# bempt/uda_aerial_semantic_segmentation_research

Measured on AMD Instinct MI355X. Metric: training images/sec at 512x512, higher is better.
Workload: dtype fp32

## Files before the change

include/udaseg.h:

```cpp
#ifndef UDASEG_H
#define UDASEG_H

#include <stddef.h>
#include <stdint.h>

#ifdef __cplusplus
extern "C" {
#endif

#define UDASEG_OK 0
#define UDASEG_E_BADARG (-1)
#define UDASEG_E_UNSUPPORTED (-2)
#define UDASEG_E_WORKSPACE (-3)
#define UDASEG_E_HIP (-4)

#define UDASEG_ACT_NONE 0
#define UDASEG_ACT_LEAKY 1

int udaseg_version(void);
#define UDASEG_OPT_GENERIC_GATHER 0
#define UDASEG_OPT_F32_SPLIT 1
#define UDASEG_OPT_WGRAD_GENERIC 2
#define UDASEG_OPT_F32_HALO 3
#define UDASEG_OPT_F3_CFG 4
#define UDASEG_OPT_F3_WS 5
#define UDASEG_OPT_F3_SIGNS 6
#define UDASEG_OPT_IGEMM_TILE 7
#define UDASEG_OPT_IGEMM_X3 8
#define UDASEG_OPT_NO_FOLD 9
#define UDASEG_OPT_WGRAD_X3_BLOCKS 10
#define UDASEG_OPT_WGRAD_BLOCKS 11
#define UDASEG_OPT_WGRAD_NO_XCD 12
#define UDASEG_OPT_WGRAD_X3 13
#define UDASEG_OPT_NO_WGRAD_HALO 14
#define UDASEG_OPT_WGRAD_F3_BLOCKS 15
#define UDASEG_OPT_WGRAD_HALO_BLOCKS 16
#define UDASEG_OPT_WGRAD_DEEP_BLOCKS 17
#define UDASEG_OPT_WGRAD_DB 18
#define UDASEG_OPT_REDUCE_BLOCKS 19
#define UDASEG_OPT_BN_APPLY_PT 20
#define UDASEG_OPT_GEMM_1X1_TILE 21
#define UDASEG_OPT_GEMM_1X1 22
#define UDASEG_OPT_GEMM_1X1_MAXM 23
#define UDASEG_OPT_NO_STREAM 24
#define UDASEG_OPT_HALO_CFG 25
#define UDASEG_OPT_NO_HALO 26
#define UDASEG_OPT_NO_HALO_S2 27
#define UDASEG_OPT_HALO_W16 28
#define UDASEG_OPT_HALO_DEEP 29
#define UDASEG_OPT_HALO_S2_CK 30
#define UDASEG_OPT_UP_CFG 31
#define UDASEG_OPT_WGRAD_UP_BLOCKS 32
#define UDASEG_OPT_COUNT 33
int udaseg_set_option(int key, int value);
int udaseg_get_option(int key);
int udaseg_option_count(void);
const char* udaseg_option_name(int key);
int udaseg_option_epoch(void);
const char* udaseg_last_error(void);
int udaseg_device_count(void);
int udaseg_memset_async(void* ptr, int value, size_t bytes, void* stream);
int udaseg_stream_wait(void* waiter_stream, void* signal_stream);

typedef struct {
  int n, hi, wi, ci;
  int ho, wo, co;
  int kh, kw, stride, pad;
} udaseg_conv_desc;


int udaseg_conv2d_fwd(const udaseg_conv_desc* d, const float* x, const float* w, const float* bias, float* y,
                      int act, float slope, int accumulate, void* stream);
int udaseg_conv2d_fwd_bnstats(const udaseg_conv_desc* d, const float* x, const float* w, const float* bias, float* y,
                              double* stats, void* stream);
int udaseg_conv2d_fwd_fused(const udaseg_conv_desc* d, const float* x, const float* w, const float* bias,
                            const float* residual, float* y, int act, float slope, void* stream);
int udaseg_conv2d_fwd_bf16(const udaseg_conv_desc* d, const void* x, const void* w, const float* bias, const void* residual,
                           void* y, int out_f32, int act, float slope, double* stats, void* stream);
int udaseg_conv2d_dgrad_bf16(const udaseg_conv_desc* d, const void* dy, const void* w_t, void* dx, int accumulate,
                             void* stream);
int udaseg_conv2d_wgrad_bf16(const udaseg_conv_desc* d, const void* x, const void* dy, float* dw, int accumulate, void* stream);
int udaseg_conv2d_dgrad(const udaseg_conv_desc* d, const float* dy, const float* w_t, float* dx, int accumulate,
                        void* stream);
int udaseg_conv2d_dgrad_bnreduce_ok(const udaseg_conv_desc* d);
int udaseg_conv2d_dgrad_bnreduce(const udaseg_conv_desc* d, const float* dy, const float* w_t, float* dx, const float* prev_y,
                                 const float* save_mean, const float* save_rstd, const float* gamma, const float* beta, int act,
                                 float slope, double* bsums, void* stream);
int udaseg_conv2d_dgrad_bnreduce_bf16_ok(const udaseg_conv_desc* d);
int udaseg_conv2d_dgrad_bnreduce_bf16(const udaseg_conv_desc* d, const void* dy, const void* w_t, void* dx, const void* prev_y,
                                      const float* save_mean, const float* save_rstd, const float* gamma, const float* beta,
                                      int act, float slope, double* bsums, void* stream);
int udaseg_conv2d_wgrad(const udaseg_conv_desc* d, const float* x, const float* dy, float* dw, int accumulate,
                        void* stream);
int udaseg_conv2d_fwd_upcat(const udaseg_conv_desc* d, const float* a, const float* skip, int ca, const float* w,
                            const float* bias, float* y, int act, float slope, double* stats, void* stream);
int udaseg_conv2d_fwd_upcat_bf16(const udaseg_conv_desc* d, const void* a, const void* skip, int ca, const void* w,
                                 const float* bias, void* y, int act, float slope, double* stats, void* stream);
int udaseg_conv2d_dgrad_split(const udaseg_conv_desc* d, const float* dy, const float* w_t, float* dx_a, float* dx_b, int ca,
                              void* stream);
int udaseg_conv2d_dgrad_split_bf16(const udaseg_conv_desc* d, const void* dy, const void* w_t, void* dx_a, void* dx_b, int ca,
                                   void* stream);
int udaseg_conv2d_wgrad_part(const udaseg_conv_desc* d, const float* src, int src_c, int c_off, int up, const float* dy,
                             float* dw, int accumulate, void* stream);
int udaseg_conv2d_wgrad_part_bf16(const udaseg_conv_desc* d, const void* src, int src_c, int c_off, int up, const void* dy,
                                  float* dw, int accumulate, void* stream);
int udaseg_pack_dgrad_weights(const udaseg_conv_desc* d, const float* w, float* w_t, void* stream);
int udaseg_pack_dgrad_batched(const float* arena, float* packed, const int* table, int entries, void* stream);
double udaseg_conv_flops(const udaseg_conv_desc* d);

int udaseg_nchw_to_nhwc(const float* x, float* y, int n, int c, int h, int w, int cpad, void* stream);

int udaseg_bn_replicas(void);
int udaseg_bn_stats(const float* y, int64_t pixels, int c, double* sums, void* stream);
int udaseg_bn_stats_bf16(const void* y, int64_t pixels, int c, double* sums, void* stream);
int udaseg_bn_apply(const float* y, const double* sums, const float* gamma, const float* beta, const float* residual,
                    float* z, int64_t pixels, int c, float eps, float momentum, float* running_mean,
                    float* running_var, float* save_mean, float* save_rstd, int act, float slope, void* stream);
int udaseg_bn_apply_eval(const float* y, const float* gamma, const float* beta, const float* running_mean,
                         const float* running_var, const float* residual, float* z, int64_t pixels, int c, float eps,
                         int act, float slope, void* stream);
int udaseg_bn_fold(const float* w, const float* bias, const float* gamma, const float* beta, const float* running_mean,
                   const float* running_var, float eps, int co, int row_len, float* w_folded, float* bias_folded, void* stream);
int udaseg_bn_bwd_reduce(const float* dz, const float* z, const float* y, const float* save_mean,
                         const float* save_rstd, const float* gamma, const float* beta, int64_t pixels, int c,
                         double* bsums, int act, float slope, void* stream);
int udaseg_bn_bwd_apply(const float* dz, const float* z, const float* y, const float* save_mean,
                        const float* save_rstd, const float* gamma, const float* beta, const double* bsums, float* dy,
                        float* dres, float* dgamma, float* dbeta, int64_t pixels, int c, int act, float slope,
                        int accumulate_dy, int accumulate_dres, int accumulate_param, void* stream);
int udaseg_act_bwd(const float* dz, const float* z, float* dy, int64_t count, int act, float slope, void* stream);
int udaseg_channel_sum(const float* x, int64_t pixels, int c, float* out,
                       int accumulate, void* stream);
int udaseg_channel_sum_ws(const float* x, int64_t pixels, int c, float* out, int accumulate, float* scratch,
                          size_t scratch_bytes, void* stream);
size_t udaseg_channel_sum_scratch_bytes(int c);

int udaseg_maxpool3x3s2_fwd(const float* x, float* y, uint8_t* idx, int n, int h, int w, int c, void* stream);
int udaseg_maxpool3x3s2_bwd(const float* dy, const uint8_t* idx, float* dx, int n, int h, int w, int c, int accumulate,
                            void* stream);
int udaseg_upsample2x_concat_fwd(const float* a, const float* skip, float* out, int n, int h, int w, int ca, int cb,
                                 void* stream);
int udaseg_upsample2x_concat_bwd(const float* dout, float* da, float* dskip, int n, int h, int w, int ca, int cb,
                                 int accumulate_da, int accumulate_dskip, void* stream);

int udaseg_upsample2x_bilinear_concat_fwd(const void* a, const void* skip, void* out, int n, int h, int w, int ca, int cb,
                                          int bf16, void* stream);
int udaseg_upsample2x_bilinear_concat_bwd(const void* dout, void* da, void* dskip, int n, int h, int w, int ca, int cb,
                                          int accumulate_da, int accumulate_dskip, int bf16, void* stream);

int udaseg_ce_partials(void);
int udaseg_ce_fwd(const float* logits, const int64_t* target, int64_t pixels, int classes, int ldc, float* lse,
                  double* partials, float* loss, void* stream);
int udaseg_ce_bwd(const float* logits, const int64_t* target, const float* lse, const float* grad_out, int64_t pixels,
                  int classes, int ldc, float* dlogits, float* colsum_partials, float* colsum, void* stream);

int udaseg_ce_fwd_bwd(const float* logits, const int64_t* target, int64_t pixels, int classes, int ldc, double* partials, float* loss,
                      float* dlogits, float* colsum_partials, float* colsum, void* stream);
int udaseg_scale_unless_one(float* x, int64_t count, float* x2, int count2, const float* g, void* stream);

int udaseg_seg_partials(void);
int udaseg_dice_fwd(const float* logits, const int64_t* target, int batch, int64_t pix_per_image, int classes, int ldc,
                    float smooth, float eps, int pooled, double* sums, float* coef, float* loss, void* stream);
int udaseg_dice_bwd(const float* logits, const int64_t* target, const float* coef, const float* grad_out, float weight,
                    int batch, int64_t pix_per_image, int classes, int ldc, float* dlogits, int accumulate, void* stream);
int udaseg_focal_fwd(const float* logits, const int64_t* target, const float* class_weights, float alpha, float gamma,
                     int64_t pixels, int classes, int ldc, int mean, double* partials, float* loss, int accumulate,
                     void* stream);
int udaseg_focal_bwd(const float* logits, const int64_t* target, const float* class_weights, float alpha, float gamma,
                     const float* grad_out, float weight, int64_t pixels, int classes, int ldc, float* dlogits,
                     int accumulate, void* stream);
int udaseg_consistency_fwd(const float* z1, const float* z2, float temperature, int batch, int64_t pixels, int classes,
                           int ldc, double* partials, float* loss, void* stream);
int udaseg_consistency_bwd(const float* z1, const float* z2, float temperature, const float* grad_out, float weight,
                           int batch, int64_t pixels, int classes, int ldc, float* d1, float* d2, int accumulate,
                           void* stream);

int udaseg_argmax_confusion(const float* logits, const int64_t* target, int64_t pixels, int classes, int ldc,
                            int64_t* confusion, int64_t* pred, void* stream);

int udaseg_gap_splits(int hw);
int udaseg_gap_linear_sigmoid_fwd(const float* z, const float* w, const float* b, float* partial, float* pooled,
                                  float* p, int n, int hw, int c, void* stream);
int udaseg_gap_linear_sigmoid_bwd(const float* dp, const float* p, const float* pooled, const float* w, float* dz,
                                  float* dw, float* db, int n, int hw, int c, int accumulate_param, void* stream);
int udaseg_gap_linear_fwd(const float* z, const float* w, const float* b, float* partial, float* pooled, float* logit, int n,
                          int hw, int c, void* stream);
int udaseg_gap_linear_bwd(const float* dlogit, const float* pooled, const float* w, float* dz, float* dw, float* db, int n,
                          int hw, int c, int accumulate_param, void* stream);
int udaseg_bce_logits_fwd(const float* x, int n, float label, float weight, float* loss, int accumulate, void* stream);
int udaseg_bce_logits_bwd(const float* x, int n, float label, float weight, const float* grad_out, float* dx,
                          int accumulate, void* stream);
int udaseg_bce_logits_target_fwd(const float* x, const float* target, int n, float weight, float* loss, int accumulate,
                                 void* stream);
int udaseg_bce_logits_target_bwd(const float* x, const float* target, int n, float weight, const float* grad_out, float* dx,
                                 int accumulate, void* stream);

int udaseg_adam_flat(float* p, const float* g, float* m, float* v, int64_t count, float lr, float beta1, float beta2,
                     float eps, float bc1, float bc2, void* stream);

int udaseg_prepare_batch_u8(const uint8_t* images, const uint8_t* masks, const int32_t* d4, int n, int h, int w,
                            const float* mean255, const float* inv_std255, void* out_images, int cpad, int out_bf16,
                            int64_t* out_masks, int square_checked, void* stream);

int udaseg_set_workspace(void* ptr, size_t bytes);
size_t udaseg_workspace_bytes(const udaseg_conv_desc* d);

int udaseg_bn_apply_bf16(const void* y, const double* sums, const float* gamma, const float* beta, const void* residual,
                         void* z, int64_t pixels, int c, float eps, float momentum, float* running_mean, float* running_var,
                         float* save_mean, float* save_rstd, int act, float slope, void* stream);
int udaseg_bn_bwd_reduce_bf16(const void* dz, const void* z, const void* y, const float* save_mean, const float* save_rstd,
                              int64_t pixels, int c, double* bsums, int act, float slope, void* stream);
int udaseg_bn_bwd_apply_bf16(const void* dz, const void* z, const void* y, const float* save_mean, const float* save_rstd,
                             const float* gamma, const double* bsums, void* dy, void* dres, float* dgamma, float* dbeta,
                             int64_t pixels, int c, int act, float slope, int accumulate_dy, int accumulate_dres,
                             int accumulate_param, void* stream);
int udaseg_act_bwd_bf16(const void* dz, const void* z, void* dy, int64_t count, int act, float slope, void* stream);
int udaseg_channel_sum_bf16(const void* x, int64_t pixels, int c, float* out, int accumulate, void* stream);
int udaseg_channel_sum_bf16_ws(const void* x, int64_t pixels, int c, float* out, int accumulate, float* scratch,
                               size_t scratch_bytes, void* stream);
int udaseg_nchw_to_nhwc_bf16(const float* x, void* y, int n, int c, int h, int w, int cpad, void* stream);
int udaseg_cast_f32_to_bf16(const float* x, void* y, int64_t count, void* stream);
int udaseg_maxpool3x3s2_fwd_bf16(const void* x, void* y, uint8_t* idx, int n, int h, int w, int c, void* stream);
int udaseg_maxpool3x3s2_bwd_bf16(const void* dy, const uint8_t* idx, void* dx, int n, int h, int w, int c, int accumulate,
                                 void* stream);
int udaseg_upsample2x_concat_bwd_bf16(const void* dout, void* da, void* dskip, int n, int h, int w, int ca, int cb,
                                      int accumulate_da, int accumulate_dskip, void* stream);
int udaseg_gap_partial_bf16(const void* z, float* partial, int n, int hw, int c, void* stream);
int udaseg_gap_finish(const float* partial, const float* w, const float* b, float* pooled, float* p, int n, int hw, int c,
                      void* stream);
int udaseg_gap_bwd_broadcast_bf16(const float* dp, const float* p, const float* w, void* dz, int n, int hw, int c, void* stream);
int udaseg_gap_bwd_param(const float* dp, const float* p, const float* pooled, float* dw, float* db, int n, int c,
                         int accumulate_param, void* stream);
int udaseg_pack_dgrad_batched_bf16(const float* arena, void* packed, const int* table, int entries, void* stream);

int64_t udaseg_frag_elems(int n_out, int k_in, int ks);
int udaseg_set_stats_scratch(void* ptr, size_t bytes);
int udaseg_pack_frag_batched_bf16(const void* w16, const void* wt16, void* packed, const int* table, int entries, void* stream);
int udaseg_bn_finalize(const double* sums, const float* gamma, const float* beta, int64_t pixels, int c, float eps, float momentum,
                       float* running_mean, float* running_var, float* save_mean, float* save_rstd, float* scale, float* shift,
                       void* stream);
int udaseg_bn_bwd_apply_recompute_bf16(const void* dz, const void* y, const float* fwd_scale, const float* fwd_shift,
                                       const float* save_mean, const float* save_rstd, const float* gamma, const double* bsums,
                                       void* dy, float* dgamma, float* dbeta, int64_t pixels, int c, int act, float slope,
                                       void* stream);
int udaseg_conv2d_wgrad_halo_bf16_ok(const udaseg_conv_desc* d, int up_ca);
int udaseg_conv2d_wgrad_halo_bf16(const udaseg_conv_desc* d, const void* x, const void* skip, int up_ca, const void* dy, float* dw,
                                  void* stream);
int udaseg_conv2d_wgrad_bnin_bf16(const udaseg_conv_desc* d, const void* x, const float* in_scale, const float* in_shift, int in_act,
                                  float in_slope, const void* dy, float* dw, int accumulate, void* stream);
int udaseg_conv_frag_ok(const udaseg_conv_desc* d, int dgrad, int up_ca);
int udaseg_conv_frag_preferred(const udaseg_conv_desc* d, int dgrad, int up_ca);
int udaseg_conv2d_fwd_frag_bf16(const udaseg_conv_desc* d, const void* x, const void* skip, int up_ca, const void* wfrag,
                                const float* bias, const float* in_scale, const float* in_shift, int in_act, float in_slope,
                                void* y, int out_f32, int act, float slope, double* stats, void* stream);
int udaseg_conv2d_dgrad_frag_bf16(const udaseg_conv_desc* d, const void* dy, const void* wfrag_t, void* dx, void* dx2, int split,
                                  const void* prev_y, const float* save_mean, const float* save_rstd, const float* gamma,
                                  const float* beta, int bn_act, float bn_slope, double* bsums, int accumulate, void* stream);

int udaseg_pack_frag_batched_f32x3(const float* w32, const float* wt32, void* packed, const int* table, int entries, void* stream);
int udaseg_conv_f32x3_ok(const udaseg_conv_desc* d, int dgrad, int up_ca);
int udaseg_conv_f32x3_preferred(const udaseg_conv_desc* d, int dgrad, int up_ca);
int udaseg_f32x3_force_config(int cfg);
int udaseg_conv2d_fwd_f32x3(const udaseg_conv_desc* d, const float* x, const float* skip, int up_ca, const void* wfrag3,
                            const float* bias, float* y, int act, float slope, double* stats, void* stream);
int udaseg_conv2d_fwd_f32x3_bnin_ok(const udaseg_conv_desc* d, int up);
int udaseg_conv2d_fwd_f32x3_bnin_writes(const udaseg_conv_desc* d);
int udaseg_conv2d_fwd_f32x3_bnin(const udaseg_conv_desc* d, const float* x, int up, const float* in_scale, const float* in_shift,
                                 int in_act, float in_slope, float* z_out, const void* wfrag3, const float* bias, float* y, int act,
                                 float slope, double* stats, void* stream);
int udaseg_conv2d_wgrad_bnin_ok(const udaseg_conv_desc* d, int up);
int udaseg_conv2d_wgrad_bnin(const udaseg_conv_desc* d, const float* x, int up, const float* in_scale, const float* in_shift,
                             int in_act, float in_slope, const float* dy, float* dw, int accumulate, void* stream);
int udaseg_conv2d_dgrad_f32x3(const udaseg_conv_desc* d, const float* dy, const void* wfrag3_t, float* dx, float* dx2, int split,
                              const float* prev_y, const float* save_mean, const float* save_rstd, const float* gamma,
                              const float* beta, int bn_act, float bn_slope, double* bsums, int accumulate, void* stream);

int udaseg_conv2d_wgrad_halo_f32x3_ok(const udaseg_conv_desc* d, int up_ca);
int udaseg_conv2d_wgrad_halo_f32x3(const udaseg_conv_desc* d, const float* x, const float* skip, int up_ca, const float* dy,
                                   float* dw, void* stream);

int udaseg_conv_up_f32x3_ok(const udaseg_conv_desc* d, int up_ca);
int udaseg_pack_up_batched_f32x3(const float* w32, const float* wt32, void* packed, const int* table, int entries, void* stream);
int udaseg_conv2d_fwd_up_f32x3(const udaseg_conv_desc* d, const float* a, int up_ca, const void* wfrag_up, float* y, int accumulate,
                               double* stats, void* stream);
int udaseg_conv2d_dgrad_up_f32x3(const udaseg_conv_desc* d, const float* dy, int up_ca, const void* wfrag_up_t, float* da,
                                 const float* prev_y, const float* save_mean, const float* save_rstd, const float* gamma,
                                 const float* beta, int bn_act, float bn_slope, double* bsums, int accumulate, void* stream);
int udaseg_up_f32x3_force_config(int cfg);
int udaseg_conv2d_wgrad_up_f32x3_ok(const udaseg_conv_desc* d, int up_ca);
int udaseg_conv2d_wgrad_up_f32x3(const udaseg_conv_desc* d, const float* a, int up_ca, const float* dy, float* dw, void* stream);
int udaseg_conv2d_wgrad_halo_slice_f32x3(const udaseg_conv_desc* d, const float* x, const float* dy, float* dw, int ldw, int c_off,
                                         void* stream);
int udaseg_wgrad_up_set_blocks(int blocks);

int udaseg_conv_n16_f32x3_ok(const udaseg_conv_desc* d, int dgrad);
int udaseg_conv2d_fwd_n16_f32x3(const udaseg_conv_desc* d, const float* x, const float* in_scale, const float* in_shift, int in_act,
                                float in_slope, const void* wfrag, float* y, double* stats, void* stream);
int udaseg_conv2d_dgrad_n16_f32x3(const udaseg_conv_desc* d, const float* dy, const void* wfrag_t, float* dx, const float* prev_y,
                                  const float* save_mean, const float* save_rstd, const float* gamma, const float* beta, int bn_act,
                                  float bn_slope, double* bsums, void* stream);

int udaseg_conv_stem_f32x3_ok(const udaseg_conv_desc* d);
int udaseg_conv2d_fwd_stem_f32x3(const udaseg_conv_desc* d, const float* x, const void* wfrag, float* y, double* stats, void* stream);

int udaseg_debug_set_timeline(void* buffer, int blocks);

int udaseg_fill_f32(float* p, int64_t count, float value, void* stream);
int udaseg_axpy_f32(float* y, const float* x, int64_t count, float alpha, void* stream);
int udaseg_add_i64(int64_t* p, int64_t count, int64_t value, void* stream);
int udaseg_scale_f32(const float* x, float* y, int64_t count, float alpha, void* stream);

int udaseg_predict_gather_u8(const uint8_t* image, int h, int w, int th, int tw, int rows, int cols, int sy, int sx, int first,
                             int tiles, int views, const float* mean255, const float* inv_std255, void* out, int cpad,
                             int out_bf16, void* stream);
int udaseg_predict_blend(const float* logits, int ldc, int h, int w, int th, int tw, int rows, int cols, int sy, int sx, int first,
                         int tiles, int views, int classes, const float* win_y, const float* win_x, float* acc, int ldp,
                         float* wsum, void* stream);
int udaseg_predict_finish(float* probs, const float* wsum, int64_t pixels, int classes, int ldc, int64_t* labels, void* stream);
int udaseg_predict_threshold(const float* logits, int n, int hw, int classes, int ldc, float* out, void* stream);

int udaseg_prof_enable(int on);
int udaseg_prof_reset(void);
int udaseg_prof_read(int family, double* total_ms, double* total_flops, int64_t* launches);
int udaseg_prof_kernel_count(void);
const char* udaseg_prof_kernel_name(int kid);
int udaseg_prof_kernel_read(int kid, double* total_ms, double* total_flops, int64_t* launches);
int udaseg_prof_records(int family, int max_records, double* ms, double* flops, int* kind, int* desc11);

#ifdef __cplusplus
}
#endif
#endif
```

uda_aerial_semantic_segmentation_research_amd/_lib.py:

```python
import ctypes as C
import os

_HERE = os.path.dirname(os.path.abspath(__file__))
LIB_PATH = os.environ.get("UDASEG_LIB", os.path.join(_HERE, "libudaseg_hip.so"))

ACT_NONE = 0
ACT_LEAKY = 1


class ConvDesc(C.Structure):
    _fields_ = [(k, C.c_int) for k in ("n", "hi", "wi", "ci", "ho", "wo", "co", "kh", "kw", "stride", "pad")]


_P = C.c_void_p
_I = C.c_int
_L = C.c_int64
_F = C.c_float
_D = C.POINTER(ConvDesc)

SIGNATURES = {
    "udaseg_version": (_I, []),
    "udaseg_set_option": (_I, [_I, _I]),
    "udaseg_get_option": (_I, [_I]),
    "udaseg_option_count": (_I, []),
    "udaseg_option_name": (C.c_char_p, [_I]),
    "udaseg_option_epoch": (_I, []),
    "udaseg_last_error": (C.c_char_p, []),
    "udaseg_device_count": (_I, []),
    "udaseg_memset_async": (_I, [_P, _I, C.c_size_t, _P]),
    "udaseg_stream_wait": (_I, [_P, _P]),
    "udaseg_conv2d_fwd": (_I, [_D, _P, _P, _P, _P, _I, _F, _I, _P]),
    "udaseg_conv2d_fwd_bnstats": (_I, [_D, _P, _P, _P, _P, _P, _P]),
    "udaseg_conv2d_fwd_fused": (_I, [_D, _P, _P, _P, _P, _P, _I, _F, _P]),
    "udaseg_conv2d_fwd_bf16": (_I, [_D, _P, _P, _P, _P, _P, _I, _I, _F, _P, _P]),
    "udaseg_conv2d_dgrad_bf16": (_I, [_D, _P, _P, _P, _I, _P]),
    "udaseg_conv2d_wgrad_bf16": (_I, [_D, _P, _P, _P, _I, _P]),
    "udaseg_conv2d_dgrad": (_I, [_D, _P, _P, _P, _I, _P]),
    "udaseg_conv2d_wgrad": (_I, [_D, _P, _P, _P, _I, _P]),
    "udaseg_conv2d_dgrad_bnreduce_ok": (_I, [_D]),
    "udaseg_conv2d_dgrad_bnreduce": (_I, [_D, _P, _P, _P, _P, _P, _P, _P, _P, _I, _F, _P, _P]),
    "udaseg_conv2d_dgrad_bnreduce_bf16_ok": (_I, [_D]),
    "udaseg_conv2d_dgrad_bnreduce_bf16": (_I, [_D, _P, _P, _P, _P, _P, _P, _P, _P, _I, _F, _P, _P]),
    "udaseg_conv2d_fwd_upcat": (_I, [_D, _P, _P, _I, _P, _P, _P, _I, _F, _P, _P]),
    "udaseg_conv2d_fwd_upcat_bf16": (_I, [_D, _P, _P, _I, _P, _P, _P, _I, _F, _P, _P]),
    "udaseg_conv2d_dgrad_split": (_I, [_D, _P, _P, _P, _P, _I, _P]),
    "udaseg_conv2d_dgrad_split_bf16": (_I, [_D, _P, _P, _P, _P, _I, _P]),
    "udaseg_conv2d_wgrad_part": (_I, [_D, _P, _I, _I, _I, _P, _P, _I, _P]),
    "udaseg_conv2d_wgrad_part_bf16": (_I, [_D, _P, _I, _I, _I, _P, _P, _I, _P]),
    "udaseg_pack_dgrad_weights": (_I, [_D, _P, _P, _P]),
    "udaseg_pack_dgrad_batched": (_I, [_P, _P, _P, _I, _P]),
    "udaseg_conv_flops": (C.c_double, [_D]),
    "udaseg_nchw_to_nhwc": (_I, [_P, _P, _I, _I, _I, _I, _I, _P]),
    "udaseg_bn_replicas": (_I, []),
    "udaseg_bn_stats": (_I, [_P, _L, _I, _P, _P]),
    "udaseg_bn_stats_bf16": (_I, [_P, _L, _I, _P, _P]),
    "udaseg_bn_apply": (_I, [_P, _P, _P, _P, _P, _P, _L, _I, _F, _F, _P, _P, _P, _P, _I, _F, _P]),
    "udaseg_bn_apply_eval": (_I, [_P, _P, _P, _P, _P, _P, _P, _L, _I, _F, _I, _F, _P]),
    "udaseg_bn_fold": (_I, [_P, _P, _P, _P, _P, _P, _F, _I, _I, _P, _P, _P]),
    "udaseg_bn_bwd_reduce": (_I, [_P, _P, _P, _P, _P, _P, _P, _L, _I, _P, _I, _F, _P]),
    "udaseg_bn_bwd_apply": (_I, [_P, _P, _P, _P, _P, _P, _P, _P, _P, _P, _P, _P, _L, _I, _I, _F, _I, _I, _I, _P]),
    "udaseg_act_bwd": (_I, [_P, _P, _P, _L, _I, _F, _P]),
    "udaseg_channel_sum": (_I, [_P, _L, _I, _P, _I, _P]),
    "udaseg_channel_sum_ws": (_I, [_P, _L, _I, _P, _I, _P, C.c_size_t, _P]),
    "udaseg_channel_sum_scratch_bytes": (C.c_size_t, [_I]),
    "udaseg_maxpool3x3s2_fwd": (_I, [_P, _P, _P, _I, _I, _I, _I, _P]),
    "udaseg_maxpool3x3s2_bwd": (_I, [_P, _P, _P, _I, _I, _I, _I, _I, _P]),
    "udaseg_upsample2x_concat_fwd": (_I, [_P, _P, _P, _I, _I, _I, _I, _I, _P]),
    "udaseg_upsample2x_concat_bwd": (_I, [_P, _P, _P, _I, _I, _I, _I, _I, _I, _I, _P]),
    "udaseg_upsample2x_bilinear_concat_fwd": (_I, [_P, _P, _P, _I, _I, _I, _I, _I, _I, _P]),
    "udaseg_upsample2x_bilinear_concat_bwd": (_I, [_P, _P, _P, _I, _I, _I, _I, _I, _I, _I, _I, _P]),
    "udaseg_ce_partials": (_I, []),
    "udaseg_ce_fwd": (_I, [_P, _P, _L, _I, _I, _P, _P, _P, _P]),
    "udaseg_ce_bwd": (_I, [_P, _P, _P, _P, _L, _I, _I, _P, _P, _P, _P]),
    "udaseg_ce_fwd_bwd": (_I, [_P, _P, _L, _I, _I, _P, _P, _P, _P, _P, _P]),
    "udaseg_scale_unless_one": (_I, [_P, _L, _P, _I, _P, _P]),
    "udaseg_seg_partials": (_I, []),
    "udaseg_dice_fwd": (_I, [_P, _P, _I, _L, _I, _I, _F, _F, _I, _P, _P, _P, _P]),
    "udaseg_gap_linear_fwd": (_I, [_P, _P, _P, _P, _P, _P, _I, _I, _I, _P]),
    "udaseg_gap_linear_bwd": (_I, [_P, _P, _P, _P, _P, _P, _I, _I, _I, _I, _P]),
    "udaseg_bce_logits_target_fwd": (_I, [_P, _P, _I, _F, _P, _I, _P]),
    "udaseg_bce_logits_target_bwd": (_I, [_P, _P, _I, _F, _P, _P, _I, _P]),
    "udaseg_scale_f32": (_I, [_P, _P, _L, _F, _P]),
    "udaseg_prepare_batch_u8": (_I, [_P, _P, _P, _I, _I, _I, _P, _P, _P, _I, _I, _P, _I, _P]),
    "udaseg_predict_gather_u8": (_I, [_P, _I, _I, _I, _I, _I, _I, _I, _I, _I, _I, _I, _P, _P, _P, _I, _I, _P]),
    "udaseg_predict_blend": (_I, [_P, _I, _I, _I, _I, _I, _I, _I, _I, _I, _I, _I, _I, _I, _P, _P, _P, _I, _P, _P]),
    "udaseg_predict_finish": (_I, [_P, _P, _L, _I, _I, _P, _P]),
    "udaseg_predict_threshold": (_I, [_P, _I, _I, _I, _I, _P, _P]),
    "udaseg_dice_bwd": (_I, [_P, _P, _P, _P, _F, _I, _L, _I, _I, _P, _I, _P]),
    "udaseg_focal_fwd": (_I, [_P, _P, _P, _F, _F, _L, _I, _I, _I, _P, _P, _I, _P]),
    "udaseg_focal_bwd": (_I, [_P, _P, _P, _F, _F, _P, _F, _L, _I, _I, _P, _I, _P]),
    "udaseg_consistency_fwd": (_I, [_P, _P, _F, _I, _L, _I, _I, _P, _P, _P]),
    "udaseg_consistency_bwd": (_I, [_P, _P, _F, _P, _F, _I, _L, _I, _I, _P, _P, _I, _P]),
    "udaseg_argmax_confusion": (_I, [_P, _P, _L, _I, _I, _P, _P, _P]),
    "udaseg_gap_splits": (_I, [_I]),
    "udaseg_gap_linear_sigmoid_fwd": (_I, [_P, _P, _P, _P, _P, _P, _I, _I, _I, _P]),
    "udaseg_gap_linear_sigmoid_bwd": (_I, [_P, _P, _P, _P, _P, _P, _P, _I, _I, _I, _I, _P]),
    "udaseg_bce_logits_fwd": (_I, [_P, _I, _F, _F, _P, _I, _P]),
    "udaseg_bce_logits_bwd": (_I, [_P, _I, _F, _F, _P, _P, _I, _P]),
    "udaseg_adam_flat": (_I, [_P, _P, _P, _P, _L, _F, _F, _F, _F, _F, _F, _P]),
    "udaseg_bn_apply_bf16": (_I, [_P, _P, _P, _P, _P, _P, _L, _I, _F, _F, _P, _P, _P, _P, _I, _F, _P]),
    "udaseg_bn_bwd_reduce_bf16": (_I, [_P, _P, _P, _P, _P, _L, _I, _P, _I, _F, _P]),
    "udaseg_bn_bwd_apply_bf16": (_I, [_P, _P, _P, _P, _P, _P, _P, _P, _P, _P, _P, _L, _I, _I, _F, _I, _I, _I, _P]),
    "udaseg_act_bwd_bf16": (_I, [_P, _P, _P, _L, _I, _F, _P]),
    "udaseg_channel_sum_bf16": (_I, [_P, _L, _I, _P, _I, _P]),
    "udaseg_channel_sum_bf16_ws": (_I, [_P, _L, _I, _P, _I, _P, C.c_size_t, _P]),
    "udaseg_nchw_to_nhwc_bf16": (_I, [_P, _P, _I, _I, _I, _I, _I, _P]),
    "udaseg_cast_f32_to_bf16": (_I, [_P, _P, _L, _P]),
    "udaseg_maxpool3x3s2_fwd_bf16": (_I, [_P, _P, _P, _I, _I, _I, _I, _P]),
    "udaseg_maxpool3x3s2_bwd_bf16": (_I, [_P, _P, _P, _I, _I, _I, _I, _I, _P]),
    "udaseg_upsample2x_concat_bwd_bf16": (_I, [_P, _P, _P, _I, _I, _I, _I, _I, _I, _I, _P]),
    "udaseg_gap_partial_bf16": (_I, [_P, _P, _I, _I, _I, _P]),
    "udaseg_gap_finish": (_I, [_P, _P, _P, _P, _P, _I, _I, _I, _P]),
    "udaseg_gap_bwd_broadcast_bf16": (_I, [_P, _P, _P, _P, _I, _I, _I, _P]),
    "udaseg_gap_bwd_param": (_I, [_P, _P, _P, _P, _P, _I, _I, _I, _P]),
    "udaseg_pack_dgrad_batched_bf16": (_I, [_P, _P, _P, _I, _P]),
    "udaseg_bn_finalize": (_I, [_P, _P, _P, _L, _I, _F, _F, _P, _P, _P, _P, _P, _P, _P]),
    "udaseg_bn_bwd_apply_recompute_bf16": (_I, [_P, _P, _P, _P, _P, _P, _P, _P, _P, _P, _P, _L, _I, _I, _F, _P]),
    "udaseg_conv2d_wgrad_halo_bf16_ok": (_I, [_D, _I]),
    "udaseg_conv2d_wgrad_halo_bf16": (_I, [_D, _P, _P, _I, _P, _P, _P]),
    "udaseg_conv2d_wgrad_bnin_bf16": (_I, [_D, _P, _P, _P, _I, _F, _P, _P, _I, _P]),
    "udaseg_frag_elems": (_L, [_I, _I, _I]),
    "udaseg_set_stats_scratch": (_I, [_P, C.c_size_t]),
    "udaseg_pack_frag_batched_bf16": (_I, [_P, _P, _P, _P, _I, _P]),
    "udaseg_conv_frag_ok": (_I, [_D, _I, _I]),
    "udaseg_conv_frag_preferred": (_I, [_D, _I, _I]),
    "udaseg_conv2d_fwd_frag_bf16": (_I, [_D, _P, _P, _I, _P, _P, _P, _P, _I, _F, _P, _I, _I, _F, _P, _P]),
    "udaseg_conv2d_dgrad_frag_bf16": (_I, [_D, _P, _P, _P, _P, _I, _P, _P, _P, _P, _P, _I, _F, _P, _I, _P]),
    "udaseg_pack_frag_batched_f32x3": (_I, [_P, _P, _P, _P, _I, _P]),
    "udaseg_conv2d_wgrad_halo_f32x3_ok": (_I, [_D, _I]),
    "udaseg_conv2d_wgrad_halo_f32x3": (_I, [_D, _P, _P, _I, _P, _P, _P]),
    "udaseg_conv_f32x3_ok": (_I, [_D, _I, _I]),
    "udaseg_f32x3_force_config": (_I, [_I]),
    "udaseg_conv_f32x3_preferred": (_I, [_D, _I, _I]),
    "udaseg_conv2d_fwd_f32x3": (_I, [_D, _P, _P, _I, _P, _P, _P, _I, _F, _P, _P]),
    "udaseg_conv2d_fwd_f32x3_bnin_ok": (_I, [_D, _I]),
    "udaseg_conv2d_fwd_f32x3_bnin_writes": (_I, [_D]),
    "udaseg_conv2d_fwd_f32x3_bnin": (_I, [_D, _P, _I, _P, _P, _I, _F, _P, _P, _P, _P, _I, _F, _P, _P]),
    "udaseg_conv2d_wgrad_bnin_ok": (_I, [_D, _I]),
    "udaseg_conv2d_wgrad_bnin": (_I, [_D, _P, _I, _P, _P, _I, _F, _P, _P, _I, _P]),
    "udaseg_conv2d_dgrad_f32x3": (_I, [_D, _P, _P, _P, _P, _I, _P, _P, _P, _P, _P, _I, _F, _P, _I, _P]),
    "udaseg_conv_up_f32x3_ok": (_I, [_D, _I]),
    "udaseg_pack_up_batched_f32x3": (_I, [_P, _P, _P, _P, _I, _P]),
    "udaseg_conv2d_fwd_up_f32x3": (_I, [_D, _P, _I, _P, _P, _I, _P, _P]),
    "udaseg_conv2d_dgrad_up_f32x3": (_I, [_D, _P, _I, _P, _P, _P, _P, _P, _P, _P, _I, _F, _P, _I, _P]),
    "udaseg_up_f32x3_force_config": (_I, [_I]),
    "udaseg_conv2d_wgrad_up_f32x3_ok": (_I, [_D, _I]),
    "udaseg_conv2d_wgrad_up_f32x3": (_I, [_D, _P, _I, _P, _P, _P]),
    "udaseg_conv2d_wgrad_halo_slice_f32x3": (_I, [_D, _P, _P, _P, _I, _I, _P]),
    "udaseg_wgrad_up_set_blocks": (_I, [_I]),
    "udaseg_conv_stem_f32x3_ok": (_I, [_D]),
    "udaseg_conv2d_fwd_stem_f32x3": (_I, [_D, _P, _P, _P, _P, _P]),
    "udaseg_conv_n16_f32x3_ok": (_I, [_D, _I]),
    "udaseg_conv2d_fwd_n16_f32x3": (_I, [_D, _P, _P, _P, _I, _F, _P, _P, _P, _P]),
    "udaseg_conv2d_dgrad_n16_f32x3": (_I, [_D, _P, _P, _P, _P, _P, _P, _P, _P, _I, _F, _P, _P]),
    "udaseg_set_workspace": (_I, [_P, C.c_size_t]),
    "udaseg_workspace_bytes": (C.c_size_t, [_D]),
    "udaseg_debug_set_timeline": (_I, [_P, _I]),
    "udaseg_fill_f32": (_I, [_P, _L, _F, _P]),
    "udaseg_axpy_f32": (_I, [_P, _P, _L, _F, _P]),
    "udaseg_add_i64": (_I, [_P, _L, _L, _P]),
    "udaseg_prof_enable": (_I, [_I]),
    "udaseg_prof_reset": (_I, []),
    "udaseg_prof_read": (_I, [_I, C.POINTER(C.c_double), C.POINTER(C.c_double), C.POINTER(C.c_int64)]),
    "udaseg_prof_kernel_count": (_I, []),
    "udaseg_prof_kernel_name": (C.c_char_p, [_I]),
    "udaseg_prof_kernel_read": (_I, [_I, C.POINTER(C.c_double), C.POINTER(C.c_double), C.POINTER(C.c_int64)]),
    "udaseg_prof_records": (_I, [_I, _I, C.POINTER(C.c_double), C.POINTER(C.c_double), C.POINTER(C.c_int), C.POINTER(C.c_int)]),
}

OPTIONS = {"GENERIC_GATHER": 0, "F32_SPLIT": 1, "WGRAD_GENERIC": 2, "F32_HALO": 3, "F3_CFG": 4, "F3_WS": 5, "F3_SIGNS": 6, "IGEMM_TILE": 7, "IGEMM_X3": 8, "NO_FOLD": 9, "WGRAD_X3_BLOCKS": 10, "WGRAD_BLOCKS": 11, "WGRAD_NO_XCD": 12, "WGRAD_X3": 13, "NO_WGRAD_HALO": 14, "WGRAD_F3_BLOCKS": 15, "WGRAD_HALO_BLOCKS": 16, "WGRAD_DEEP_BLOCKS": 17, "WGRAD_DB": 18, "REDUCE_BLOCKS": 19, "BN_APPLY_PT": 20, "GEMM_1X1_TILE": 21, "GEMM_1X1": 22, "GEMM_1X1_MAXM": 23, "NO_STREAM": 24, "HALO_CFG": 25, "NO_HALO": 26, "NO_HALO_S2": 27, "HALO_W16": 28, "HALO_DEEP": 29, "HALO_S2_CK": 30, "UP_CFG": 31, "WGRAD_UP_BLOCKS": 32}

_lib = None


def load():
    global _lib
    if _lib is not None:
        return _lib
    if not os.path.exists(LIB_PATH):
        raise RuntimeError(
            f"{LIB_PATH} not found: the HIP extension is not built. Run `python -c \"import __graft_entry__ as g; "
            f"g.build()\"` (or `make -C {os.path.join(_HERE, 'csrc')}`). There is no CPU fallback.")
    lib = C.CDLL(LIB_PATH)
    for name, (res, args) in SIGNATURES.items():
        fn = getattr(lib, name)
        fn.restype = res
        fn.argtypes = args
    _lib = lib
    return lib


def check(rc, what=""):
    if rc != 0:
        msg = load().udaseg_last_error().decode(errors="replace")
        raise RuntimeError(f"libudaseg_hip {what} failed (rc={rc}): {msg}")


def require_gpu():
    lib = load()
    if lib.udaseg_device_count() < 1:
        raise RuntimeError("libudaseg_hip: no HIP device visible; this path has no CPU fallback")
    return lib
```

uda_aerial_semantic_segmentation_research_amd/csrc/api.hip:

```cpp
#include <string.h>
#include <mutex>
#include <vector>

#include "common.h"
#include "options.h"

namespace udaseg {

static thread_local char g_err[512] = "";

void set_error(const char* fmt, ...) {
  va_list ap;
  va_start(ap, fmt);
  vsnprintf(g_err, sizeof(g_err), fmt, ap);
  va_end(ap);
}

int hip_fail(hipError_t e, const char* what) {
  set_error("%s: %s", what, hipGetErrorString(e));
  return UDASEG_E_HIP;
}

struct ProfRec {
  hipEvent_t a, b;
  double flops;
  int kind;
  udaseg_conv_desc d;
};
static bool g_prof_on = false;
struct KRec {
  hipEvent_t a, b;
  double flops;
};
static const char* const g_knames_fixed[PROF_NKERNELS] = {
    "conv_igemm_kernel<128, 128, 2, 2, false, false, false>", "conv_igemm_kernel<128, 64, 2, 2, false, false, false>",
    "conv_igemm_kernel<64, 64, 2, 2, false, false, false>",   "conv_igemm_kernel<128, 32, 4, 1, false, false, false>",
    "conv3x3_small_kernel<1, 1>",                             "conv3x3_small_kernel<2, 1>",
    "conv3x3_small_kernel<1, 2>",                             "conv_wgrad_kernel<64, 64, 2, 2, false>",
    "conv_wgrad_kernel<32, 128, 1, 4, false>",                "conv3x3_small_wgrad_kernel<1, 1>",
    "conv3x3_small_wgrad_kernel<2, 1>",                       "conv3x3_small_wgrad_kernel<1, 2>",
    "conv_igemm_kernel<*, bf16>",                             "conv_wgrad_bf16_kernel",
    "conv_igemm_kernel<128, 128, 2, 2, false, true, false>",  "conv_igemm_kernel<128, 64, 2, 2, false, true, false>",
    "conv_igemm_kernel<64, 64, 2, 2, false, true, false>",    "conv_igemm_kernel<128, 32, 4, 1, false, true, false>",
    "conv_wgrad_kernel<64, 64, 2, 2, true>",                  "conv_wgrad_kernel<32, 128, 1, 4, true>",
    "conv_igemm_kernel<128, 128, 2, 2, false, true, true>",   "conv_igemm_kernel<128, 64, 2, 2, false, true, true>",
    "conv_igemm_kernel<64, 64, 2, 2, false, true, true>",     "conv_igemm_kernel<128, 32, 4, 1, false, true, true>"};
constexpr int PROF_MAX_KERNELS = 160;
static std::vector<KRec> g_krecs[PROF_MAX_KERNELS];
static char g_knames_dyn[PROF_MAX_KERNELS][160];
static int g_nkernels = PROF_NKERNELS;

static std::mutex g_kprof_mutex;
int kprof_id(const char* name) {
  std::lock_guard<std::mutex> lock(g_kprof_mutex);
  for (int k = PROF_NKERNELS; k < g_nkernels; ++k)
    if (strcmp(g_knames_dyn[k], name) == 0) return k;
  if (g_nkernels >= PROF_MAX_KERNELS) {
    static bool warned = false;
    if (!warned) {
      fprintf(stderr, "libudaseg_hip: kernel-timing table full (%d symbols); '%s' and later symbols are booked under '%s'\n",
              PROF_MAX_KERNELS, name, g_knames_dyn[PROF_NKERNELS]);
      warned = true;
    }
    return PROF_NKERNELS;
  }
  strncpy(g_knames_dyn[g_nkernels], name, sizeof(g_knames_dyn[0]) - 1);
  return g_nkernels++;
}
static const char* kname(int kid) {
  if (kid < 0 || kid >= g_nkernels) return "";
  return kid < PROF_NKERNELS ? g_knames_fixed[kid] : g_knames_dyn[kid];
}
static std::vector<ProfRec> g_recs[2];
static std::vector<hipEvent_t> g_pool;
static hipEvent_t g_open[2];

static hipEvent_t get_event() {
  if (!g_pool.empty()) {
    hipEvent_t e = g_pool.back();
    g_pool.pop_back();
    return e;
  }
  hipEvent_t e;
  if (hipEventCreate(&e) != hipSuccess) return nullptr;
  return e;
}

hipEvent_t kprof_begin(hipStream_t s) {
  if (!g_prof_on) return nullptr;
  hipEvent_t a = get_event();
  if (a) (void)hipEventRecord(a, s);
  return a;
}

void kprof_end(int kid, hipEvent_t a, hipStream_t s, double flops) {
  if (!a) return;
  hipEvent_t b = get_event();
  if (!b || kid < 0 || kid >= PROF_MAX_KERNELS) return;
  (void)hipEventRecord(b, s);
  g_krecs[kid].push_back({a, b, flops});
}

static int g_prof_suspended = 0;
void prof_suspend(int on) { g_prof_suspended = on; }

void prof_begin(int family, hipStream_t s) {
  if (!g_prof_on || g_prof_suspended) return;
  g_open[family] = get_event();
  if (g_open[family]) (void)hipEventRecord(g_open[family], s);
}

void prof_end(int family, hipStream_t s, double flops, int kind, const udaseg_conv_desc* d) {
  if (!g_prof_on || g_prof_suspended || !g_open[family]) return;
  hipEvent_t b = get_event();
  if (!b) return;
  (void)hipEventRecord(b, s);
  ProfRec r = {g_open[family], b, flops, kind, {}};
  if (d) r.d = *d;
  g_recs[family].push_back(r);
  g_open[family] = nullptr;
}

}

using namespace udaseg;

extern "C" int udaseg_version(void) { return 100; }
extern "C" const char* udaseg_last_error(void) { return g_err; }

extern "C" int udaseg_device_count(void) {
  int n = 0;
  if (hipGetDeviceCount(&n) != hipSuccess) return 0;
  return n;
}

extern "C" int udaseg_memset_async(void* ptr, int value, size_t bytes, void* stream) {
  UDASEG_CHECK_ARG(ptr != nullptr || bytes == 0, "memset_async: NULL pointer");
  if (bytes == 0) return UDASEG_OK;
  hipError_t e = hipMemsetAsync(ptr, value, bytes, as_stream(stream));
  if (e != hipSuccess) return hip_fail(e, "hipMemsetAsync");
  return UDASEG_OK;
}

extern "C" int udaseg_stream_wait(void* waiter, void* signal) {
  constexpr int RING = 256;
  static hipEvent_t ring[16][RING] = {};
  static unsigned next[16] = {};
  static std::mutex mu;
  int dev = 0;
  UDASEG_CHECK_ARG(hipGetDevice(&dev) == hipSuccess && dev >= 0 && dev < 16, "stream_wait: no current HIP device");
  std::lock_guard<std::mutex> lk(mu);
  const unsigned slot = next[dev] % RING;
  if (ring[dev][slot] == nullptr) {
    hipError_t e = hipEventCreateWithFlags(&ring[dev][slot], hipEventDisableTiming);
    if (e != hipSuccess) {
      ring[dev][slot] = nullptr;
      return hip_fail(e, "hipEventCreateWithFlags(stream_wait ring)");
    }
  }
  hipEvent_t ev = ring[dev][slot];
  hipError_t e = hipEventRecord(ev, as_stream(signal));
  if (e != hipSuccess) return hip_fail(e, "hipEventRecord(stream_wait: is `signal` a stream of the current device?)");
  e = hipStreamWaitEvent(as_stream(waiter), ev, 0);
  if (e != hipSuccess) return hip_fail(e, "hipStreamWaitEvent(stream_wait)");
  ++next[dev];
  return UDASEG_OK;
}

extern "C" int udaseg_prof_enable(int on) {
  g_prof_on = on != 0;
  return UDASEG_OK;
}

extern "C" int udaseg_prof_reset(void) {
  for (int f = 0; f < 2; ++f) {
    for (auto& r : g_recs[f]) {
      g_pool.push_back(r.a);
      g_pool.push_back(r.b);
    }
    g_recs[f].clear();
  }
  for (int k = 0; k < g_nkernels; ++k) {
    for (auto& r : g_krecs[k]) {
      g_pool.push_back(r.a);
      g_pool.push_back(r.b);
    }
    g_krecs[k].clear();
  }
  return UDASEG_OK;
}

extern "C" int udaseg_prof_read(int family, double* total_ms, double* total_flops, int64_t* launches) {
  UDASEG_CHECK_ARG(family >= 0 && family < 2 && total_ms && total_flops && launches, "prof_read: bad arguments");
  double ms = 0.0, fl = 0.0;
  for (auto& r : g_recs[family]) {
    hipError_t e = hipEventSynchronize(r.b);
    if (e != hipSuccess) return hip_fail(e, "hipEventSynchronize(prof)");
    float t = 0.f;
    e = hipEventElapsedTime(&t, r.a, r.b);
    if (e != hipSuccess) return hip_fail(e, "hipEventElapsedTime(prof)");
    ms += t;
    fl += r.flops;
  }
  *total_ms = ms;
  *total_flops = fl;
  *launches = (int64_t)g_recs[family].size();
  return UDASEG_OK;
}

extern "C" int udaseg_prof_records(int family, int max_records, double* ms, double* flops, int* kind, int* desc11) {
  UDASEG_CHECK_ARG(family >= 0 && family < 2 && ms && flops && kind && desc11 && max_records >= 0, "prof_records: bad arguments");
  int n = 0;
  for (auto& r : g_recs[family]) {
    if (n >= max_records) break;
    hipError_t e = hipEventSynchronize(r.b);
    if (e != hipSuccess) return hip_fail(e, "hipEventSynchronize(prof)");
    float t = 0.f;
    e = hipEventElapsedTime(&t, r.a, r.b);
    if (e != hipSuccess) return hip_fail(e, "hipEventElapsedTime(prof)");
    ms[n] = t;
    flops[n] = r.flops;
    kind[n] = r.kind;
    const int v[11] = {r.d.n, r.d.hi, r.d.wi, r.d.ci, r.d.ho, r.d.wo, r.d.co, r.d.kh, r.d.kw, r.d.stride, r.d.pad};
    for (int i = 0; i < 11; ++i) desc11[n * 11 + i] = v[i];
    ++n;
  }
  return n;
}

namespace udaseg {
enum { K_INT, K_FLAG, K_OFF0 };
struct OptRow {
  const char* env;
  int kind, dflt;
};
static const OptRow g_opt_rows[UDASEG_OPT_COUNT] = {
     {"UDASEG_IGEMM_GENERIC", K_INT, 0},
     {"UDASEG_F32_SPLIT", K_OFF0, 1},
     {"UDASEG_WGRAD_GENERIC", K_INT, 0},
     {"UDASEG_F32_SPLIT", K_OFF0, 1},
     {"UDASEG_F3_CFG", K_INT, 0},
     {"UDASEG_F3_WS", K_OFF0, 1},
     {"UDASEG_F3_SIGNS", K_OFF0, 1},
     {"UDASEG_IGEMM_TILE", K_INT, 0},
     {"UDASEG_IGEMM_X3", K_INT, 1},
     {"UDASEG_NO_FOLD", K_FLAG, 0},
     {"UDASEG_WGRAD_X3_BLOCKS", K_INT, 1024},
     {"UDASEG_WGRAD_BLOCKS", K_INT, 0},
     {"UDASEG_WGRAD_NO_XCD", K_FLAG, 0},
     {"UDASEG_WGRAD_X3", K_OFF0, 1},
     {"UDASEG_NO_WGRAD_HALO", K_FLAG, 0},
     {"UDASEG_WGRAD_F3_BLOCKS", K_INT, 120},
     {"UDASEG_WGRAD_HALO_BLOCKS", K_INT, 96},
     {"UDASEG_WGRAD_DEEP_BLOCKS", K_INT, 0},
     {"UDASEG_WGRAD_DB", K_INT, 1},
     {"UDASEG_REDUCE_BLOCKS", K_INT, 0},
     {"UDASEG_BN_APPLY_PT", K_INT, 4},
     {"UDASEG_GEMM_1X1_TILE", K_INT, 0},
     {"UDASEG_GEMM_1X1", K_OFF0, 1},
     {"UDASEG_GEMM_1X1_MAXM", K_INT, 73728},
     {"UDASEG_NO_STREAM", K_FLAG, 0},
     {"UDASEG_HALO_CFG", K_INT, 0},
     {"UDASEG_NO_HALO", K_FLAG, 0},
     {"UDASEG_NO_HALO_S2", K_FLAG, 0},
     {"UDASEG_HALO_W16", K_INT, 6},
     {"UDASEG_HALO_DEEP", K_OFF0, 1},
     {"UDASEG_HALO_S2_CK", K_INT, 64},
     {"UDASEG_UP_CFG", K_INT, 0},
     {"UDASEG_WGRAD_UP_BLOCKS", K_INT, 0}};
int g_opt_val[UDASEG_OPT_COUNT];
static int g_opt_default[UDASEG_OPT_COUNT];
std::atomic<bool> g_opt_ready{false};
static std::atomic<int> g_opt_epoch{0};
static std::mutex g_opt_mutex;
void opt_init() {
  std::lock_guard<std::mutex> lk(g_opt_mutex);
  if (g_opt_ready.load(std::memory_order_relaxed)) return;
  for (int k = 0; k < UDASEG_OPT_COUNT; ++k) {
    const OptRow& r = g_opt_rows[k];
    const char* e = getenv(r.env);
    int v = r.dflt;
    if (r.kind == K_INT) v = e ? atoi(e) : r.dflt;
    else if (r.kind == K_FLAG) v = e != nullptr ? 1 : 0;
    else v = (e && atoi(e) == 0) ? 0 : 1;
    g_opt_default[k] = g_opt_val[k] = v;
  }
  g_opt_ready.store(true, std::memory_order_release);
}
}

extern "C" int udaseg_set_option(int key, int value) {
  UDASEG_CHECK_ARG(key >= 0 && key < UDASEG_OPT_COUNT, "set_option: unknown key %d (0 .. %d)", key, UDASEG_OPT_COUNT - 1);
  UDASEG_CHECK_ARG(value >= -1, "set_option: value must be >= 0, or -1 for the default");
  udaseg::opt_get(key);
  std::lock_guard<std::mutex> lk(udaseg::g_opt_mutex);
  udaseg::g_opt_val[key] = value < 0 ? udaseg::g_opt_default[key] : value;
  if (key == UDASEG_OPT_GENERIC_GATHER)
    udaseg::g_opt_val[UDASEG_OPT_WGRAD_GENERIC] = value < 0 ? udaseg::g_opt_default[UDASEG_OPT_WGRAD_GENERIC] : value;
  udaseg::g_opt_epoch.fetch_add(1);
  return UDASEG_OK;
}

extern "C" int udaseg_get_option(int key) {
  if (key < 0 || key >= UDASEG_OPT_COUNT) return -1;
  return udaseg::opt_get(key);
}

extern "C" int udaseg_option_count(void) { return UDASEG_OPT_COUNT; }
extern "C" const char* udaseg_option_name(int key) { return key >= 0 && key < UDASEG_OPT_COUNT ? udaseg::g_opt_rows[key].env : ""; }
extern "C" int udaseg_option_epoch(void) { return udaseg::g_opt_epoch.load(); }

extern "C" int udaseg_prof_kernel_count(void) { return g_nkernels; }
extern "C" const char* udaseg_prof_kernel_name(int kid) { return kname(kid); }

extern "C" int udaseg_prof_kernel_read(int kid, double* total_ms, double* total_flops, int64_t* launches) {
  UDASEG_CHECK_ARG(kid >= 0 && kid < g_nkernels && total_ms && total_flops && launches, "prof_kernel_read: bad arguments");
  double ms = 0.0, fl = 0.0;
  for (auto& r : g_krecs[kid]) {
    hipError_t e = hipEventSynchronize(r.b);
    if (e != hipSuccess) return hip_fail(e, "hipEventSynchronize(kprof)");
    float t = 0.f;
    e = hipEventElapsedTime(&t, r.a, r.b);
    if (e != hipSuccess) return hip_fail(e, "hipEventElapsedTime(kprof)");
    ms += t;
    fl += r.flops;
  }
  *total_ms = ms;
  *total_flops = fl;
  *launches = (int64_t)g_krecs[kid].size();
  return UDASEG_OK;
}
```

uda_aerial_semantic_segmentation_research_amd/csrc/common.h:

```cpp
#pragma once
#include <stdlib.h>
#include <hip/hip_runtime.h>
#include <stdint.h>
#include <stdio.h>
#include <stdarg.h>
#include <atomic>

#include "../../include/udaseg.h"
#include "options.h"

namespace udaseg {

void set_error(const char* fmt, ...);
int hip_fail(hipError_t e, const char* what);

#define UDASEG_CHECK_ARG(cond, ...)                 \
  do {                                              \
    if (!(cond)) {                                  \
      ::udaseg::set_error(__VA_ARGS__);             \
      return UDASEG_E_BADARG;                       \
    }                                               \
  } while (0)

#define UDASEG_LAUNCH_CHECK(what)                          \
  do {                                                     \
    hipError_t e__ = hipGetLastError();                    \
    if (e__ != hipSuccess) return ::udaseg::hip_fail(e__, what); \
  } while (0)

static inline hipStream_t as_stream(void* s) { return reinterpret_cast<hipStream_t>(s); }
static inline int64_t cdiv64(int64_t a, int64_t b) { return (a + b - 1) / b; }
static inline int cdiv(int a, int b) { return (a + b - 1) / b; }

typedef float f32x4 __attribute__((ext_vector_type(4)));
typedef float f32x16 __attribute__((ext_vector_type(16)));

__device__ __forceinline__ int fast_div(int n, int d, float rcp) {
  int q = (int)((float)n * rcp);
  int r = n - q * d;
  if (r < 0) { q -= 1; r += d; }
  if (r >= d) { q += 1; }
  return q;
}

__device__ __forceinline__ float act_apply(float x, int act, float slope) {
  return (act == UDASEG_ACT_LEAKY && x < 0.f) ? x * slope : x;
}
__device__ __forceinline__ float act_grad(float z, int act, float slope) {
  return (act == UDASEG_ACT_LEAKY && !(z > 0.f)) ? slope : 1.f;
}

__device__ __forceinline__ float wave_sum(float v) {
#pragma unroll
  for (int o = 32; o > 0; o >>= 1) v += __shfl_xor(v, o, 64);
  return v;
}
__device__ __forceinline__ double wave_sum_d(double v) {
#pragma unroll
  for (int o = 32; o > 0; o >>= 1) v += __shfl_xor(v, o, 64);
  return v;
}

template <int V, typename T>
__device__ __forceinline__ void block_fold_atomic(const T (&v)[V], T* __restrict__ dst, int cq, T* __restrict__ red) {
  const int tid = threadIdx.x, bs = blockDim.x;
#pragma unroll
  for (int e = 0; e < V; ++e) red[tid * V + e] = v[e];
  __syncthreads();
  if (cq >= bs) {
    const int base = (int)(((int64_t)blockIdx.x * bs) % cq);
    for (int j = tid; j < bs * V; j += bs) {
      int qq = base + j / V;
      if (qq >= cq) qq -= cq;
      atomicAdd(dst + qq * V + (j % V), red[j]);
    }
  } else {
    const int C = cq * V;
    for (int t = tid; t < C; t += bs) {
      T s = 0;
      for (int r = t / V; r < bs; r += cq) s += red[r * V + (t % V)];
      atomicAdd(dst + t, s);
    }
  }
  __syncthreads();
}

constexpr int BN_REPLICAS = 16;
constexpr int REDUCE_MAX_BLOCKS = 512;
static inline int reduce_max_blocks() {
  const int x = opt_get(UDASEG_OPT_REDUCE_BLOCKS);
  return x > 0 ? x : REDUCE_MAX_BLOCKS;
}

template <typename OutT>
__device__ __forceinline__ void pack_dgrad_tiles(const float* __restrict__ w, OutT* __restrict__ wt, int co, int T, int ci) {
  __shared__ float tile[32][33];
  const int ta = (co + 31) >> 5, tb = (ci + 31) >> 5;
  const int ntiles = T * ta * tb;
  const int row = threadIdx.x >> 3, q = threadIdx.x & 7;
  for (int tl = blockIdx.x; tl < ntiles; tl += gridDim.x) {
    const int b = tl % tb, r = tl / tb, a = r % ta, t = r / ta;
    {
      const int o = 32 * a + row, c = 32 * b + 4 * q;
      f32x4 v = {0.f, 0.f, 0.f, 0.f};
      if (o < co && c < ci) v = *reinterpret_cast<const f32x4*>(w + ((size_t)o * T + t) * ci + c);
#pragma unroll
      for (int k = 0; k < 4; ++k) tile[row][4 * q + k] = v[k];
    }
    __syncthreads();
    {
      const int c = 32 * b + row, o = 32 * a + 4 * q;
      if (c < ci && o < co) {
        OutT* dst = wt + ((size_t)c * T + t) * co + o;
        if constexpr (sizeof(OutT) == 4) {
          f32x4 v;
#pragma unroll
          for (int k = 0; k < 4; ++k) v[k] = tile[4 * q + k][row];
          *reinterpret_cast<f32x4*>(dst) = v;
        } else {
          unsigned short h[4];
#pragma unroll
          for (int k = 0; k < 4; ++k) h[k] = __builtin_bit_cast(unsigned short, (__bf16)tile[4 * q + k][row]);
          uint2 pk;
          pk.x = (unsigned)h[0] | ((unsigned)h[1] << 16);
          pk.y = (unsigned)h[2] | ((unsigned)h[3] << 16);
          *reinterpret_cast<uint2*>(dst) = pk;
        }
      }
    }
    __syncthreads();
  }
}
constexpr int PACK_DGRAD_GRID_X = 256;

void* workspace_ptr(size_t* bytes);

constexpr int CHSUM_REPLICAS = 16;
constexpr int CHSUM_DIRECT_BLOCKS = 32;
static __global__ void fold_replicas_kernel(const float* __restrict__ rep, int c, float* __restrict__ out, int accumulate) {
  const int i = blockIdx.x * blockDim.x + threadIdx.x;
  if (i >= c) return;
  float s = 0.f;
#pragma unroll
  for (int r = 0; r < CHSUM_REPLICAS; ++r) s += rep[(size_t)r * c + i];
  out[i] = accumulate ? out[i] + s : s;
}

struct StreamShape {
  int bs;
  int grid;
  int c4;
};

static inline StreamShape stream_shape(int64_t n4, int c4, int max_blocks = 2048, int per_thread = 4) {
  StreamShape s;
  s.c4 = c4;
  int unit;
  if (c4 <= 256) {
    s.bs = (256 / c4) * c4;
    unit = 1;
  } else {
    s.bs = 256;
    unit = (c4 + 255) / 256;
    while ((unit * 256) % c4 != 0) ++unit;
  }
  int64_t want = (n4 + (int64_t)s.bs * per_thread - 1) / ((int64_t)s.bs * per_thread);
  if (want > max_blocks) want = max_blocks;
  if (want < 1) want = 1;
  s.grid = (int)(((want + unit - 1) / unit) * unit);
  while ((int64_t)s.grid * s.bs < c4) s.grid += unit;
  return s;
}


static inline int apply_per_thread() {
  const int v = opt_get(UDASEG_OPT_BN_APPLY_PT);
  return (v < 1 || v > 256) ? 4 : v;
}

bool small_conv_applicable(int k, int stride, int pad, int ci_gather, int co_out);
int launch_small_conv(const float* x, const float* w, const float* bias, float* y, int n, int h, int wd, int ci, int co,
                      int flip, int accumulate, int act, float slope, double* stats, const float* residual, hipStream_t s,
                      int up = 0);
bool small_wgrad_applicable(int k, int stride, int pad, int ci, int co, int ntiles);
int launch_small_wgrad(const float* x, const float* dy, float* dw, int n, int h, int wd, int ci, int co, int accumulate,
                       hipStream_t s, int up = 0, const float* in_scale = nullptr, const float* in_shift = nullptr,
                       int in_act = 0, float in_slope = 0.f);

constexpr int PROF_NKERNELS = 24;
int kprof_id(const char* rocprof_symbol);
hipEvent_t kprof_begin(hipStream_t s);
void kprof_end(int kid, hipEvent_t a, hipStream_t s, double flops);
struct KTimer {
  std::atomic<int>* kid;
  hipStream_t s;
  hipEvent_t ev;
  double work;
  KTimer(std::atomic<int>* k, const char* rocprof_symbol, hipStream_t st, double w) : kid(k), s(st), work(w) {
    if (*kid < 0) *kid = kprof_id(rocprof_symbol);
    ev = kprof_begin(s);
  }
  ~KTimer() { kprof_end(*kid, ev, s, work); }
};
void prof_begin(int family, hipStream_t s);
void prof_suspend(int on);
void prof_end(int family, hipStream_t s, double flops, int kind, const udaseg_conv_desc* d);

}
```

uda_aerial_semantic_segmentation_research_amd/csrc/conv_n16_f32x3.hip:

```cpp
#include <stdlib.h>

#include "common.h"
#include "halo_common.h"

namespace udaseg {

struct N16Args {
  const float* x;
  const void* wf;
  float* y;
  int n, h, w, ci;
  double* stats;
  double* sscr;
  const float* bnb_y;
  const float* bnb_mean;
  const float* bnb_rstd;
  const float* bnb_gamma;
  const float* bnb_beta;
  int bnb_act;
  float bnb_slope;
  const float* in_scale;
  const float* in_shift;
  int in_act;
  float in_slope;
  int ntx, nty, nk16;
  int q1, q3;
  unsigned x_bytes, w_plane_bytes, y_bytes;
};

typedef float f32x4v __attribute__((ext_vector_type(4)));

struct N16Cfg {
  static constexpr int NT = 256, WM = 4, RPW = 2;
  static constexpr int TH = WM * RPW, TW = 32;
  static constexpr int HR = TH + 2, HWD = TW + 2;
  static constexpr int PLANE = HR * HWD * 32;
  static constexpr int LDS_HALO = 3 * PLANE;
  static constexpr int NPIECE = HR * HWD * 2;
  static constexpr int NI = (NPIECE + NT - 1) / NT;
  static constexpr int WCHUNK = 5 * 3 * 1024;
  static constexpr int NB = 2 * RPW;
};

template <int N>
__device__ __forceinline__ void row16_sum_n(float (&x)[N]) {
#pragma unroll
  for (int v = 0; v < N; ++v) asm volatile("v_add_f32_dpp %0, %0, %0 row_ror:8 row_mask:0xf bank_mask:0xf" : "+v"(x[v]));
  asm volatile("s_nop 1");
#pragma unroll
  for (int v = 0; v < N; ++v) asm volatile("v_add_f32_dpp %0, %0, %0 row_ror:4 row_mask:0xf bank_mask:0xf" : "+v"(x[v]));
  asm volatile("s_nop 1");
#pragma unroll
  for (int v = 0; v < N; ++v) asm volatile("v_add_f32_dpp %0, %0, %0 row_ror:2 row_mask:0xf bank_mask:0xf" : "+v"(x[v]));
  asm volatile("s_nop 1");
#pragma unroll
  for (int v = 0; v < N; ++v) asm volatile("v_add_f32_dpp %0, %0, %0 row_ror:1 row_mask:0xf bank_mask:0xf" : "+v"(x[v]));
  asm volatile("s_nop 1");
}

template <bool XF>
__global__ __launch_bounds__(256, 2) void conv3x3_n16_f32x3_kernel(const N16Args a) {
  using C = N16Cfg;
  extern __shared__ __attribute__((aligned(16))) char smem[];
  char* const wlds = smem + C::LDS_HALO;
  const int tid = threadIdx.x, lane = tid & 63;
  const int wave = __builtin_amdgcn_readfirstlane(tid >> 6);
  const int p = lane & 15, g = lane >> 4;

  const int H = a.h, W = a.w;
  const int ntiles = a.n * a.nty * a.ntx;
  const int oct = tid & 1;
  unsigned voff[C::NI], soffl[C::NI];
  unsigned inmask = 0;
#pragma unroll
  for (int i = 0; i < C::NI; ++i) soffl[i] = (unsigned)(((tid + i * C::NT) >> 1) * 32 + oct * 16);
  int img = 0, y0 = 0, x0 = 0;
  auto tile_setup = [&](int tl) {
    const int tx = tl % a.ntx;
    const int t2 = tl / a.ntx;
    const int ty = t2 % a.nty;
    img = t2 / a.nty;
    y0 = ty * C::TH;
    x0 = tx * C::TW;
#pragma unroll
    for (int i = 0; i < C::NI; ++i) {
      const int piece = tid + i * C::NT;
      const int pix = piece >> 1;
      const int hy = pix / C::HWD, hx = pix - hy * C::HWD;
      const int iy = y0 + hy - 1, ix = x0 + hx - 1;
      const bool ok = piece < C::NPIECE && (unsigned)iy < (unsigned)H && (unsigned)ix < (unsigned)W;
      voff[i] = ok ? (unsigned)((((img * H + iy) * W + ix) * a.ci + oct * 8) * 4) : 0x80000000u;
    }
  };
  __amdgpu_buffer_rsrc_t rs_x = __builtin_amdgcn_make_buffer_rsrc(const_cast<float*>(a.x), 0, (int)a.x_bytes, 0x00020000);
  __amdgpu_buffer_rsrc_t rs_w = __builtin_amdgcn_make_buffer_rsrc(const_cast<void*>(a.wf), 0, (int)(3u * a.w_plane_bytes), 0x00020000);

  u32x4 stage[C::NI][2];
  auto load_chunk = [&](int c) {
    const int soff = c * 64;
    const unsigned kill = (c * 16 + oct * 8 < a.ci) ? 0u : 0x80000000u;
    inmask = 0;
#pragma unroll
    for (int i = 0; i < C::NI; ++i) {
      stage[i][0] = __builtin_amdgcn_raw_buffer_load_b128(rs_x, (int)(voff[i] | kill), soff, 0);
      stage[i][1] = __builtin_amdgcn_raw_buffer_load_b128(rs_x, (int)(voff[i] | kill), soff + 16, 0);
      inmask |= (voff[i] != 0x80000000u ? 1u : 0u) << i;
    }
  };
  const bool xf_relu = a.in_act == UDASEG_ACT_LEAKY && a.in_slope == 0.f;
  auto store_chunk = [&](int c) {
    f32x4 sc0 = {0.f, 0.f, 0.f, 0.f}, sc1 = sc0, sh0 = sc0, sh1 = sc0;
    if constexpr (XF) {
      const int ch = c * 16 + oct * 8;
      if (ch < a.ci) {
        sc0 = *reinterpret_cast<const f32x4*>(a.in_scale + ch);
        sh0 = *reinterpret_cast<const f32x4*>(a.in_shift + ch);
        if (ch + 4 < a.ci) {
          sc1 = *reinterpret_cast<const f32x4*>(a.in_scale + ch + 4);
          sh1 = *reinterpret_cast<const f32x4*>(a.in_shift + ch + 4);
        }
      }
    }
#pragma unroll
    for (int i = 0; i < C::NI; ++i) {
      if (i < C::NI - 1 || tid + i * C::NT < C::NPIECE) {
        u32x4 lo = stage[i][0], hi = stage[i][1];
        if constexpr (XF) {
          const bool inside = (inmask >> i) & 1u;
          f32x4 l = __builtin_bit_cast(f32x4, lo), h = __builtin_bit_cast(f32x4, hi);
#pragma unroll
          for (int e = 0; e < 4; ++e) {
            float t0 = __builtin_fmaf(l[e], sc0[e], sh0[e]), t1 = __builtin_fmaf(h[e], sc1[e], sh1[e]);
            if (xf_relu) {
              t0 = t0 > 0.f ? t0 : 0.f;
              t1 = t1 > 0.f ? t1 : 0.f;
            } else {
              t0 = act_apply(t0, a.in_act, a.in_slope);
              t1 = act_apply(t1, a.in_act, a.in_slope);
            }
            l[e] = inside ? t0 : 0.f;
            h[e] = inside ? t1 : 0.f;
          }
          lo = __builtin_bit_cast(u32x4, l);
          hi = __builtin_bit_cast(u32x4, h);
        }
        u32x4 p0, p1, p2;
        split3(lo, hi, p0, p1, p2);
        *reinterpret_cast<u32x4*>(smem + soffl[i]) = p0;
        *reinterpret_cast<u32x4*>(smem + C::PLANE + soffl[i]) = p1;
        *reinterpret_cast<u32x4*>(smem + 2 * C::PLANE + soffl[i]) = p2;
      }
    }
  };

  {
    const int npc = a.nk16 * 5 * 64;
    for (int i = tid; i < 3 * npc; i += C::NT) {
      const int pl = i / npc, r = i - pl * npc;
      const int f = r >> 6, ln = r & 63;
      const u32x4 v = __builtin_amdgcn_raw_buffer_load_b128(rs_w, (int)(pl * a.w_plane_bytes + r * 16), 0, 0);
      *reinterpret_cast<u32x4*>(wlds + (f * 3 + pl) * 1024 + ln * 16) = v;
    }
  }

  int toff[5];
#pragma unroll
  for (int j = 0; j < 5; ++j) {
    int tap = 2 * j + (g >> 1);
    if (tap > 8) tap = 8;
    toff[j] = ((tap / 3) * C::HWD + (tap % 3)) * 32;
  }
  const int pbase = ((wave * C::RPW) * C::HWD + p) * 32 + (g & 1) * 16;

  __amdgpu_buffer_rsrc_t rs_y = __builtin_amdgcn_make_buffer_rsrc(a.y, 0, (int)a.y_bytes, 0x00020000);
  const bool want_stats = a.stats != nullptr && a.bnb_y == nullptr;
  const bool want_bnb = a.bnb_y != nullptr;
  __amdgpu_buffer_rsrc_t rs_p = __builtin_amdgcn_make_buffer_rsrc(const_cast<float*>(want_bnb ? a.bnb_y : a.x), 0,
                                                                  (int)(want_bnb ? a.y_bytes : 0u), 0x00020000);
  float s[8];
#pragma unroll
  for (int v = 0; v < 8; ++v) s[v] = 0.f;
  f32x4 sc = {0.f, 0.f, 0.f, 0.f}, sh = sc, mu = sc, rsd = sc;
  if (want_bnb) {
    mu = *reinterpret_cast<const f32x4*>(a.bnb_mean + 4 * g);
    rsd = *reinterpret_cast<const f32x4*>(a.bnb_rstd + 4 * g);
    const f32x4 gm = *reinterpret_cast<const f32x4*>(a.bnb_gamma + 4 * g), bt = *reinterpret_cast<const f32x4*>(a.bnb_beta + 4 * g);
#pragma unroll
    for (int e = 0; e < 4; ++e) {
      sc[e] = gm[e] * rsd[e];
      sh[e] = bt[e] - mu[e] * sc[e];
    }
  }

  int tile = blockIdx.x;
  if (tile < ntiles) {
    tile_setup(tile);
    load_chunk(0);
  }
  for (; tile < ntiles; tile += gridDim.x) {
    const int cimg = img, cy0 = y0, cx0 = x0;
    f32x4v acc[C::NB];
#pragma unroll
    for (int b = 0; b < C::NB; ++b) acc[b] = f32x4v{0.f, 0.f, 0.f, 0.f};
    for (int c = 0; c < a.nk16; ++c) {
      store_chunk(c);
      __syncthreads();
      if (c + 1 < a.nk16) {
        load_chunk(c + 1);
      } else if (tile + (int)gridDim.x < ntiles) {
        tile_setup(tile + gridDim.x);
        load_chunk(0);
      }
#pragma unroll
      for (int j = 0; j < 5; ++j) {
        const int G = 5 * c + j;
        if (G == a.q1 || G == a.q3) {
#pragma unroll
          for (int b = 0; b < C::NB; ++b) acc[b] = -acc[b];
        }
        u32x4 A[3];
#pragma unroll
        for (int pl = 0; pl < 3; ++pl) A[pl] = *reinterpret_cast<const u32x4*>(wlds + ((c * 5 + j) * 3 + pl) * 1024 + lane * 16);
#pragma unroll
        for (int b = 0; b < C::NB; ++b) {
          const int r = b >> 1, bx = b & 1;
          u32x4 B[3];
#pragma unroll
          for (int pl = 0; pl < 3; ++pl)
            B[pl] = *reinterpret_cast<const u32x4*>(smem + pl * C::PLANE + pbase + toff[j] + (r * C::HWD + bx * 16) * 32);
#pragma unroll
          for (int ij = 2; ij >= 0; --ij)
#pragma unroll
            for (int i = 0; i <= ij; ++i)
              acc[b] = __builtin_amdgcn_mfma_f32_16x16x32_bf16(__builtin_bit_cast(bf16x8, A[i]), __builtin_bit_cast(bf16x8, B[ij - i]), acc[b], 0, 0, 0);
        }
      }
      __syncthreads();
    }

#pragma unroll
    for (int b = 0; b < C::NB; ++b) {
      const int oy = cy0 + wave * C::RPW + (b >> 1), ox = cx0 + 16 * (b & 1) + p;
      const bool cv = oy < H && ox < W;
      const unsigned off = cv ? (((unsigned)((cimg * H + oy) * W + ox)) * 16u + 4u * (unsigned)g) * 4u : 0x80000000u;
      const u32x4 d = __builtin_bit_cast(u32x4, acc[b]);
      __builtin_amdgcn_raw_buffer_store_b128(d, rs_y, (int)off, 0, 0);
      if (want_stats) {
#pragma unroll
        for (int e = 0; e < 4; ++e) {
          const float q = cv ? acc[b][e] : 0.f;
          s[e] += q;
          s[4 + e] = __builtin_fmaf(q, q, s[4 + e]);
        }
      }
      if (want_bnb) {
        const f32x4 yv = __builtin_bit_cast(f32x4, __builtin_amdgcn_raw_buffer_load_b128(rs_p, (int)off, 0, 0));
#pragma unroll
        for (int e = 0; e < 4; ++e) {
          const float yy = yv[e];
          const float gg = cv ? acc[b][e] * act_grad(__builtin_fmaf(yy, sc[e], sh[e]), a.bnb_act, a.bnb_slope) : 0.f;
          s[e] += gg;
          s[4 + e] = __builtin_fmaf(gg, (yy - mu[e]) * rsd[e], s[4 + e]);
        }
      }
    }
  }
  if (want_stats || want_bnb) {
    asm volatile("s_nop 1");
    row16_sum_n(s);
    float* red = reinterpret_cast<float*>(smem);
    if (p == 0) {
#pragma unroll
      for (int e = 0; e < 4; ++e) {
        red[wave * 32 + 4 * g + e] = s[e];
        red[wave * 32 + 16 + 4 * g + e] = s[4 + e];
      }
    }
    __syncthreads();
    if (tid < 32) {
      const float tot = red[tid] + red[32 + tid] + red[64 + tid] + red[96 + tid];
      atomicAdd(a.stats + (size_t)(blockIdx.x % HALO_STATS_REPLICAS) * 32 + tid, (double)tot);
    }
  }
}

static bool n16_applicable(const udaseg_conv_desc* d, int dgrad) {
  if (!d || !f32_halo_enabled()) return false;
  if (d->kh != 3 || d->kw != 3 || d->stride != 1 || d->pad != 1 || d->ho != d->hi || d->wo != d->wi) return false;
  const int gathered = dgrad ? d->co : d->ci, produced = dgrad ? d->ci : d->co;
  if (produced != 16 || gathered % 8 != 0 || gathered < 8 || gathered > 32 || d->n <= 0 || d->hi <= 0 || d->wi < 16) return false;
  const long long px = (long long)d->n * d->hi * d->wi;
  return px * 32 * 4 < (1LL << 31);
}

static int launch_n16(N16Args a, hipStream_t s, double flops) {
  using C = N16Cfg;
  a.ntx = cdiv(a.w, C::TW);
  a.nty = cdiv(a.h, C::TH);
  a.nk16 = (a.ci + 15) / 16;
  a.q1 = a.q3 = -1;
  if (f3_signs_on()) {
    const int ng = 5 * a.nk16;
    a.q1 = (ng + 2) / 4;
    a.q3 = ng - a.q1;
  }
  const int lds = C::LDS_HALO + a.nk16 * C::WCHUNK;
  const long long ntiles = (long long)a.n * a.nty * a.ntx;
  if (ntiles <= 0) return UDASEG_OK;
  if (ntiles >= (1LL << 31)) return UDASEG_E_UNSUPPORTED;
  static int cus = 0;
  if (cus == 0) {
    int dev = 0;
    hipDeviceProp_t pr;
    cus = (hipGetDevice(&dev) == hipSuccess && hipGetDeviceProperties(&pr, dev) == hipSuccess && pr.multiProcessorCount > 0)
              ? pr.multiProcessorCount : 256;
  }
  const long long resident = (long long)cus * (a.nk16 == 1 ? 3 : 2);
  const long long blocks = ntiles < resident ? ntiles : resident;
  a.sscr = nullptr;
  const bool xf = a.in_scale != nullptr;
  auto kern = xf ? conv3x3_n16_f32x3_kernel<true> : conv3x3_n16_f32x3_kernel<false>;
  static std::atomic<bool> attr_done[2] = {{false}, {false}};
  if (!attr_done[xf]) {
    hipError_t e = hipFuncSetAttribute(reinterpret_cast<const void*>(kern), hipFuncAttributeMaxDynamicSharedMemorySize,
                                       C::LDS_HALO + 2 * C::WCHUNK);
    if (e != hipSuccess) return hip_fail(e, "hipFuncSetAttribute(conv3x3_n16_f32x3)");
    attr_done[xf] = true;
  }
  static std::atomic<int> kid[2] = {{-1}, {-1}};
  if (kid[xf] < 0) kid[xf] = kprof_id(xf ? "conv3x3_n16_f32x3_kernel<true>" : "conv3x3_n16_f32x3_kernel<false>");
  hipEvent_t ev = kprof_begin(s);
  hipLaunchKernelGGL(kern, dim3((unsigned)blocks), dim3(C::NT), lds, s, a);
  kprof_end(kid[xf], ev, s, flops);
  UDASEG_LAUNCH_CHECK("conv3x3_n16_f32x3 launch");
  return UDASEG_OK;
}

}

using namespace udaseg;

extern "C" int udaseg_conv_n16_f32x3_ok(const udaseg_conv_desc* d, int dgrad) { return n16_applicable(d, dgrad) ? 1 : 0; }

extern "C" int udaseg_conv2d_fwd_n16_f32x3(const udaseg_conv_desc* d, const float* x, const float* in_scale, const float* in_shift,
                                           int in_act, float in_slope, const void* wfrag, float* y, double* stats, void* stream) {
  UDASEG_CHECK_ARG(d && x && wfrag && y, "conv2d_fwd_n16_f32x3: NULL pointer");
  UDASEG_CHECK_ARG((in_scale == nullptr) == (in_shift == nullptr), "conv2d_fwd_n16_f32x3: in_scale and in_shift come together");
  UDASEG_CHECK_ARG(in_act == UDASEG_ACT_NONE || in_act == UDASEG_ACT_LEAKY, "conv2d_fwd_n16_f32x3: unknown activation %d", in_act);
  if (!n16_applicable(d, 0)) {
    set_error("conv2d_fwd_n16_f32x3: geometry not supported (ask udaseg_conv_n16_f32x3_ok first)");
    return UDASEG_E_UNSUPPORTED;
  }
  N16Args a = {};
  a.x = x; a.wf = wfrag; a.y = y;
  a.n = d->n; a.h = d->hi; a.w = d->wi; a.ci = d->ci;
  a.stats = stats;
  a.in_scale = in_scale; a.in_shift = in_shift; a.in_act = in_act; a.in_slope = in_slope;
  const long long px = (long long)d->n * d->hi * d->wi;
  a.x_bytes = (unsigned)(px * d->ci * 4);
  a.w_plane_bytes = (unsigned)(((d->ci + 15) / 16) * 5 * 1024);
  a.y_bytes = (unsigned)(px * 16 * 4);
  hipStream_t st = as_stream(stream);
  prof_begin(0, st);
  const int rc = launch_n16(a, st, udaseg_conv_flops(d));
  prof_end(0, st, udaseg_conv_flops(d), 0, d);
  return rc;
}

extern "C" int udaseg_conv2d_dgrad_n16_f32x3(const udaseg_conv_desc* d, const float* dy, const void* wfrag_t, float* dx,
                                             const float* prev_y, const float* save_mean, const float* save_rstd, const float* gamma,
                                             const float* beta, int bn_act, float bn_slope, double* bsums, void* stream) {
  UDASEG_CHECK_ARG(d && dy && wfrag_t && dx, "conv2d_dgrad_n16_f32x3: NULL pointer");
  const bool bn = prev_y != nullptr;
  UDASEG_CHECK_ARG(!bn || (save_mean && save_rstd && gamma && beta && bsums), "conv2d_dgrad_n16_f32x3: the BatchNorm-backward sums "
                   "need mean, rstd, gamma, beta, bsums");
  UDASEG_CHECK_ARG(bn || bsums == nullptr, "conv2d_dgrad_n16_f32x3: bsums without prev_y");
  if (!n16_applicable(d, 1)) {
    set_error("conv2d_dgrad_n16_f32x3: geometry not supported (ask udaseg_conv_n16_f32x3_ok first)");
    return UDASEG_E_UNSUPPORTED;
  }
  N16Args a = {};
  a.x = dy; a.wf = wfrag_t; a.y = dx;
  a.n = d->n; a.h = d->hi; a.w = d->wi; a.ci = d->co;
  if (bn) {
    a.bnb_y = prev_y; a.bnb_mean = save_mean; a.bnb_rstd = save_rstd; a.bnb_gamma = gamma; a.bnb_beta = beta;
    a.bnb_act = bn_act; a.bnb_slope = bn_slope; a.stats = bsums;
  }
  const long long px = (long long)d->n * d->hi * d->wi;
  a.x_bytes = (unsigned)(px * d->co * 4);
  a.w_plane_bytes = (unsigned)(((d->co + 15) / 16) * 5 * 1024);
  a.y_bytes = (unsigned)(px * 16 * 4);
  hipStream_t st = as_stream(stream);
  prof_begin(0, st);
  const int rc = launch_n16(a, st, udaseg_conv_flops(d));
  prof_end(0, st, udaseg_conv_flops(d), 1, d);
  return rc;
}
```

uda_aerial_semantic_segmentation_research_amd/csrc/conv_stem_f32x3.hip:

```cpp
#include <stdlib.h>

#include "common.h"
#include "halo_common.h"

namespace udaseg {

struct StemArgs {
  const float* x;
  const void* wf;
  float* y;
  int n, h, w;
  double* stats;
  int ntx, nty;
  int q1, q3;
  unsigned x_bytes, w_plane_bytes, y_bytes;
};

struct StemCfg {
  static constexpr int NT = 512, NW = 8;
  static constexpr int TH = 8, TW = 32;
  static constexpr int IR = 2 * TH + 5;
  static constexpr int NP = 35;
  static constexpr int ROWB = NP * 16;
  static constexpr int PLANE = IR * ROWB;
  static constexpr int LDS_BAND = 3 * PLANE;
  static constexpr int NPIECE = IR * NP;
  static constexpr int NI = (NPIECE + NT - 1) / NT;
  static constexpr int NFRAG = 7 * 2 * 2;
  static constexpr int LDS_W = 3 * NFRAG * 1024;
  static constexpr int LDS = LDS_BAND + LDS_W;
};

__global__ __launch_bounds__(512, 1) void conv_stem_f32x3_kernel(const StemArgs a) {
  using C = StemCfg;
  extern __shared__ __attribute__((aligned(16))) char smem[];
  char* const wlds = smem + C::LDS_BAND;
  const int tid = threadIdx.x, lane = tid & 63;
  const int wave = __builtin_amdgcn_readfirstlane(tid >> 6);
  const int lp = lane & 31, lh = lane >> 5;
  const int H = a.h, W = a.w, HO = a.h >> 1, WO = a.w >> 1;
  const int ntiles = a.n * a.nty * a.ntx;

  unsigned voff[C::NI][2];
  int img = 0, y0 = 0, x0 = 0;
  auto tile_setup = [&](int tl) {
    const int tx = tl % a.ntx;
    const int t2 = tl / a.ntx;
    const int ty = t2 % a.nty;
    img = t2 / a.nty;
    y0 = ty * C::TH;
    x0 = tx * C::TW;
#pragma unroll
    for (int i = 0; i < C::NI; ++i) {
      const int piece = tid + i * C::NT;
      const int r = piece / C::NP, q = piece - r * C::NP;
      const int iy = 2 * y0 - 3 + r, ix = 2 * x0 - 3 + 2 * q;
      const bool rok = piece < C::NPIECE && (unsigned)iy < (unsigned)H;
#pragma unroll
      for (int e = 0; e < 2; ++e)
        voff[i][e] = (rok && (unsigned)(ix + e) < (unsigned)W) ? (unsigned)(((img * H + iy) * W + ix + e) * 16) : 0x80000000u;
    }
  };
  __amdgpu_buffer_rsrc_t rs_x = __builtin_amdgcn_make_buffer_rsrc(const_cast<float*>(a.x), 0, (int)a.x_bytes, 0x00020000);
  __amdgpu_buffer_rsrc_t rs_w = __builtin_amdgcn_make_buffer_rsrc(const_cast<void*>(a.wf), 0, (int)(3u * a.w_plane_bytes), 0x00020000);
  u32x4 stage[C::NI][2];
  auto load_band = [&]() {
#pragma unroll
    for (int i = 0; i < C::NI; ++i) {
      stage[i][0] = __builtin_amdgcn_raw_buffer_load_b128(rs_x, (int)voff[i][0], 0, 0);
      stage[i][1] = __builtin_amdgcn_raw_buffer_load_b128(rs_x, (int)voff[i][1], 0, 0);
    }
  };
  auto store_band = [&]() {
#pragma unroll
    for (int i = 0; i < C::NI; ++i) {
      const int piece = tid + i * C::NT;
      if (i < C::NI - 1 || piece < C::NPIECE) {
        u32x4 p0, p1, p2;
        split3(stage[i][0], stage[i][1], p0, p1, p2);
        *reinterpret_cast<u32x4*>(smem + piece * 16) = p0;
        *reinterpret_cast<u32x4*>(smem + C::PLANE + piece * 16) = p1;
        *reinterpret_cast<u32x4*>(smem + 2 * C::PLANE + piece * 16) = p2;
      }
    }
  };

  for (int i = tid; i < 3 * C::NFRAG * 64; i += C::NT) {
    const int pl = i / (C::NFRAG * 64), r = i - pl * (C::NFRAG * 64);
    const int f = r >> 6, ln = r & 63;
    const u32x4 v = __builtin_amdgcn_raw_buffer_load_b128(rs_w, (int)(pl * a.w_plane_bytes + r * 16), 0, 0);
    *reinterpret_cast<u32x4*>(wlds + (f * 3 + pl) * 1024 + ln * 16) = v;
  }

  __amdgpu_buffer_rsrc_t rs_y = __builtin_amdgcn_make_buffer_rsrc(a.y, 0, (int)a.y_bytes, 0x00020000);
  const bool want_stats = a.stats != nullptr;
  float sA[32], sB[32];
#pragma unroll
  for (int v = 0; v < 32; ++v) sA[v] = sB[v] = 0.f;
  const int pbase = (2 * wave) * C::ROWB + 16 * lp + 16 * lh;

  int tile = blockIdx.x;
  if (tile < ntiles) {
    tile_setup(tile);
    load_band();
  }
  for (; tile < ntiles; tile += gridDim.x) {
    const int cimg = img, cy0 = y0, cx0 = x0;
    store_band();
    __syncthreads();
    if (tile + (int)gridDim.x < ntiles) {
      tile_setup(tile + gridDim.x);
      load_band();
    }
    f32x16 acc[2];
#pragma unroll
    for (int cb = 0; cb < 2; ++cb)
#pragma unroll
      for (int v = 0; v < 16; ++v) acc[cb][v] = 0.f;
#pragma unroll
    for (int ky = 0; ky < 7; ++ky)
#pragma unroll
      for (int h = 0; h < 2; ++h) {
        const int G = 2 * ky + h;
        if (G == a.q1 || G == a.q3) {
#pragma unroll
          for (int cb = 0; cb < 2; ++cb) acc[cb] = -acc[cb];
        }
        u32x4 B[3];
#pragma unroll
        for (int pl = 0; pl < 3; ++pl) B[pl] = *reinterpret_cast<const u32x4*>(smem + pl * C::PLANE + pbase + ky * C::ROWB + 32 * h);
#pragma unroll
        for (int cb = 0; cb < 2; ++cb) {
          u32x4 A[3];
#pragma unroll
          for (int pl = 0; pl < 3; ++pl) A[pl] = *reinterpret_cast<const u32x4*>(wlds + (((ky * 2 + h) * 2 + cb) * 3 + pl) * 1024 + lane * 16);
#pragma unroll
          for (int ij = 2; ij >= 0; --ij)
#pragma unroll
            for (int i = 0; i <= ij; ++i)
              acc[cb] = __builtin_amdgcn_mfma_f32_32x32x16_bf16(__builtin_bit_cast(bf16x8, A[i]), __builtin_bit_cast(bf16x8, B[ij - i]), acc[cb], 0, 0, 0);
        }
      }
    __syncthreads();

    const int oy = cy0 + wave, ox = cx0 + lp;
    const bool cv = oy < HO && ox < WO;
    const unsigned pixoff = (unsigned)((cimg * HO + oy) * WO + ox);
#pragma unroll
    for (int cb = 0; cb < 2; ++cb)
#pragma unroll
      for (int g = 0; g < 4; ++g) {
        const unsigned off = cv ? (pixoff * 64u + (unsigned)(cb * 32 + 8 * g + 4 * lh)) * 4u : 0x80000000u;
        float val[4];
#pragma unroll
        for (int e = 0; e < 4; ++e) val[e] = acc[cb][4 * g + e];
        if (want_stats) {
#pragma unroll
          for (int e = 0; e < 4; ++e) {
            const float q = cv ? val[e] : 0.f;
            sA[cb * 16 + 4 * g + e] += q;
            sB[cb * 16 + 4 * g + e] = __builtin_fmaf(q, q, sB[cb * 16 + 4 * g + e]);
          }
        }
        u32x4 d;
#pragma unroll
        for (int e = 0; e < 4; ++e) d[e] = __builtin_bit_cast(unsigned, val[e]);
        __builtin_amdgcn_raw_buffer_store_b128(d, rs_y, (int)off, 0, 0);
      }
  }
  if (want_stats) {
    asm volatile("s_nop 1");
    halfwave_sum_n(sA);
    halfwave_sum_n(sB);
    asm volatile("s_nop 1");
    float* red = reinterpret_cast<float*>(smem);
    if (lp == 31) {
#pragma unroll
      for (int v = 0; v < 32; ++v) {
        const int ch = (v >> 4) * 32 + (v & 3) + 8 * ((v & 15) >> 2) + 4 * lh;
        red[wave * 64 + ch] = sA[v];
        red[C::NW * 64 + wave * 64 + ch] = sB[v];
      }
    }
    __syncthreads();
    if (tid < 128) {
      const int which = tid >> 6, ch = tid & 63;
      float t = 0.f;
#pragma unroll
      for (int w8 = 0; w8 < C::NW; ++w8) t += red[which * C::NW * 64 + w8 * 64 + ch];
      atomicAdd(a.stats + (size_t)(blockIdx.x % HALO_STATS_REPLICAS) * 128 + which * 64 + ch, (double)t);
    }
  }
}

static bool stem_applicable(const udaseg_conv_desc* d) {
  if (!d || !f32_halo_enabled()) return false;
  if (d->kh != 7 || d->kw != 7 || d->stride != 2 || d->pad != 3 || d->ci != 4 || d->co != 64) return false;
  if (d->n <= 0 || d->hi < 2 || d->wi < 2 || d->hi % 2 != 0 || d->wi % 2 != 0 || d->ho * 2 != d->hi || d->wo * 2 != d->wi) return false;
  const long long pin = (long long)d->n * d->hi * d->wi, pout = (long long)d->n * d->ho * d->wo;
  return pin * 16 < (1LL << 31) && pout * 256 < (1LL << 31);
}

}

using namespace udaseg;

extern "C" int udaseg_conv_stem_f32x3_ok(const udaseg_conv_desc* d) { return stem_applicable(d) ? 1 : 0; }

extern "C" int udaseg_conv2d_fwd_stem_f32x3(const udaseg_conv_desc* d, const float* x, const void* wfrag, float* y, double* stats,
                                            void* stream) {
  UDASEG_CHECK_ARG(d && x && wfrag && y, "conv2d_fwd_stem_f32x3: NULL pointer");
  if (!stem_applicable(d)) {
    set_error("conv2d_fwd_stem_f32x3: geometry not supported (7x7 / stride 2 / pad 3, 4 -> 64 channels, even extents; ask "
              "udaseg_conv_stem_f32x3_ok first)");
    return UDASEG_E_UNSUPPORTED;
  }
  using C = StemCfg;
  StemArgs a = {};
  a.x = x; a.wf = wfrag; a.y = y;
  a.n = d->n; a.h = d->hi; a.w = d->wi;
  a.stats = stats;
  a.ntx = cdiv(d->wo, C::TW);
  a.nty = cdiv(d->ho, C::TH);
  a.q1 = a.q3 = -1;
  if (f3_signs_on()) {
    a.q1 = (14 + 2) / 4;
    a.q3 = 14 - a.q1;
  }
  a.x_bytes = (unsigned)((long long)d->n * d->hi * d->wi * 16);
  a.w_plane_bytes = (unsigned)(C::NFRAG * 1024);
  a.y_bytes = (unsigned)((long long)d->n * d->ho * d->wo * 256);
  const long long ntiles = (long long)d->n * a.nty * a.ntx;
  if (ntiles <= 0) return UDASEG_OK;
  static int cus = 0;
  if (cus == 0) {
    int dev = 0;
    hipDeviceProp_t pr;
    cus = (hipGetDevice(&dev) == hipSuccess && hipGetDeviceProperties(&pr, dev) == hipSuccess && pr.multiProcessorCount > 0)
              ? pr.multiProcessorCount : 256;
  }
  const long long blocks = ntiles < cus ? ntiles : cus;
  static std::atomic<bool> attr_done{false};
  if (!attr_done) {
    hipError_t e = hipFuncSetAttribute(reinterpret_cast<const void*>(conv_stem_f32x3_kernel), hipFuncAttributeMaxDynamicSharedMemorySize,
                                       C::LDS);
    if (e != hipSuccess) return hip_fail(e, "hipFuncSetAttribute(conv_stem_f32x3)");
    attr_done = true;
  }
  static std::atomic<int> kid{-1};
  if (kid < 0) kid = kprof_id("conv_stem_f32x3_kernel");
  hipStream_t st = as_stream(stream);
  prof_begin(0, st);
  hipEvent_t ev = kprof_begin(st);
  hipLaunchKernelGGL(conv_stem_f32x3_kernel, dim3((unsigned)blocks), dim3(C::NT), C::LDS, st, a);
  kprof_end(kid, ev, st, udaseg_conv_flops(d));
  prof_end(0, st, udaseg_conv_flops(d), 0, d);
  UDASEG_LAUNCH_CHECK("conv_stem_f32x3 launch");
  return UDASEG_OK;
}
```

uda_aerial_semantic_segmentation_research_amd/csrc/conv_wgrad.hip:

```cpp
#include <stdlib.h>

#include <type_traits>

#include "common.h"
#include "halo_common.h"

namespace udaseg {

struct WgradArgs {
  const void* x;
  const void* dy;
  float* dw;
  int hi, wi, ci, ho, wo, co;
  int kw, stride, pad;
  int M, J;
  int kchunk;
  int use_atomic;
  float inv_ci, inv_kw, inv_wo, inv_ho;
  int row_uniform;
  unsigned x_bytes, dy_bytes;
  int ci_full, c_off, J_ld, up;
  const float* in_scale;
  const float* in_shift;
  int in_act;
  float in_slope;
  int xcd_tiles, xcd_splits;
};

constexpr int WBK = 32;

template <int BMW, int BNW, int WAVES_M, int WAVES_N, bool ROWU>
__global__ __launch_bounds__(256) void conv_wgrad_kernel(const WgradArgs a) {
  constexpr int WM = BMW / WAVES_M, WN = BNW / WAVES_N;
  constexpr int TM = WM / 32, TN = WN / 32;
  constexpr int AQ = BMW / 4, BQ = BNW / 4;
  constexpr int A_ROWS = 256 / AQ, B_ROWS = 256 / BQ;
  constexpr int A_PASS = WBK / A_ROWS, B_PASS = WBK / B_ROWS;
  static_assert(WAVES_M * WAVES_N == 4, "4 waves");
  static_assert(A_PASS >= 1 && B_PASS >= 1, "tile too wide");

  __shared__ __attribute__((aligned(16))) float As[2][WBK][BMW];
  __shared__ __attribute__((aligned(16))) float Bs[2][WBK][BNW];

  const int tid = threadIdx.x, lane = tid & 63, wave = tid >> 6;
  const int lr = lane & 31, lh = lane >> 5;
  const int wm = (wave / WAVES_N) * WM, wn = (wave % WAVES_N) * WN;

  const int ntj = (a.J + BNW - 1) / BNW;
  const int co0 = (blockIdx.x / ntj) * BMW;
  const int j0 = (blockIdx.x % ntj) * BNW;
  const int kbeg = blockIdx.y * a.kchunk;
  const int kend = min(a.M, kbeg + a.kchunk);

  const int aq = tid % AQ, arow = tid / AQ;
  const int a_co = co0 + aq * 4;
  const bool a_ok = a_co < a.co;
  const int bq = tid % BQ, brow = tid / BQ;
  const int j = j0 + bq * 4;
  const bool b_ok = j < a.J;
  int b_dy = 0, b_dx = 0, b_c = 0;
  if (b_ok) {
    const int tap = fast_div(j, a.ci, a.inv_ci);
    b_c = j - tap * a.ci;
    const int r = fast_div(tap, a.kw, a.inv_kw);
    b_dy = r - a.pad;
    b_dx = (tap - r * a.kw) - a.pad;
  }

  f32x16 acc[TM][TN];
#pragma unroll
  for (int i = 0; i < TM; ++i)
#pragma unroll
    for (int jn = 0; jn < TN; ++jn)
#pragma unroll
      for (int v = 0; v < 16; ++v) acc[i][jn][v] = 0.f;

  f32x4 ra[A_PASS], rb[B_PASS];
  const int nkt = (kend - kbeg + WBK - 1) / WBK;

  unsigned u_ac[A_PASS], u_bc = 0;
  int u_bdy = 0, u_bx = 0;
  int s_ni[B_PASS], s_oy[B_PASS], s_ox[B_PASS];
  unsigned s_dyoff = 0;
  __amdgpu_buffer_rsrc_t rsrc_x, rsrc_dy;
  if constexpr (ROWU) {
    rsrc_x = __builtin_amdgcn_make_buffer_rsrc(const_cast<void*>(a.x), 0, (int)a.x_bytes, 0x00020000);
    rsrc_dy = __builtin_amdgcn_make_buffer_rsrc(const_cast<void*>(a.dy), 0, (int)a.dy_bytes, 0x00020000);
#pragma unroll
    for (int p = 0; p < A_PASS; ++p)
      u_ac[p] = a_ok ? (unsigned)((arow + A_ROWS * p) * a.co + a_co) * 4u : 0x80000000u;
    u_bdy = b_dy;
    u_bx = brow * a.stride + b_dx;
    u_bc = !b_ok ? 0x80000000u
                 : a.up ? (unsigned)((u_bx >> 1) * a.ci + b_c) * 4u
                        : (unsigned)((b_dy * a.wi + brow * a.stride + b_dx) * a.ci + b_c) * 4u;
    s_dyoff = (unsigned)kbeg * (unsigned)a.co * 4u;
#pragma unroll
    for (int p = 0; p < B_PASS; ++p) {
      const int m = kbeg + B_ROWS * p;
      const int t1 = m / a.wo;
      s_ox[p] = m - t1 * a.wo;
      s_ni[p] = t1 / a.ho;
      s_oy[p] = t1 - s_ni[p] * a.ho;
    }
  }

  auto load_tile = [&](int kt) {
    if constexpr (ROWU) {
#pragma unroll
      for (int p = 0; p < A_PASS; ++p)
        ra[p] = __builtin_bit_cast(f32x4, __builtin_amdgcn_raw_buffer_load_b128(rsrc_dy, (int)(u_ac[p] + s_dyoff), 0, 0));
      s_dyoff += (unsigned)(WBK * 4) * (unsigned)a.co;
#pragma unroll
      for (int p = 0; p < B_PASS; ++p) {
        const int oys = s_oy[p] * a.stride, oxs = s_ox[p] * a.stride;
        const bool ok = (unsigned)(oys + u_bdy) < (unsigned)a.hi && (unsigned)(oxs + u_bx) < (unsigned)a.wi;
        unsigned voff;
        if (a.up) {
          const int w2 = a.wi >> 1;
          const unsigned s_off = (unsigned)((s_ni[p] * (a.hi >> 1) * w2 + (oxs >> 1)) * a.ci) * 4u;
          voff = u_bc + s_off + (unsigned)(((oys + u_bdy) >> 1) * w2 * a.ci) * 4u;
        } else {
          const unsigned s_off = (unsigned)(((s_ni[p] * a.hi + oys) * a.wi + oxs) * a.ci) * 4u;
          voff = u_bc + s_off;
        }
        voff = ok ? voff : 0x80000000u;
        rb[p] = __builtin_bit_cast(f32x4, __builtin_amdgcn_raw_buffer_load_b128(rsrc_x, (int)voff, 0, 0));
        s_ox[p] += WBK;
        while (s_ox[p] >= a.wo) {
          s_ox[p] -= a.wo;
          if (++s_oy[p] == a.ho) {
            s_oy[p] = 0;
            ++s_ni[p];
          }
        }
      }
      return;
    }
    const int mb = kbeg + kt * WBK;
#pragma unroll
    for (int p = 0; p < A_PASS; ++p) {
      const int m = mb + arow + A_ROWS * p;
      f32x4 v = {0.f, 0.f, 0.f, 0.f};
      if (a_ok && m < kend) v = *reinterpret_cast<const f32x4*>(static_cast<const float*>(a.dy) + (size_t)m * a.co + a_co);
      ra[p] = v;
    }
#pragma unroll
    for (int p = 0; p < B_PASS; ++p) {
      const int m = mb + brow + B_ROWS * p;
      f32x4 v = {0.f, 0.f, 0.f, 0.f};
      if (b_ok && m < kend) {
        const int t1 = fast_div(m, a.wo, a.inv_wo);
        const int ox = m - t1 * a.wo;
        const int ni = fast_div(t1, a.ho, a.inv_ho);
        const int oy = t1 - ni * a.ho;
        const int iy = oy * a.stride + b_dy, ix = ox * a.stride + b_dx;
        if ((unsigned)iy < (unsigned)a.hi && (unsigned)ix < (unsigned)a.wi) {
          const size_t pix = a.up ? (size_t)(ni * (a.hi >> 1) + (iy >> 1)) * (a.wi >> 1) + (ix >> 1) : (size_t)(ni * a.hi + iy) * a.wi + ix;
          v = *reinterpret_cast<const f32x4*>(static_cast<const float*>(a.x) + pix * (size_t)a.ci + b_c);
        }
      }
      rb[p] = v;
    }
  };
  auto store_tile = [&](int buf) {
#pragma unroll
    for (int p = 0; p < A_PASS; ++p) *reinterpret_cast<f32x4*>(&As[buf][arow + A_ROWS * p][aq * 4]) = ra[p];
#pragma unroll
    for (int p = 0; p < B_PASS; ++p) *reinterpret_cast<f32x4*>(&Bs[buf][brow + B_ROWS * p][bq * 4]) = rb[p];
  };

  if (nkt > 0) {
    load_tile(0);
    store_tile(0);
  }
  __syncthreads();
  int cur = 0;
  for (int kt = 0; kt < nkt; ++kt) {
    const bool more = (kt + 1) < nkt;
    if (more) load_tile(kt + 1);
#pragma unroll
    for (int k2 = 0; k2 < WBK / 2; ++k2) {
      float af[TM], bf[TN];
#pragma unroll
      for (int i = 0; i < TM; ++i) af[i] = As[cur][2 * k2 + lh][wm + i * 32 + lr];
#pragma unroll
      for (int jn = 0; jn < TN; ++jn) bf[jn] = Bs[cur][2 * k2 + lh][wn + jn * 32 + lr];
#pragma unroll
      for (int i = 0; i < TM; ++i)
#pragma unroll
        for (int jn = 0; jn < TN; ++jn)
          acc[i][jn] = __builtin_amdgcn_mfma_f32_32x32x2f32(af[i], bf[jn], acc[i][jn], 0, 0, 0);
    }
    if (more) store_tile(cur ^ 1);
    __syncthreads();
    cur ^= 1;
  }

  int col[TN];
#pragma unroll
  for (int jn = 0; jn < TN; ++jn) {
    const int jj = j0 + wn + jn * 32 + lr;
    const int tap = fast_div(jj, a.ci, a.inv_ci);
    col[jn] = jj < a.J ? tap * a.ci_full + a.c_off + (jj - tap * a.ci) : -1;
  }
#pragma unroll
  for (int i = 0; i < TM; ++i)
#pragma unroll
    for (int v = 0; v < 16; ++v) {
      const int co = co0 + wm + i * 32 + (v & 3) + 8 * (v >> 2) + 4 * lh;
      if (co >= a.co) continue;
#pragma unroll
      for (int jn = 0; jn < TN; ++jn) {
        if (col[jn] >= 0) {
          float* dst = a.dw + (size_t)co * a.J_ld + col[jn];
          if (a.use_atomic) atomicAdd(dst, acc[i][jn][v]);
          else *dst = acc[i][jn][v];
        }
      }
    }
}

typedef short s16x4 __attribute__((ext_vector_type(4)));
typedef short s16x8 __attribute__((ext_vector_type(8)));
typedef __bf16 bf16x8w __attribute__((ext_vector_type(8)));
constexpr int WBKB = 64;

__device__ __forceinline__ bf16x8w tr_fragment(const unsigned short* row0, int ld) {
  const s16x4 lo = __builtin_amdgcn_ds_read_tr16_b64_v4i16((s16x4 __attribute__((address_space(3)))*)(row0));
  const s16x4 hi = __builtin_amdgcn_ds_read_tr16_b64_v4i16((s16x4 __attribute__((address_space(3)))*)(row0 + 4 * ld));
  const s16x8 f = __builtin_shufflevector(lo, hi, 0, 1, 2, 3, 4, 5, 6, 7);
  return __builtin_bit_cast(bf16x8w, f);
}

template <int BMW, int BNW, int WAVES_M, int WAVES_N, bool ROWU>
__global__ __launch_bounds__(256) void conv_wgrad_bf16_kernel(const WgradArgs a) {
  constexpr int WM = BMW / WAVES_M, WN = BNW / WAVES_N;
  constexpr int TM = WM / 32, TN = WN / 32;
  constexpr int LDA = BMW + 8, LDB = BNW + 8;
  constexpr int AQ = BMW / 8, BQ = BNW / 8;
  constexpr int A_ROWS = 256 / AQ, B_ROWS = 256 / BQ;
  constexpr int A_PASS = (WBKB + A_ROWS - 1) / A_ROWS, B_PASS = (WBKB + B_ROWS - 1) / B_ROWS;
  static_assert(WAVES_M * WAVES_N == 4, "4 waves");

  __shared__ __attribute__((aligned(16))) unsigned short As[2][WBKB][LDA];
  __shared__ __attribute__((aligned(16))) unsigned short Bs[2][WBKB][LDB];
  const unsigned short* xg = reinterpret_cast<const unsigned short*>(a.x);
  const unsigned short* dyg = reinterpret_cast<const unsigned short*>(a.dy);

  const int tid = threadIdx.x, lane = tid & 63, wave = tid >> 6;
  const int lr = lane & 31, lh = lane >> 5;
  const int wm = (wave / WAVES_N) * WM, wn = (wave % WAVES_N) * WN;
  const int grp = lane >> 4, cb = 16 * (grp & 1), hk = grp >> 1, tq = (lane & 15) >> 2, tp = lane & 3;

  const int ntj = (a.J + BNW - 1) / BNW;
  int tile_id = blockIdx.x, split_id = blockIdx.y;
  if (a.xcd_tiles > 0) {
    const int L = blockIdx.x, xcd = L & 7, idx = L >> 3;
    split_id = xcd + 8 * (idx / a.xcd_tiles);
    tile_id = idx % a.xcd_tiles;
  }
  const int co0 = (tile_id / ntj) * BMW;
  const int j0 = (tile_id % ntj) * BNW;
  const int kbeg = split_id * a.kchunk;
  const int kend = min(a.M, kbeg + a.kchunk);
  if (kbeg >= a.M) return;

  const int aq = tid % AQ, arow = tid / AQ;
  const int a_co = co0 + aq * 8;
  const bool a_ok = a_co < a.co;
  const int bq = tid % BQ, brow = tid / BQ;
  const int j = j0 + bq * 8;
  const bool b_ok = j < a.J;
  int b_dy = 0, b_dx = 0, b_c = 0;
  if (b_ok) {
    const int tap = fast_div(j, a.ci, a.inv_ci);
    b_c = j - tap * a.ci;
    const int r = fast_div(tap, a.kw, a.inv_kw);
    b_dy = r - a.pad;
    b_dx = (tap - r * a.kw) - a.pad;
  }

  f32x16 acc[TM][TN];
#pragma unroll
  for (int i = 0; i < TM; ++i)
#pragma unroll
    for (int jn = 0; jn < TN; ++jn)
#pragma unroll
      for (int v = 0; v < 16; ++v) acc[i][jn][v] = 0.f;

  f32x4 ra[A_PASS], rb[B_PASS];
  const int nkt = (kend - kbeg + WBKB - 1) / WBKB;
  const bool xform = a.in_scale != nullptr;
  const bool x_relu = a.in_act == UDASEG_ACT_LEAKY && a.in_slope == 0.f;
  float x_sc[8], x_sh[8];
  unsigned x_ok = 0;
  if (xform) {
#pragma unroll
    for (int e = 0; e < 8; ++e) {
      x_sc[e] = b_ok ? a.in_scale[b_c + e] : 0.f;
      x_sh[e] = b_ok ? a.in_shift[b_c + e] : 0.f;
    }
  }

  static_assert(!ROWU || (WBKB % A_ROWS == 0 && WBKB % B_ROWS == 0), "row-uniform passes must tile the K-tile");
  unsigned u_ac[A_PASS], u_bc = 0;
  int u_bdy = 0, u_bx = 0;
  int s_ni[B_PASS], s_oy[B_PASS], s_ox[B_PASS];
  unsigned s_dyoff = 0;
  __amdgpu_buffer_rsrc_t rsrc_x, rsrc_dy;
  if constexpr (ROWU) {
    rsrc_x = __builtin_amdgcn_make_buffer_rsrc(const_cast<void*>(a.x), 0, (int)a.x_bytes, 0x00020000);
    rsrc_dy = __builtin_amdgcn_make_buffer_rsrc(const_cast<void*>(a.dy), 0, (int)a.dy_bytes, 0x00020000);
#pragma unroll
    for (int p = 0; p < A_PASS; ++p)
      u_ac[p] = a_ok ? (unsigned)((arow + A_ROWS * p) * a.co + a_co) * 2u : 0x80000000u;
    u_bdy = b_dy;
    u_bx = brow * a.stride + b_dx;
    u_bc = !b_ok ? 0x80000000u
                 : a.up ? (unsigned)((u_bx >> 1) * a.ci + b_c) * 2u
                        : (unsigned)((b_dy * a.wi + brow * a.stride + b_dx) * a.ci + b_c) * 2u;
    s_dyoff = (unsigned)kbeg * (unsigned)a.co * 2u;
#pragma unroll
    for (int p = 0; p < B_PASS; ++p) {
      const int m = kbeg + B_ROWS * p;
      const int t1 = m / a.wo;
      s_ox[p] = m - t1 * a.wo;
      s_ni[p] = t1 / a.ho;
      s_oy[p] = t1 - s_ni[p] * a.ho;
    }
  }

  auto load_tile = [&](int kt) {
    if constexpr (ROWU) {
#pragma unroll
      for (int p = 0; p < A_PASS; ++p)
        ra[p] = __builtin_bit_cast(f32x4, __builtin_amdgcn_raw_buffer_load_b128(rsrc_dy, (int)(u_ac[p] + s_dyoff), 0, 0));
      s_dyoff += (unsigned)(WBKB * 2) * (unsigned)a.co;
#pragma unroll
      for (int p = 0; p < B_PASS; ++p) {
        const int oys = s_oy[p] * a.stride, oxs = s_ox[p] * a.stride;
        const bool ok = (unsigned)(oys + u_bdy) < (unsigned)a.hi && (unsigned)(oxs + u_bx) < (unsigned)a.wi;
        unsigned voff;
        if (a.up) {
          const int w2 = a.wi >> 1;
          const unsigned s_off = (unsigned)((s_ni[p] * (a.hi >> 1) * w2 + (oxs >> 1)) * a.ci) * 2u;
          voff = u_bc + s_off + (unsigned)(((oys + u_bdy) >> 1) * w2 * a.ci) * 2u;
        } else {
          const unsigned s_off = (unsigned)(((s_ni[p] * a.hi + oys) * a.wi + oxs) * a.ci) * 2u;
          voff = u_bc + s_off;
        }
        voff = ok ? voff : 0x80000000u;
        x_ok = (x_ok & ~(1u << p)) | ((ok && b_ok ? 1u : 0u) << p);
        rb[p] = __builtin_bit_cast(f32x4, __builtin_amdgcn_raw_buffer_load_b128(rsrc_x, (int)voff, 0, 0));
        s_ox[p] += WBKB;
        while (s_ox[p] >= a.wo) {
          s_ox[p] -= a.wo;
          if (++s_oy[p] == a.ho) {
            s_oy[p] = 0;
            ++s_ni[p];
          }
        }
      }
      return;
    }
    const int mb = kbeg + kt * WBKB;
#pragma unroll
    for (int p = 0; p < A_PASS; ++p) {
      const int row = arow + A_ROWS * p, m = mb + row;
      f32x4 v = {0.f, 0.f, 0.f, 0.f};
      if (a_ok && row < WBKB && m < kend) v = *reinterpret_cast<const f32x4*>(dyg + (size_t)m * a.co + a_co);
      ra[p] = v;
    }
#pragma unroll
    for (int p = 0; p < B_PASS; ++p) {
      const int row = brow + B_ROWS * p, m = mb + row;
      f32x4 v = {0.f, 0.f, 0.f, 0.f};
      bool inside = false;
      if (b_ok && row < WBKB && m < kend) {
        const int t1 = fast_div(m, a.wo, a.inv_wo);
        const int ox = m - t1 * a.wo;
        const int ni = fast_div(t1, a.ho, a.inv_ho);
        const int oy = t1 - ni * a.ho;
        const int iy = oy * a.stride + b_dy, ix = ox * a.stride + b_dx;
        if ((unsigned)iy < (unsigned)a.hi && (unsigned)ix < (unsigned)a.wi) {
          const size_t pix = a.up ? (size_t)(ni * (a.hi >> 1) + (iy >> 1)) * (a.wi >> 1) + (ix >> 1) : (size_t)(ni * a.hi + iy) * a.wi + ix;
          v = *reinterpret_cast<const f32x4*>(xg + pix * (size_t)a.ci + b_c);
          inside = true;
        }
      }
      x_ok = (x_ok & ~(1u << p)) | ((inside ? 1u : 0u) << p);
      rb[p] = v;
    }
  };
  auto store_tile = [&](int buf) {
#pragma unroll
    for (int p = 0; p < A_PASS; ++p)
      if (arow + A_ROWS * p < WBKB) *reinterpret_cast<f32x4*>(&As[buf][arow + A_ROWS * p][aq * 8]) = ra[p];
    if (xform) {
#pragma unroll
      for (int p = 0; p < B_PASS; ++p) {
        typedef unsigned u32x4w __attribute__((ext_vector_type(4)));
        const u32x4w wv = __builtin_bit_cast(u32x4w, rb[p]);
        u32x4w dv;
        const bool ok = (x_ok >> p) & 1u;
#pragma unroll
        for (int e = 0; e < 4; ++e) {
          const unsigned w = wv[e];
          float t0 = __builtin_fmaf(__builtin_bit_cast(float, w << 16), x_sc[2 * e], x_sh[2 * e]);
          float t1 = __builtin_fmaf(__builtin_bit_cast(float, w & 0xffff0000u), x_sc[2 * e + 1], x_sh[2 * e + 1]);
          if (x_relu) {
            t0 = t0 > 0.f ? t0 : 0.f;
            t1 = t1 > 0.f ? t1 : 0.f;
          } else {
            t0 = act_apply(t0, a.in_act, a.in_slope);
            t1 = act_apply(t1, a.in_act, a.in_slope);
          }
          dv[e] = ok ? ((unsigned)__builtin_bit_cast(unsigned short, (__bf16)t0) | ((unsigned)__builtin_bit_cast(unsigned short, (__bf16)t1) << 16))
                     : 0u;
        }
        rb[p] = __builtin_bit_cast(f32x4, dv);
      }
    }
#pragma unroll
    for (int p = 0; p < B_PASS; ++p)
      if (brow + B_ROWS * p < WBKB) *reinterpret_cast<f32x4*>(&Bs[buf][brow + B_ROWS * p][bq * 8]) = rb[p];
  };

  if (nkt > 0) {
    load_tile(0);
    store_tile(0);
  }
  __syncthreads();
  int cur = 0;
  for (int kt = 0; kt < nkt; ++kt) {
    const bool more = (kt + 1) < nkt;
    if (more) load_tile(kt + 1);
#pragma unroll
    for (int ks = 0; ks < WBKB / 16; ++ks) {
      bf16x8w af[TM], bfr[TN];
#pragma unroll
      for (int i = 0; i < TM; ++i) af[i] = tr_fragment(&As[cur][16 * ks + 8 * hk + tq][wm + 32 * i + cb + 4 * tp], LDA);
#pragma unroll
      for (int jn = 0; jn < TN; ++jn) bfr[jn] = tr_fragment(&Bs[cur][16 * ks + 8 * hk + tq][wn + 32 * jn + cb + 4 * tp], LDB);
#pragma unroll
      for (int i = 0; i < TM; ++i)
#pragma unroll
        for (int jn = 0; jn < TN; ++jn)
          acc[i][jn] = __builtin_amdgcn_mfma_f32_32x32x16_bf16(af[i], bfr[jn], acc[i][jn], 0, 0, 0);
    }
    if (more) store_tile(cur ^ 1);
    __syncthreads();
    cur ^= 1;
  }

  int col[TN];
#pragma unroll
  for (int jn = 0; jn < TN; ++jn) {
    const int jj = j0 + wn + jn * 32 + lr;
    const int tap = fast_div(jj, a.ci, a.inv_ci);
    col[jn] = jj < a.J ? tap * a.ci_full + a.c_off + (jj - tap * a.ci) : -1;
  }
#pragma unroll
  for (int i = 0; i < TM; ++i)
#pragma unroll
    for (int v = 0; v < 16; ++v) {
      const int co = co0 + wm + i * 32 + (v & 3) + 8 * (v >> 2) + 4 * lh;
      if (co >= a.co) continue;
#pragma unroll
      for (int jn = 0; jn < TN; ++jn) {
        if (col[jn] >= 0) {
          float* dst = a.dw + (size_t)co * a.J_ld + col[jn];
          if (a.use_atomic) atomicAdd(dst, acc[i][jn][v]);
          else *dst = acc[i][jn][v];
        }
      }
    }
}

constexpr int WBKX = 32;

template <int BMW, int BNW, int WAVES_M, int WAVES_N, bool ROWU>
__global__ __launch_bounds__(256) void conv_wgrad_x3_kernel(const WgradArgs a) {
  constexpr int WM = BMW / WAVES_M, WN = BNW / WAVES_N;
  constexpr int TM = WM / 32, TN = WN / 32;
  constexpr int LDA = BMW + 8, LDB = BNW + 8;
  constexpr int AQ = BMW / 8, BQ = BNW / 8;
  constexpr int A_ROWS = 256 / AQ, B_ROWS = 256 / BQ;
  constexpr int A_PASS = (WBKX + A_ROWS - 1) / A_ROWS, B_PASS = (WBKX + B_ROWS - 1) / B_ROWS;
  static_assert(WAVES_M * WAVES_N == 4, "4 waves");
  static_assert(!ROWU || (WBKX % A_ROWS == 0 && WBKX % B_ROWS == 0), "row-uniform passes must tile the K-tile");

  __shared__ __attribute__((aligned(16))) unsigned short As[3][2][WBKX][LDA];
  __shared__ __attribute__((aligned(16))) unsigned short Bs[3][2][WBKX][LDB];
  const float* xg = reinterpret_cast<const float*>(a.x);
  const float* dyg = reinterpret_cast<const float*>(a.dy);

  const int tid = threadIdx.x, lane = tid & 63, wave = tid >> 6;
  const int lr = lane & 31, lh = lane >> 5;
  const int wm = (wave / WAVES_N) * WM, wn = (wave % WAVES_N) * WN;
  const int grp = lane >> 4, cb = 16 * (grp & 1), hk = grp >> 1, tq = (lane & 15) >> 2, tp = lane & 3;

  const int ntj = (a.J + BNW - 1) / BNW;
  const int co0 = (blockIdx.x / ntj) * BMW;
  const int j0 = (blockIdx.x % ntj) * BNW;
  const int kbeg = blockIdx.y * a.kchunk;
  const int kend = min(a.M, kbeg + a.kchunk);
  if (kbeg >= a.M) return;

  const int aq = tid % AQ, arow = tid / AQ;
  const int a_co = co0 + aq * 8;
  const bool a_ok = a_co < a.co;
  const int bq = tid % BQ, brow = tid / BQ;
  const int j = j0 + bq * 8;
  const bool b_ok = j < a.J;
  int b_dy = 0, b_dx = 0, b_c = 0;
  if (b_ok) {
    const int tap = fast_div(j, a.ci, a.inv_ci);
    b_c = j - tap * a.ci;
    const int r = fast_div(tap, a.kw, a.inv_kw);
    b_dy = r - a.pad;
    b_dx = (tap - r * a.kw) - a.pad;
  }
  const bool b_two = (a.ci & 7) != 0;
  int b2_dy = 0, b2_dx = 0, b2_c = 0;
  const bool b2_ok = b_two && (j + 4) < a.J;
  if (b2_ok) {
    const int tap = fast_div(j + 4, a.ci, a.inv_ci);
    b2_c = (j + 4) - tap * a.ci;
    const int r = fast_div(tap, a.kw, a.inv_kw);
    b2_dy = r - a.pad;
    b2_dx = (tap - r * a.kw) - a.pad;
  }

  f32x16 acc[TM][TN];
#pragma unroll
  for (int i = 0; i < TM; ++i)
#pragma unroll
    for (int jn = 0; jn < TN; ++jn)
#pragma unroll
      for (int v = 0; v < 16; ++v) acc[i][jn][v] = 0.f;

  f32x16 acc2[TM][TN];
#pragma unroll
  for (int i = 0; i < TM; ++i)
#pragma unroll
    for (int jn = 0; jn < TN; ++jn)
#pragma unroll
      for (int v = 0; v < 16; ++v) acc2[i][jn][v] = 0.f;

  u32x4 ra[A_PASS][2], rb[B_PASS][2];
  const int nkt = (kend - kbeg + WBKX - 1) / WBKX;

  unsigned u_ac[A_PASS], u_bc = 0;
  int u_bdy = 0, u_bx = 0;
  int s_ni[B_PASS], s_oy[B_PASS], s_ox[B_PASS];
  unsigned s_dyoff = 0;
  __amdgpu_buffer_rsrc_t rsrc_x, rsrc_dy;
  if constexpr (ROWU) {
    rsrc_x = __builtin_amdgcn_make_buffer_rsrc(const_cast<void*>(a.x), 0, (int)a.x_bytes, 0x00020000);
    rsrc_dy = __builtin_amdgcn_make_buffer_rsrc(const_cast<void*>(a.dy), 0, (int)a.dy_bytes, 0x00020000);
#pragma unroll
    for (int p = 0; p < A_PASS; ++p)
      u_ac[p] = a_ok ? (unsigned)((arow + A_ROWS * p) * a.co + a_co) * 4u : 0x80000000u;
    u_bdy = b_dy;
    u_bx = brow * a.stride + b_dx;
    u_bc = !b_ok ? 0x80000000u
                 : a.up ? (unsigned)((u_bx >> 1) * a.ci + b_c) * 4u
                        : (unsigned)((b_dy * a.wi + brow * a.stride + b_dx) * a.ci + b_c) * 4u;
    s_dyoff = (unsigned)kbeg * (unsigned)a.co * 4u;
#pragma unroll
    for (int p = 0; p < B_PASS; ++p) {
      const int m = kbeg + B_ROWS * p;
      const int t1 = m / a.wo;
      s_ox[p] = m - t1 * a.wo;
      s_ni[p] = t1 / a.ho;
      s_oy[p] = t1 - s_ni[p] * a.ho;
    }
  }

  const u32x4 zero4 = {0u, 0u, 0u, 0u};
  auto load_tile = [&](int kt) {
    if constexpr (ROWU) {
#pragma unroll
      for (int p = 0; p < A_PASS; ++p) {
        ra[p][0] = __builtin_amdgcn_raw_buffer_load_b128(rsrc_dy, (int)(u_ac[p] + s_dyoff), 0, 0);
        ra[p][1] = __builtin_amdgcn_raw_buffer_load_b128(rsrc_dy, (int)(u_ac[p] + s_dyoff), 16, 0);
      }
      s_dyoff += (unsigned)(WBKX * 4) * (unsigned)a.co;
#pragma unroll
      for (int p = 0; p < B_PASS; ++p) {
        const int oys = s_oy[p] * a.stride, oxs = s_ox[p] * a.stride;
        const bool ok = (unsigned)(oys + u_bdy) < (unsigned)a.hi && (unsigned)(oxs + u_bx) < (unsigned)a.wi;
        unsigned voff;
        if (a.up) {
          const int w2 = a.wi >> 1;
          const unsigned s_off = (unsigned)((s_ni[p] * (a.hi >> 1) * w2 + (oxs >> 1)) * a.ci) * 4u;
          voff = u_bc + s_off + (unsigned)(((oys + u_bdy) >> 1) * w2 * a.ci) * 4u;
        } else {
          const unsigned s_off = (unsigned)(((s_ni[p] * a.hi + oys) * a.wi + oxs) * a.ci) * 4u;
          voff = u_bc + s_off;
        }
        voff = ok ? voff : 0x80000000u;
        rb[p][0] = __builtin_amdgcn_raw_buffer_load_b128(rsrc_x, (int)voff, 0, 0);
        rb[p][1] = __builtin_amdgcn_raw_buffer_load_b128(rsrc_x, (int)voff, 16, 0);
        s_ox[p] += WBKX;
        while (s_ox[p] >= a.wo) {
          s_ox[p] -= a.wo;
          if (++s_oy[p] == a.ho) {
            s_oy[p] = 0;
            ++s_ni[p];
          }
        }
      }
      return;
    }
    const int mb = kbeg + kt * WBKX;
#pragma unroll
    for (int p = 0; p < A_PASS; ++p) {
      const int row = arow + A_ROWS * p, m = mb + row;
      u32x4 v0 = zero4, v1 = zero4;
      if (a_ok && row < WBKX && m < kend) {
        const u32x4* src = reinterpret_cast<const u32x4*>(dyg + (size_t)m * a.co + a_co);
        v0 = src[0];
        if (a_co + 4 < a.co) v1 = src[1];
      }
      ra[p][0] = v0;
      ra[p][1] = v1;
    }
#pragma unroll
    for (int p = 0; p < B_PASS; ++p) {
      const int row = brow + B_ROWS * p, m = mb + row;
      u32x4 v0 = zero4, v1 = zero4;
      if (b_ok && row < WBKX && m < kend) {
        const int t1 = fast_div(m, a.wo, a.inv_wo);
        const int ox = m - t1 * a.wo;
        const int ni = fast_div(t1, a.ho, a.inv_ho);
        const int oy = t1 - ni * a.ho;
        {
          const int iy = oy * a.stride + b_dy, ix = ox * a.stride + b_dx;
          if ((unsigned)iy < (unsigned)a.hi && (unsigned)ix < (unsigned)a.wi) {
            const size_t pix = a.up ? (size_t)(ni * (a.hi >> 1) + (iy >> 1)) * (a.wi >> 1) + (ix >> 1) : (size_t)(ni * a.hi + iy) * a.wi + ix;
            const u32x4* src = reinterpret_cast<const u32x4*>(xg + pix * (size_t)a.ci + b_c);
            v0 = src[0];
            if (!b_two && j + 4 < a.J) v1 = src[1];
          }
        }
        if (b2_ok) {
          const int iy = oy * a.stride + b2_dy, ix = ox * a.stride + b2_dx;
          if ((unsigned)iy < (unsigned)a.hi && (unsigned)ix < (unsigned)a.wi) {
            const size_t pix = a.up ? (size_t)(ni * (a.hi >> 1) + (iy >> 1)) * (a.wi >> 1) + (ix >> 1) : (size_t)(ni * a.hi + iy) * a.wi + ix;
            v1 = *reinterpret_cast<const u32x4*>(xg + pix * (size_t)a.ci + b2_c);
          }
        }
      }
      rb[p][0] = v0;
      rb[p][1] = v1;
    }
  };
  auto store_tile = [&](auto BUF) {
    constexpr int buf = decltype(BUF)::value;
#pragma unroll
    for (int p = 0; p < A_PASS; ++p)
      if (arow + A_ROWS * p < WBKX) {
        u32x4 p0, p1, p2;
        split3(ra[p][0], ra[p][1], p0, p1, p2);
        if constexpr (buf != 0) {
          p0 ^= 0x80008000u;
          p1 ^= 0x80008000u;
          p2 ^= 0x80008000u;
        }
        *reinterpret_cast<u32x4*>(&As[0][buf][arow + A_ROWS * p][aq * 8]) = p0;
        *reinterpret_cast<u32x4*>(&As[1][buf][arow + A_ROWS * p][aq * 8]) = p1;
        *reinterpret_cast<u32x4*>(&As[2][buf][arow + A_ROWS * p][aq * 8]) = p2;
      }
#pragma unroll
    for (int p = 0; p < B_PASS; ++p)
      if (brow + B_ROWS * p < WBKX) {
        u32x4 p0, p1, p2;
        split3(rb[p][0], rb[p][1], p0, p1, p2);
        *reinterpret_cast<u32x4*>(&Bs[0][buf][brow + B_ROWS * p][bq * 8]) = p0;
        *reinterpret_cast<u32x4*>(&Bs[1][buf][brow + B_ROWS * p][bq * 8]) = p1;
        *reinterpret_cast<u32x4*>(&Bs[2][buf][brow + B_ROWS * p][bq * 8]) = p2;
      }
  };
  auto step = [&](auto CUR, int kt) {
    constexpr int cur = decltype(CUR)::value;
    const bool more = (kt + 1) < nkt;
    if (more) load_tile(kt + 1);
#pragma unroll
    for (int ks = 0; ks < WBKX / 16; ++ks) {
      bf16x8w af[3][TM], bfr[3][TN];
#pragma unroll
      for (int pl = 0; pl < 3; ++pl) {
#pragma unroll
        for (int i = 0; i < TM; ++i) af[pl][i] = tr_fragment(&As[pl][cur][16 * ks + 8 * hk + tq][wm + 32 * i + cb + 4 * tp], LDA);
#pragma unroll
        for (int jn = 0; jn < TN; ++jn) bfr[pl][jn] = tr_fragment(&Bs[pl][cur][16 * ks + 8 * hk + tq][wn + 32 * jn + cb + 4 * tp], LDB);
      }
#pragma unroll
      for (int pq = 2; pq >= 0; --pq)
#pragma unroll
        for (int pa = 0; pa <= pq; ++pa)
#pragma unroll
          for (int i = 0; i < TM; ++i)
#pragma unroll
            for (int jn = 0; jn < TN; ++jn) {
              if constexpr (cur != 0)
                acc2[i][jn] = __builtin_amdgcn_mfma_f32_32x32x16_bf16(af[pa][i], bfr[pq - pa][jn], acc2[i][jn], 0, 0, 0);
              else
                acc[i][jn] = __builtin_amdgcn_mfma_f32_32x32x16_bf16(af[pa][i], bfr[pq - pa][jn], acc[i][jn], 0, 0, 0);
            }
    }
    if (more) store_tile(std::integral_constant<int, cur ^ 1>{});
    __syncthreads();
  };

  if (nkt > 0) {
    load_tile(0);
    store_tile(std::integral_constant<int, 0>{});
  }
  __syncthreads();
  for (int kt = 0; kt < nkt; kt += 2) {
    step(std::integral_constant<int, 0>{}, kt);
    if (kt + 1 < nkt) step(std::integral_constant<int, 1>{}, kt + 1);
  }

#pragma unroll
  for (int i = 0; i < TM; ++i)
#pragma unroll
    for (int jn = 0; jn < TN; ++jn) acc[i][jn] -= acc2[i][jn];
  int col[TN];
#pragma unroll
  for (int jn = 0; jn < TN; ++jn) {
    const int jj = j0 + wn + jn * 32 + lr;
    const int tap = fast_div(jj, a.ci, a.inv_ci);
    col[jn] = jj < a.J ? tap * a.ci_full + a.c_off + (jj - tap * a.ci) : -1;
  }
#pragma unroll
  for (int i = 0; i < TM; ++i)
#pragma unroll
    for (int v = 0; v < 16; ++v) {
      const int co = co0 + wm + i * 32 + (v & 3) + 8 * (v >> 2) + 4 * lh;
      if (co >= a.co) continue;
#pragma unroll
      for (int jn = 0; jn < TN; ++jn) {
        if (col[jn] >= 0) {
          float* dst = a.dw + (size_t)co * a.J_ld + col[jn];
          if (a.use_atomic) atomicAdd(dst, acc[i][jn][v]);
          else *dst = acc[i][jn][v];
        }
      }
    }
}

template <int BMW, int BNW, int WAVES_M, int WAVES_N>
static int launch_wgrad_x3(WgradArgs a, int accumulate, hipStream_t s) {
  const int tiles = cdiv(a.co, BMW) * cdiv(a.J, BNW);
  int target = opt_get(UDASEG_OPT_WGRAD_X3_BLOCKS);
  if (target < 64) target = 1024;
  int splits = cdiv(target, tiles);
  const int max_splits = cdiv(a.M, 256);
  if (splits > max_splits) splits = max_splits;
  if (splits < 1) splits = 1;
  if (splits > 65535) splits = 65535;
  const int kchunk = cdiv(cdiv(a.M, splits), WBKX) * WBKX;
  splits = cdiv(a.M, kchunk);
  a.kchunk = kchunk;
  a.use_atomic = (splits > 1 || accumulate) ? 1 : 0;
  if (a.use_atomic && !accumulate) {
    if (a.J != a.J_ld) {
      set_error("conv2d_wgrad_part: a channel slice of dW must be accumulated onto a caller-zeroed gradient");
      return UDASEG_E_BADARG;
    }
    hipError_t e = hipMemsetAsync(a.dw, 0, (size_t)a.co * a.J * sizeof(float), s);
    if (e != hipSuccess) return hip_fail(e, "hipMemsetAsync(dw)");
  }
  dim3 grid((unsigned)tiles, (unsigned)splits), block(256);
  a.xcd_tiles = a.xcd_splits = 0;
  constexpr int b_rows = 256 / (BNW / 8);
  const long long xb = (long long)a.M / (a.ho * a.wo) * (a.up ? (a.hi >> 1) * (a.wi >> 1) : a.hi * a.wi) * a.ci * 4,
                  dyb = (long long)a.M * a.co * 4;
  a.row_uniform = !opt_get(UDASEG_OPT_WGRAD_GENERIC) && a.wo % b_rows == 0 && a.ci % 8 == 0 && a.co % 8 == 0 &&
                  xb <= (1LL << 30) && dyb <= (1LL << 30);
  a.x_bytes = (unsigned)xb;
  a.dy_bytes = (unsigned)dyb;
  hipEvent_t ev = kprof_begin(s);
  if (a.row_uniform)
    hipLaunchKernelGGL((conv_wgrad_x3_kernel<BMW, BNW, WAVES_M, WAVES_N, true>), grid, block, 0, s, a);
  else
    hipLaunchKernelGGL((conv_wgrad_x3_kernel<BMW, BNW, WAVES_M, WAVES_N, false>), grid, block, 0, s, a);
  static std::atomic<int> kidx[2] = {{-1}, {-1}};
  std::atomic<int>& kid = kidx[a.row_uniform ? 1 : 0];
  if (kid < 0) {
    char nm[96];
    snprintf(nm, sizeof(nm), "conv_wgrad_x3_kernel<%d, %d, %d, %d, %s>", BMW, BNW, WAVES_M, WAVES_N, a.row_uniform ? "true" : "false");
    kid = kprof_id(nm);
  }
  kprof_end(kid, ev, s, 2.0 * (double)a.M * a.co * a.J);
  UDASEG_LAUNCH_CHECK("conv_wgrad_x3 launch");
  return UDASEG_OK;
}

template <int BMW, int BNW, int WAVES_M, int WAVES_N>
static int launch_wgrad(WgradArgs a, int accumulate, hipStream_t s, bool bf16 = false) {
  const int tiles = cdiv(a.co, BMW) * cdiv(a.J, BNW);
  int target = opt_get(UDASEG_OPT_WGRAD_BLOCKS);
  const bool target_from_env = target >= 64;
  if (!target_from_env) target = 3072;
  const int bf16_target = (BMW == 32 && a.M >= (1 << 20)) ? 2048 : 512;
  int splits = cdiv(bf16 && !target_from_env ? bf16_target : target, tiles);
  const int max_splits = cdiv(a.M, 256);
  if (splits > max_splits) splits = max_splits;
  if (splits < 1) splits = 1;
  const int ktile = bf16 ? WBKB : WBK;
  int kchunk = cdiv(cdiv(a.M, splits), ktile) * ktile;
  splits = cdiv(a.M, kchunk);
  if (bf16 && splits >= 16 && tiles > 1 && splits % 8 != 0) {
    const int s8 = ((splits + 4) / 8) * 8;
    const int kc = cdiv(cdiv(a.M, s8), ktile) * ktile;
    if ((long long)kc * (s8 - 8) < a.M) {
      kchunk = kc;
      splits = s8;
    }
  }
  a.kchunk = kchunk;
  a.use_atomic = (splits > 1 || accumulate) ? 1 : 0;
  if (a.use_atomic && !accumulate) {
    if (a.J != a.J_ld) {
      set_error("conv2d_wgrad_part: a channel slice of dW must be accumulated onto a caller-zeroed gradient");
      return UDASEG_E_BADARG;
    }
    hipError_t e = hipMemsetAsync(a.dw, 0, (size_t)a.co * a.J * sizeof(float), s);
    if (e != hipSuccess) return hip_fail(e, "hipMemsetAsync(dw)");
  }
  dim3 grid((unsigned)tiles, (unsigned)splits), block(256);
  a.xcd_tiles = a.xcd_splits = 0;
  if (bf16 && splits % 8 == 0 && tiles > 1) {
    if (!opt_get(UDASEG_OPT_WGRAD_NO_XCD)) {
      a.xcd_tiles = tiles;
      a.xcd_splits = splits;
      grid = dim3((unsigned)(tiles * splits), 1u);
    }
  }
  hipEvent_t ev = kprof_begin(s);
  if (bf16) {
    constexpr int b_rows16 = 256 / (BNW / 8);
    const long long xb16 = (long long)a.M / (a.ho * a.wo) * (a.up ? (a.hi >> 1) * (a.wi >> 1) : a.hi * a.wi) * a.ci * 2,
                    dyb16 = (long long)a.M * a.co * 2;
    a.row_uniform = !opt_get(UDASEG_OPT_WGRAD_GENERIC) && a.wo % b_rows16 == 0 && xb16 <= (1LL << 30) && dyb16 <= (1LL << 30);
    a.x_bytes = (unsigned)xb16;
    a.dy_bytes = (unsigned)dyb16;
    if (a.row_uniform)
      hipLaunchKernelGGL((conv_wgrad_bf16_kernel<BMW, BNW, WAVES_M, WAVES_N, true>), grid, block, 0, s, a);
    else
      hipLaunchKernelGGL((conv_wgrad_bf16_kernel<BMW, BNW, WAVES_M, WAVES_N, false>), grid, block, 0, s, a);
    static std::atomic<int> kid16[2] = {{-1}, {-1}};
    std::atomic<int>& kid = kid16[a.row_uniform ? 1 : 0];
    if (kid < 0) {
      char nm[96];
      snprintf(nm, sizeof(nm), "conv_wgrad_bf16_kernel<%d, %d, %d, %d, %s>", BMW, BNW, WAVES_M, WAVES_N, a.row_uniform ? "true" : "false");
      kid = kprof_id(nm);
    }
    kprof_end(kid, ev, s, 2.0 * (double)a.M * a.co * a.J);
  } else {
    constexpr int b_rows = 256 / (BNW / 4);
    const long long xb = (long long)a.M / (a.ho * a.wo) * (a.up ? (a.hi >> 1) * (a.wi >> 1) : a.hi * a.wi) * a.ci * 4,
                    dyb = (long long)a.M * a.co * 4;
    a.row_uniform = !opt_get(UDASEG_OPT_WGRAD_GENERIC) && a.wo % b_rows == 0 && xb <= (1LL << 30) && dyb <= (1LL << 30);
    a.x_bytes = (unsigned)xb;
    a.dy_bytes = (unsigned)dyb;
    if (a.row_uniform)
      hipLaunchKernelGGL((conv_wgrad_kernel<BMW, BNW, WAVES_M, WAVES_N, true>), grid, block, 0, s, a);
    else
      hipLaunchKernelGGL((conv_wgrad_kernel<BMW, BNW, WAVES_M, WAVES_N, false>), grid, block, 0, s, a);
    int kid32 = (a.row_uniform ? 18 : 7) + (BMW == 64 ? 0 : 1);
    if (BMW == 128) {
      static std::atomic<int> kid128[2] = {{-1}, {-1}};
      std::atomic<int>& k = kid128[a.row_uniform ? 1 : 0];
      if (k < 0) {
        char nm[96];
        snprintf(nm, sizeof(nm), "conv_wgrad_kernel<%d, %d, %d, %d, %s>", BMW, BNW, WAVES_M, WAVES_N, a.row_uniform ? "true" : "false");
        k = kprof_id(nm);
      }
      kid32 = k;
    }
    kprof_end(kid32, ev, s, 2.0 * (double)a.M * a.co * a.J);
  }
  UDASEG_LAUNCH_CHECK("conv_wgrad launch");
  return UDASEG_OK;
}


}

using namespace udaseg;

static bool wgrad_x3_on() {
  return udaseg::opt_get(UDASEG_OPT_WGRAD_X3) != 0 && udaseg::f32_split_enabled();
}

static int conv2d_wgrad_impl(const udaseg_conv_desc* d, const void* x, int src_c, int c_off, int up, const void* dy, float* dw,
                             int accumulate, void* stream, int bf16, const float* in_scale = nullptr, const float* in_shift = nullptr,
                             int in_act = UDASEG_ACT_NONE, float in_slope = 0.f) {
  UDASEG_CHECK_ARG(d && x && dy && dw, "conv2d_wgrad: NULL pointer");
  const int g = bf16 ? 8 : 4;
  UDASEG_CHECK_ARG(d->ci % g == 0 && d->co % g == 0 && d->ci > 0 && d->co > 0, "conv2d_wgrad: channels must be multiples of %d", g);
  UDASEG_CHECK_ARG(d->kh > 0 && d->kw > 0 && d->stride >= 1 && d->pad >= 0, "conv2d_wgrad: bad kernel/stride");
  UDASEG_CHECK_ARG(d->n > 0 && d->hi > 0 && d->wi > 0 && d->ho > 0 && d->wo > 0, "conv2d_wgrad: non-positive extent");
  UDASEG_CHECK_ARG(d->ho == (d->hi + 2 * d->pad - d->kh) / d->stride + 1 && d->wo == (d->wi + 2 * d->pad - d->kw) / d->stride + 1,
                   "conv2d_wgrad: output extent %dx%d inconsistent with input %dx%d k%d s%d p%d", d->ho, d->wo, d->hi, d->wi,
                   d->kh, d->stride, d->pad);
  UDASEG_CHECK_ARG((long long)d->n * d->hi * d->wi * d->ci < (1LL << 31) && (long long)d->n * d->ho * d->wo * d->co < (1LL << 31),
                   "conv2d_wgrad: tensor exceeds 2^31 elements");
  UDASEG_CHECK_ARG(src_c > 0 && src_c % g == 0 && c_off >= 0 && c_off % g == 0 && c_off + src_c <= d->ci,
                   "conv2d_wgrad_part: channel slice [%d, %d) of %d", c_off, c_off + src_c, d->ci);
  UDASEG_CHECK_ARG(!up || (d->stride == 1 && d->hi % 2 == 0 && d->wi % 2 == 0), "conv2d_wgrad_part: an up-sampled source needs stride 1 and even extents");
  const bool whole = src_c == d->ci;
  UDASEG_CHECK_ARG(whole || accumulate, "conv2d_wgrad_part: a channel slice of dW must be accumulated onto a caller-zeroed gradient");
  WgradArgs a = {};
  a.x = x; a.dy = dy; a.dw = dw;
  a.hi = d->hi; a.wi = d->wi; a.ci = src_c; a.ho = d->ho; a.wo = d->wo; a.co = d->co;
  a.kw = d->kw; a.stride = d->stride; a.pad = d->pad;
  a.M = d->n * d->ho * d->wo;
  a.J = d->kh * d->kw * src_c;
  a.ci_full = d->ci; a.c_off = c_off; a.J_ld = d->kh * d->kw * d->ci; a.up = up;
  a.in_scale = in_scale; a.in_shift = in_shift; a.in_act = in_act; a.in_slope = in_slope;
  a.inv_ci = 1.0f / src_c; a.inv_kw = 1.0f / d->kw; a.inv_wo = 1.0f / d->wo; a.inv_ho = 1.0f / d->ho;
  if (d->kh == 1 && d->kw == 1 && d->stride == 1 && d->pad == 0 && !up) {
    a.hi = 1; a.wi = a.M; a.ho = 1; a.wo = a.M;
    a.inv_wo = 1.0f / (float)a.M; a.inv_ho = 1.0f;
  }
  hipStream_t st = as_stream(stream);
  prof_begin(1, st);
  int rc;
  udaseg_conv_desc dp = *d;
  dp.ci = src_c;
  if (bf16)
    rc = d->co >= 128 ? launch_wgrad<128, 64, 2, 2>(a, accumulate, st, true)
       : d->co > 32   ? launch_wgrad<64, 64, 2, 2>(a, accumulate, st, true)
                      : launch_wgrad<32, 128, 1, 4>(a, accumulate, st, true);
  else if (whole && d->kh == d->kw &&
           small_wgrad_applicable(d->kh, d->stride, d->pad, d->ci, d->co, d->n * cdiv(d->hi, 16) * cdiv(d->wi, 16)))
    rc = launch_small_wgrad(static_cast<const float*>(x), static_cast<const float*>(dy), dw, d->n, d->hi, d->wi, d->ci, d->co,
                            accumulate, st, up);
  else if (d->co > 32 && src_c % 8 == 0 && d->co % 8 == 0 && wgrad_x3_on()) rc = launch_wgrad_x3<64, 64, 2, 2>(a, accumulate, st);
  else if (d->co > 32) rc = launch_wgrad<64, 64, 2, 2>(a, accumulate, st);
  else rc = launch_wgrad<32, 128, 1, 4>(a, accumulate, st);
  prof_end(1, st, udaseg_conv_flops(&dp), 2, &dp);
  return rc;
}

extern "C" int udaseg_conv2d_wgrad(const udaseg_conv_desc* d, const float* x, const float* dy, float* dw,
                                   int accumulate, void* stream) {
  UDASEG_CHECK_ARG(d != nullptr, "conv2d_wgrad: NULL desc");
  return conv2d_wgrad_impl(d, x, d->ci, 0, 0, dy, dw, accumulate, stream, 0);
}

extern "C" int udaseg_conv2d_wgrad_bf16(const udaseg_conv_desc* d, const void* x, const void* dy, float* dw, int accumulate,
                                        void* stream) {
  UDASEG_CHECK_ARG(d != nullptr, "conv2d_wgrad_bf16: NULL desc");
  return conv2d_wgrad_impl(d, x, d->ci, 0, 0, dy, dw, accumulate, stream, 1);
}

extern "C" int udaseg_conv2d_wgrad_bnin_bf16(const udaseg_conv_desc* d, const void* x, const float* in_scale, const float* in_shift,
                                             int in_act, float in_slope, const void* dy, float* dw, int accumulate, void* stream) {
  UDASEG_CHECK_ARG(d != nullptr && in_scale != nullptr && in_shift != nullptr, "conv2d_wgrad_bnin_bf16: NULL desc / scale / shift");
  return conv2d_wgrad_impl(d, x, d->ci, 0, 0, dy, dw, accumulate, stream, 1, in_scale, in_shift, in_act, in_slope);
}

namespace udaseg {
bool wgrad_h2_applicable(const udaseg_conv_desc* d, int up_ca, bool f32);
int launch_wgrad_h2(const udaseg_conv_desc* d, const void* x, const void* x2, int up_ca, const void* dy, float* dw, bool f32, hipStream_t s,
                    const float* in_scale = nullptr, const float* in_shift = nullptr, int in_act = 0, float in_slope = 0.f,
                    int ldw = 0, int dw_coff = 0);
static bool wgrad_halo_off(bool f32) {
  const bool off = opt_get(UDASEG_OPT_NO_WGRAD_HALO) != 0;
  return f32 ? (off || !f32_halo_enabled()) : off;
}
}

extern "C" int udaseg_conv2d_wgrad_bnin_ok(const udaseg_conv_desc* d, int up) {
  if (!d || d->kh != 3 || d->kw != 3 || d->stride != 1 || d->pad != 1 || d->n <= 0 || d->hi <= 0 || d->wi <= 0 || d->ci % 8 != 0 ||
      d->co % 4 != 0)
    return 0;
  if (small_wgrad_applicable(d->kh, d->stride, d->pad, d->ci, d->co, d->n * cdiv(d->hi, 16) * cdiv(d->wi, 16))) return 1;
  return !up && !wgrad_halo_off(true) && wgrad_h2_applicable(d, 0, true) ? 1 : 0;
}

extern "C" int udaseg_conv2d_wgrad_bnin(const udaseg_conv_desc* d, const float* x, int up, const float* in_scale, const float* in_shift,
                                        int in_act, float in_slope, const float* dy, float* dw, int accumulate, void* stream) {
  UDASEG_CHECK_ARG(d && x && in_scale && in_shift && dy && dw, "conv2d_wgrad_bnin: NULL pointer");
  UDASEG_CHECK_ARG(in_act == UDASEG_ACT_NONE || in_act == UDASEG_ACT_LEAKY, "conv2d_wgrad_bnin: unknown activation %d", in_act);
  UDASEG_CHECK_ARG(d->ho == d->hi && d->wo == d->wi, "conv2d_wgrad_bnin: stride-1 'same' convolutions only");
  UDASEG_CHECK_ARG(!up || (d->hi % 2 == 0 && d->wi % 2 == 0), "conv2d_wgrad_bnin: an up-sampled source needs even extents");
  if (!udaseg_conv2d_wgrad_bnin_ok(d, up)) {
    set_error("conv2d_wgrad_bnin: geometry not supported (ask udaseg_conv2d_wgrad_bnin_ok)");
    return UDASEG_E_UNSUPPORTED;
  }
  hipStream_t st = as_stream(stream);
  const bool small = small_wgrad_applicable(d->kh, d->stride, d->pad, d->ci, d->co, d->n * cdiv(d->hi, 16) * cdiv(d->wi, 16));
  if (!small && !accumulate) {
    hipError_t e = hipMemsetAsync(dw, 0, (size_t)d->co * 9 * d->ci * sizeof(float), st);
    if (e != hipSuccess) return hip_fail(e, "hipMemsetAsync(dw)");
  }
  prof_begin(1, st);
  int rc;
  if (small) {
    rc = launch_small_wgrad(x, dy, dw, d->n, d->hi, d->wi, d->ci, d->co, accumulate, st, up, in_scale, in_shift, in_act, in_slope);
  } else {
    rc = launch_wgrad_h2(d, x, nullptr, 0, dy, dw, true, st, in_scale, in_shift, in_act, in_slope);
  }
  prof_end(1, st, udaseg_conv_flops(d), 2, d);
  return rc;
}

extern "C" int udaseg_conv2d_wgrad_halo_bf16_ok(const udaseg_conv_desc* d, int up_ca) {
  return d != nullptr && !wgrad_halo_off(false) && wgrad_h2_applicable(d, up_ca, false) ? 1 : 0;
}

extern "C" int udaseg_conv2d_wgrad_halo_bf16(const udaseg_conv_desc* d, const void* x, const void* skip, int up_ca, const void* dy,
                                             float* dw, void* stream) {
  UDASEG_CHECK_ARG(d && x && dy && dw, "conv2d_wgrad_halo_bf16: NULL pointer");
  UDASEG_CHECK_ARG(d->n > 0 && d->hi > 0 && d->wi > 0 && d->ho == d->hi && d->wo == d->wi, "conv2d_wgrad_halo_bf16: bad extents");
  UDASEG_CHECK_ARG(up_ca == 0 ? skip == nullptr : skip != nullptr, "conv2d_wgrad_halo_bf16: up_ca and skip come together");
  if (!udaseg_conv2d_wgrad_halo_bf16_ok(d, up_ca)) {
    set_error("conv2d_wgrad_halo_bf16: geometry not supported (ask udaseg_conv2d_wgrad_halo_bf16_ok first)");
    return UDASEG_E_UNSUPPORTED;
  }
  hipStream_t st = as_stream(stream);
  prof_begin(1, st);
  const int rc = launch_wgrad_h2(d, x, skip, up_ca, dy, dw, false, st);
  prof_end(1, st, udaseg_conv_flops(d), 2, d);
  return rc;
}

extern "C" int udaseg_conv2d_wgrad_halo_f32x3_ok(const udaseg_conv_desc* d, int up_ca) {
  return d != nullptr && !wgrad_halo_off(true) && wgrad_h2_applicable(d, up_ca, true) ? 1 : 0;
}

extern "C" int udaseg_conv2d_wgrad_halo_f32x3(const udaseg_conv_desc* d, const float* x, const float* skip, int up_ca, const float* dy,
                                              float* dw, void* stream) {
  UDASEG_CHECK_ARG(d && x && dy && dw, "conv2d_wgrad_halo_f32x3: NULL pointer");
  UDASEG_CHECK_ARG(d->n > 0 && d->hi > 0 && d->wi > 0 && d->ho == d->hi && d->wo == d->wi, "conv2d_wgrad_halo_f32x3: bad extents");
  UDASEG_CHECK_ARG((up_ca > 0) == (skip != nullptr), "conv2d_wgrad_halo_f32x3: up_ca=%d, skip %s", up_ca, skip ? "given" : "NULL");
  if (!udaseg_conv2d_wgrad_halo_f32x3_ok(d, up_ca)) {
    set_error("conv2d_wgrad_halo_f32x3: geometry not supported (ask udaseg_conv2d_wgrad_halo_f32x3_ok first)");
    return UDASEG_E_UNSUPPORTED;
  }
  hipStream_t st = as_stream(stream);
  prof_begin(1, st);
  const int rc = launch_wgrad_h2(d, x, skip, up_ca, dy, dw, true, st);
  prof_end(1, st, udaseg_conv_flops(d), 2, d);
  return rc;
}

extern "C" int udaseg_conv2d_wgrad_halo_slice_f32x3(const udaseg_conv_desc* d, const float* x, const float* dy, float* dw, int ldw,
                                                    int c_off, void* stream) {
  UDASEG_CHECK_ARG(d && x && dy && dw, "conv2d_wgrad_halo_slice_f32x3: NULL pointer");
  UDASEG_CHECK_ARG(d->n > 0 && d->hi > 0 && d->wi > 0 && d->ho == d->hi && d->wo == d->wi, "conv2d_wgrad_halo_slice_f32x3: bad extents");
  UDASEG_CHECK_ARG(ldw >= d->ci && c_off >= 0 && c_off + d->ci <= ldw && c_off % 4 == 0 && ldw % 4 == 0,
                   "conv2d_wgrad_halo_slice_f32x3: slice [%d, %d) of rows of %d channels", c_off, c_off + d->ci, ldw);
  if (!udaseg_conv2d_wgrad_halo_f32x3_ok(d, 0)) {
    set_error("conv2d_wgrad_halo_slice_f32x3: geometry not supported (ask udaseg_conv2d_wgrad_halo_f32x3_ok on the slice's descriptor)");
    return UDASEG_E_UNSUPPORTED;
  }
  hipStream_t st = as_stream(stream);
  prof_begin(1, st);
  const int rc = launch_wgrad_h2(d, x, nullptr, 0, dy, dw, true, st, nullptr, nullptr, 0, 0.f, ldw, c_off);
  prof_end(1, st, udaseg_conv_flops(d), 2, d);
  return rc;
}

extern "C" int udaseg_conv2d_wgrad_part(const udaseg_conv_desc* d, const float* src, int src_c, int c_off, int up,
                                        const float* dy, float* dw, int accumulate, void* stream) {
  UDASEG_CHECK_ARG(d != nullptr, "conv2d_wgrad_part: NULL desc");
  return conv2d_wgrad_impl(d, src, src_c, c_off, up, dy, dw, accumulate, stream, 0);
}

extern "C" int udaseg_conv2d_wgrad_part_bf16(const udaseg_conv_desc* d, const void* src, int src_c, int c_off, int up,
                                             const void* dy, float* dw, int accumulate, void* stream) {
  UDASEG_CHECK_ARG(d != nullptr, "conv2d_wgrad_part_bf16: NULL desc");
  return conv2d_wgrad_impl(d, src, src_c, c_off, up, dy, dw, accumulate, stream, 1);
}

namespace udaseg {
__global__ void pack_dgrad_kernel(const float* __restrict__ w, float* __restrict__ wt, int co, int T, int ci) {
  const long long total = (long long)co * T * ci;
  for (long long i = blockIdx.x * (long long)blockDim.x + threadIdx.x; i < total; i += (long long)gridDim.x * blockDim.x) {
    const int o = (int)(i % co);
    const long long r = i / co;
    const int t = (int)(r % T);
    const int c = (int)(r / T);
    wt[i] = w[((long long)o * T + t) * ci + c];
  }
}
}

namespace udaseg {
__global__ void pack_dgrad_batched_kernel(const float* __restrict__ arena, float* __restrict__ packed,
                                          const int* __restrict__ table) {
  const int* e = table + 5 * blockIdx.y;
  const float* w = arena + e[0];
  float* wt = packed + e[1];
  if ((e[2] | e[4]) & 3) {
    const int co = e[2], T = e[3], ci = e[4];
    const int total = co * T * ci;
    for (int i = blockIdx.x * blockDim.x + threadIdx.x; i < total; i += gridDim.x * blockDim.x) {
      const int o = i % co;
      const int r = i / co;
      const int t = r % T;
      const int c = r / T;
      wt[i] = w[(o * T + t) * ci + c];
    }
    return;
  }
  pack_dgrad_tiles<float>(w, wt, e[2], e[3], e[4]);
}
}

extern "C" int udaseg_pack_dgrad_batched(const float* arena, float* packed, const int* table, int entries, void* stream) {
  UDASEG_CHECK_ARG(arena && packed && table && entries > 0, "pack_dgrad_batched: bad arguments");
  hipLaunchKernelGGL(pack_dgrad_batched_kernel, dim3(PACK_DGRAD_GRID_X, entries), dim3(256), 0, as_stream(stream), arena, packed, table);
  UDASEG_LAUNCH_CHECK("pack_dgrad_batched launch");
  return UDASEG_OK;
}

extern "C" int udaseg_pack_dgrad_weights(const udaseg_conv_desc* d, const float* w, float* w_t, void* stream) {
  UDASEG_CHECK_ARG(d && w && w_t, "pack_dgrad_weights: NULL pointer");
  const long long total = (long long)d->co * d->kh * d->kw * d->ci;
  const int blocks = (int)((total + 255) / 256 > 2048 ? 2048 : (total + 255) / 256);
  hipLaunchKernelGGL(pack_dgrad_kernel, dim3(blocks), dim3(256), 0, as_stream(stream), w, w_t, d->co, d->kh * d->kw, d->ci);
  UDASEG_LAUNCH_CHECK("pack_dgrad launch");
  return UDASEG_OK;
}
```

Baseline: 1106.

## Add MFMA split-bf16 weight-gradient kernels for stem and narrow 3x3 convs

Adds dedicated persistent weight-gradient kernels for the 7x7 stride-2 stem conv and for 3x3 convs with 32 or fewer channels. They stage inputs and output gradients in LDS as three bf16 split planes and accumulate with bf16 MFMA. Partial results are reduced in LDS and then added atomically into dw. Both paths are on by default through new options, replacing the previous generic weight-gradient kernels for these shapes. The change also centralises device CU-count and LDS-capacity queries, at the cost of more code, atomics and a higher LDS footprint.

```diff
diff --git a/include/udaseg.h b/include/udaseg.h
--- a/include/udaseg.h
+++ b/include/udaseg.h
@@ -51,7 +51,9 @@
 #define UDASEG_OPT_HALO_S2_CK 30
 #define UDASEG_OPT_UP_CFG 31
 #define UDASEG_OPT_WGRAD_UP_BLOCKS 32
-#define UDASEG_OPT_COUNT 33
+#define UDASEG_OPT_STEM_WGRAD 33
+#define UDASEG_OPT_N16_WGRAD 34
+#define UDASEG_OPT_COUNT 35
 int udaseg_set_option(int key, int value);
 int udaseg_get_option(int key);
 int udaseg_option_count(void);
diff --git a/uda_aerial_semantic_segmentation_research_amd/_lib.py b/uda_aerial_semantic_segmentation_research_amd/_lib.py
--- a/uda_aerial_semantic_segmentation_research_amd/_lib.py
+++ b/uda_aerial_semantic_segmentation_research_amd/_lib.py
@@ -168,7 +168,7 @@
     "udaseg_prof_records": (_I, [_I, _I, C.POINTER(C.c_double), C.POINTER(C.c_double), C.POINTER(C.c_int), C.POINTER(C.c_int)]),
 }
 
-OPTIONS = {"GENERIC_GATHER": 0, "F32_SPLIT": 1, "WGRAD_GENERIC": 2, "F32_HALO": 3, "F3_CFG": 4, "F3_WS": 5, "F3_SIGNS": 6, "IGEMM_TILE": 7, "IGEMM_X3": 8, "NO_FOLD": 9, "WGRAD_X3_BLOCKS": 10, "WGRAD_BLOCKS": 11, "WGRAD_NO_XCD": 12, "WGRAD_X3": 13, "NO_WGRAD_HALO": 14, "WGRAD_F3_BLOCKS": 15, "WGRAD_HALO_BLOCKS": 16, "WGRAD_DEEP_BLOCKS": 17, "WGRAD_DB": 18, "REDUCE_BLOCKS": 19, "BN_APPLY_PT": 20, "GEMM_1X1_TILE": 21, "GEMM_1X1": 22, "GEMM_1X1_MAXM": 23, "NO_STREAM": 24, "HALO_CFG": 25, "NO_HALO": 26, "NO_HALO_S2": 27, "HALO_W16": 28, "HALO_DEEP": 29, "HALO_S2_CK": 30, "UP_CFG": 31, "WGRAD_UP_BLOCKS": 32}
+OPTIONS = {"GENERIC_GATHER": 0, "F32_SPLIT": 1, "WGRAD_GENERIC": 2, "F32_HALO": 3, "F3_CFG": 4, "F3_WS": 5, "F3_SIGNS": 6, "IGEMM_TILE": 7, "IGEMM_X3": 8, "NO_FOLD": 9, "WGRAD_X3_BLOCKS": 10, "WGRAD_BLOCKS": 11, "WGRAD_NO_XCD": 12, "WGRAD_X3": 13, "NO_WGRAD_HALO": 14, "WGRAD_F3_BLOCKS": 15, "WGRAD_HALO_BLOCKS": 16, "WGRAD_DEEP_BLOCKS": 17, "WGRAD_DB": 18, "REDUCE_BLOCKS": 19, "BN_APPLY_PT": 20, "GEMM_1X1_TILE": 21, "GEMM_1X1": 22, "GEMM_1X1_MAXM": 23, "NO_STREAM": 24, "HALO_CFG": 25, "NO_HALO": 26, "NO_HALO_S2": 27, "HALO_W16": 28, "HALO_DEEP": 29, "HALO_S2_CK": 30, "UP_CFG": 31, "WGRAD_UP_BLOCKS": 32, "STEM_WGRAD": 33, "N16_WGRAD": 34}
 
 _lib = None
 
diff --git a/uda_aerial_semantic_segmentation_research_amd/csrc/api.hip b/uda_aerial_semantic_segmentation_research_amd/csrc/api.hip
--- a/uda_aerial_semantic_segmentation_research_amd/csrc/api.hip
+++ b/uda_aerial_semantic_segmentation_research_amd/csrc/api.hip
@@ -226,6 +226,34 @@
     ++n;
   }
   return n;
+}
+
+namespace udaseg {
+constexpr int PROP_DEVICES = 16;
+static std::atomic<int> g_dev_cus[PROP_DEVICES];
+static std::atomic<long long> g_dev_lds[PROP_DEVICES];
+static void dev_props(int dev) {
+  hipDeviceProp_t pr;
+  if (hipGetDeviceProperties(&pr, dev) == hipSuccess) {
+    g_dev_cus[dev] = pr.multiProcessorCount > 0 ? pr.multiProcessorCount : 256;
+    g_dev_lds[dev] = (long long)pr.sharedMemPerBlockOptin;
+  } else {
+    g_dev_cus[dev] = 256;
+    g_dev_lds[dev] = -1;
+  }
+}
+int device_cu_count() {
+  int dev = 0;
+  if (hipGetDevice(&dev) != hipSuccess || dev < 0 || dev >= PROP_DEVICES) return 256;
+  if (g_dev_cus[dev].load() == 0) dev_props(dev);
+  return g_dev_cus[dev].load();
+}
+bool device_lds_fits(int bytes) {
+  int dev = 0;
+  if (hipGetDevice(&dev) != hipSuccess || dev < 0 || dev >= PROP_DEVICES) return false;
+  if (g_dev_lds[dev].load() == 0) dev_props(dev);
+  return g_dev_lds[dev].load() >= (long long)bytes;
+}
 }
 
 namespace udaseg {
@@ -267,7 +295,9 @@
      {"UDASEG_HALO_DEEP", K_OFF0, 1},
      {"UDASEG_HALO_S2_CK", K_INT, 64},
      {"UDASEG_UP_CFG", K_INT, 0},
-     {"UDASEG_WGRAD_UP_BLOCKS", K_INT, 0}};
+     {"UDASEG_WGRAD_UP_BLOCKS", K_INT, 0},
+     {"UDASEG_STEM_WGRAD", K_INT, 1},
+     {"UDASEG_N16_WGRAD", K_INT, 1}};
 int g_opt_val[UDASEG_OPT_COUNT];
 static int g_opt_default[UDASEG_OPT_COUNT];
 std::atomic<bool> g_opt_ready{false};
diff --git a/uda_aerial_semantic_segmentation_research_amd/csrc/common.h b/uda_aerial_semantic_segmentation_research_amd/csrc/common.h
--- a/uda_aerial_semantic_segmentation_research_amd/csrc/common.h
+++ b/uda_aerial_semantic_segmentation_research_amd/csrc/common.h
@@ -187,6 +187,9 @@
                        hipStream_t s, int up = 0, const float* in_scale = nullptr, const float* in_shift = nullptr,
                        int in_act = 0, float in_slope = 0.f);
 
+int device_cu_count();
+bool device_lds_fits(int bytes);
+
 constexpr int PROF_NKERNELS = 24;
 int kprof_id(const char* rocprof_symbol);
 hipEvent_t kprof_begin(hipStream_t s);
diff --git a/uda_aerial_semantic_segmentation_research_amd/csrc/conv_n16_f32x3.hip b/uda_aerial_semantic_segmentation_research_amd/csrc/conv_n16_f32x3.hip
--- a/uda_aerial_semantic_segmentation_research_amd/csrc/conv_n16_f32x3.hip
+++ b/uda_aerial_semantic_segmentation_research_amd/csrc/conv_n16_f32x3.hip
@@ -290,7 +290,7 @@
   const int gathered = dgrad ? d->co : d->ci, produced = dgrad ? d->ci : d->co;
   if (produced != 16 || gathered % 8 != 0 || gathered < 8 || gathered > 32 || d->n <= 0 || d->hi <= 0 || d->wi < 16) return false;
   const long long px = (long long)d->n * d->hi * d->wi;
-  return px * 32 * 4 < (1LL << 31);
+  return px * 32 * 4 < (1LL << 31) && device_lds_fits(N16Cfg::LDS_HALO + ((gathered + 15) / 16) * N16Cfg::WCHUNK);
 }
 
 static int launch_n16(N16Args a, hipStream_t s, double flops) {
@@ -308,13 +308,7 @@
   const long long ntiles = (long long)a.n * a.nty * a.ntx;
   if (ntiles <= 0) return UDASEG_OK;
   if (ntiles >= (1LL << 31)) return UDASEG_E_UNSUPPORTED;
-  static int cus = 0;
-  if (cus == 0) {
-    int dev = 0;
-    hipDeviceProp_t pr;
-    cus = (hipGetDevice(&dev) == hipSuccess && hipGetDeviceProperties(&pr, dev) == hipSuccess && pr.multiProcessorCount > 0)
-              ? pr.multiProcessorCount : 256;
-  }
+  const int cus = device_cu_count();
   const long long resident = (long long)cus * (a.nk16 == 1 ? 3 : 2);
   const long long blocks = ntiles < resident ? ntiles : resident;
   a.sscr = nullptr;
diff --git a/uda_aerial_semantic_segmentation_research_amd/csrc/conv_stem_f32x3.hip b/uda_aerial_semantic_segmentation_research_amd/csrc/conv_stem_f32x3.hip
--- a/uda_aerial_semantic_segmentation_research_amd/csrc/conv_stem_f32x3.hip
+++ b/uda_aerial_semantic_segmentation_research_amd/csrc/conv_stem_f32x3.hip
@@ -193,12 +193,253 @@
   }
 }
 
+struct StemWgradArgs {
+  const float* x;
+  const float* dy;
+  float* dw;
+  int n, h, w;
+  int ntx, nty, ntiles;
+  int signs;
+  unsigned x_bytes, dy_bytes;
+};
+
+struct StemWgradCfg {
+  static constexpr int NT = 256, NW = 4;
+  static constexpr int TH = 4, TW = 32, TP = TH * TW;
+  static constexpr int IR = 2 * TH + 5, NP = StemCfg::NP, ROWB = StemCfg::ROWB, PLANE = IR * ROWB;
+  static constexpr int LDS_BAND = 3 * PLANE;
+  static constexpr int NPIECE = IR * NP;
+  static constexpr int NI = (NPIECE + NT - 1) / NT;
+  static constexpr int DSP = TP * 64 + 64;
+  static constexpr int DPLANE = 2 * DSP;
+  static constexpr int ND = TP * 8 / NT;
+  static constexpr int LDS = LDS_BAND + 3 * DPLANE;
+  static constexpr int RED = 2 * 7 * 16 * 64 * 4;
+  static_assert(TP * 8 % NT == 0 && RED <= LDS && LDS <= 160 * 1024, "stem wgrad tiling");
+  static_assert(LDS_BAND % 16 == 0 && DSP % 128 == 64, "stem wgrad LDS layout");
+};
+
+typedef short stem_s16x4 __attribute__((ext_vector_type(4)));
+typedef short stem_s16x8 __attribute__((ext_vector_type(8)));
+template <int PITCH>
+__device__ __forceinline__ bf16x8 stem_tr_fragment(const char* p) {
+  const stem_s16x4 lo = __builtin_amdgcn_ds_read_tr16_b64_v4i16((stem_s16x4 __attribute__((address_space(3)))*)(p));
+  const stem_s16x4 hi = __builtin_amdgcn_ds_read_tr16_b64_v4i16((stem_s16x4 __attribute__((address_space(3)))*)(p + 4 * PITCH));
+  return __builtin_bit_cast(bf16x8, __builtin_shufflevector(lo, hi, 0, 1, 2, 3, 4, 5, 6, 7));
+}
+
+__global__ __launch_bounds__(256, 2) void conv_stem_f32x3_kernel_wgrad(const StemWgradArgs a) {
+  using C = StemWgradCfg;
+  extern __shared__ __attribute__((aligned(16))) char smem[];
+  char* const band = smem;
+  char* const dys = smem + C::LDS_BAND;
+  const int tid = threadIdx.x, lane = tid & 63;
+  const int wave = __builtin_amdgcn_readfirstlane(tid >> 6);
+  const int half = wave & 1, rw = wave >> 1;
+  const int H = a.h, W = a.w, HO = a.h >> 1, WO = a.w >> 1;
+  const int P = gridDim.x;
+
+  unsigned xoff[C::NI][2], doff[C::ND];
+  auto tile_setup = [&](int tl) {
+    const int tx = tl % a.ntx;
+    const int t2 = tl / a.ntx;
+    const int ty = t2 % a.nty, img = t2 / a.nty;
+    const int y0 = ty * C::TH, x0 = tx * C::TW;
+#pragma unroll
+    for (int i = 0; i < C::NI; ++i) {
+      const int piece = tid + i * C::NT;
+      const int r = piece / C::NP, q = piece - r * C::NP;
+      const int iy = 2 * y0 - 3 + r, ix = 2 * x0 - 3 + 2 * q;
+      const bool rok = piece < C::NPIECE && (unsigned)iy < (unsigned)H;
+#pragma unroll
+      for (int e = 0; e < 2; ++e)
+        xoff[i][e] = (rok && (unsigned)(ix + e) < (unsigned)W) ? (unsigned)(((img * H + iy) * W + ix + e) * 16) : 0x80000000u;
+    }
+#pragma unroll
+    for (int i = 0; i < C::ND; ++i) {
+      const int pc = tid + i * C::NT;
+      const int pix = pc >> 3, oct = pc & 7;
+      const int oy = y0 + pix / C::TW, ox = x0 + pix % C::TW;
+      doff[i] = (oy < HO && ox < WO) ? (unsigned)((((img * HO + oy) * WO + ox) * 64 + oct * 8) * 4) : 0x80000000u;
+    }
+  };
+  __amdgpu_buffer_rsrc_t rs_x = __builtin_amdgcn_make_buffer_rsrc(const_cast<float*>(a.x), 0, (int)a.x_bytes, 0x00020000);
+  __amdgpu_buffer_rsrc_t rs_d = __builtin_amdgcn_make_buffer_rsrc(const_cast<float*>(a.dy), 0, (int)a.dy_bytes, 0x00020000);
+  u32x4 sx[C::NI][2], sd[C::ND][2];
+  auto load_tile = [&]() {
+#pragma unroll
+    for (int i = 0; i < C::NI; ++i) {
+      sx[i][0] = __builtin_amdgcn_raw_buffer_load_b128(rs_x, (int)xoff[i][0], 0, 0);
+      sx[i][1] = __builtin_amdgcn_raw_buffer_load_b128(rs_x, (int)xoff[i][1], 0, 0);
+    }
+#pragma unroll
+    for (int i = 0; i < C::ND; ++i) {
+      sd[i][0] = __builtin_amdgcn_raw_buffer_load_b128(rs_d, (int)doff[i], 0, 0);
+      sd[i][1] = __builtin_amdgcn_raw_buffer_load_b128(rs_d, (int)doff[i], 16, 0);
+    }
+  };
+  auto store_tile = [&](unsigned dsgn) {
+#pragma unroll
+    for (int i = 0; i < C::NI; ++i) {
+      const int piece = tid + i * C::NT;
+      if (i < C::NI - 1 || piece < C::NPIECE) {
+        u32x4 p0, p1, p2;
+        split3(sx[i][0], sx[i][1], p0, p1, p2);
+        *reinterpret_cast<u32x4*>(band + piece * 16) = p0;
+        *reinterpret_cast<u32x4*>(band + C::PLANE + piece * 16) = p1;
+        *reinterpret_cast<u32x4*>(band + 2 * C::PLANE + piece * 16) = p2;
+      }
+    }
+#pragma unroll
+    for (int i = 0; i < C::ND; ++i) {
+      const int pc = tid + i * C::NT;
+      const int pix = pc >> 3, oct = pc & 7;
+      char* const dst = dys + (oct >> 2) * C::DSP + pix * 64 + (oct & 3) * 16;
+      u32x4 p0, p1, p2;
+      split3(sd[i][0] ^ dsgn, sd[i][1] ^ dsgn, p0, p1, p2);
+      *reinterpret_cast<u32x4*>(dst) = p0;
+      *reinterpret_cast<u32x4*>(dst + C::DPLANE) = p1;
+      *reinterpret_cast<u32x4*>(dst + 2 * C::DPLANE) = p2;
+    }
+  };
+
+  f32x16 acc[7];
+#pragma unroll
+  for (int ky = 0; ky < 7; ++ky)
+#pragma unroll
+    for (int v = 0; v < 16; ++v) acc[ky][v] = 0.f;
+
+  const int grp = lane >> 4, tq = (lane & 15) >> 2, tp = lane & 3;
+  const int el = 16 * (grp & 1) + 4 * tp, px = 8 * (grp >> 1) + tq;
+  const char* const dbase = dys + half * C::DSP + (2 * rw * C::TW + px) * 64 + el * 2;
+  const char* const xbase = band + (4 * rw) * C::ROWB + px * 16 + el * 2;
+
+  const int nseq = (a.ntiles - (int)blockIdx.x + P - 1) / P;
+  const int sq1 = a.signs ? (nseq + 2) / 4 : 0, sq3 = a.signs ? nseq - sq1 : 0;
+  bool negated = false;
+  int tile = blockIdx.x, seq = 0;
+  if (tile < a.ntiles) {
+    tile_setup(tile);
+    load_tile();
+  }
+  for (; tile < a.ntiles; tile += P, ++seq) {
+    const bool neg = seq >= sq1 && seq < sq3;
+    if (neg != negated) {
+      negated = neg;
+#pragma unroll
+      for (int ky = 0; ky < 7; ++ky) acc[ky] = -acc[ky];
+    }
+    store_tile(neg ? 0x80000000u : 0u);
+    __syncthreads();
+    if (tile + P < a.ntiles) {
+      tile_setup(tile + P);
+      load_tile();
+    }
+#pragma unroll 1
+    for (int ks = 0; ks < 4; ++ks) {
+        const int r = ks >> 1, s16 = ks & 1;
+        bf16x8 A[3];
+#pragma unroll
+        for (int pl = 0; pl < 3; ++pl) A[pl] = stem_tr_fragment<64>(dbase + pl * C::DPLANE + (r * C::TW + 16 * s16) * 64);
+#pragma unroll
+        for (int ky = 0; ky < 7; ++ky) {
+          bf16x8 B[3];
+#pragma unroll
+          for (int pl = 0; pl < 3; ++pl) B[pl] = stem_tr_fragment<16>(xbase + pl * C::PLANE + (2 * r + ky) * C::ROWB + 16 * s16 * 16);
+#pragma unroll
+          for (int ij = 2; ij >= 0; --ij)
+#pragma unroll
+            for (int i = 0; i <= ij; ++i) acc[ky] = __builtin_amdgcn_mfma_f32_32x32x16_bf16(A[i], B[ij - i], acc[ky], 0, 0, 0);
+        }
+      }
+    __syncthreads();
+  }
+  if (negated) {
+#pragma unroll
+    for (int ky = 0; ky < 7; ++ky) acc[ky] = -acc[ky];
+  }
+
+  float* const red = reinterpret_cast<float*>(smem);
+  __syncthreads();
+#pragma unroll 1
+  for (int rr = 0; rr < C::NW / 2; ++rr) {
+    if (rw == rr) {
+#pragma unroll
+      for (int ky = 0; ky < 7; ++ky)
+#pragma unroll
+        for (int v = 0; v < 16; ++v) {
+          float* const q = red + ((half * 7 + ky) * 16 + v) * 64 + lane;
+          *q = (rr == 0 ? 0.f : *q) + acc[ky][v];
+        }
+    }
+    __syncthreads();
+  }
+  for (int idx = tid; idx < 2 * 7 * 16 * 64; idx += C::NT) {
+    const int l = idx & 63, v = (idx >> 6) & 15, hk = idx >> 10;
+    const int ky = hk % 7, hf = hk / 7, n = l & 31;
+    const int co = 32 * hf + (v & 3) + 8 * (v >> 2) + 4 * (l >> 5);
+    if (n < 28) atomicAdd(a.dw + co * 196 + ky * 28 + n, red[idx]);
+  }
+}
+
+static bool stem_wgrad_applicable(const udaseg_conv_desc* d) {
+  if (!d || !f32_halo_enabled() || opt_get(UDASEG_OPT_STEM_WGRAD) == 0) return false;
+  if (d->kh != 7 || d->kw != 7 || d->stride != 2 || d->pad != 3 || d->ci != 4 || d->co != 64) return false;
+  if (d->n <= 0 || d->hi < 2 || d->wi < 2 || d->hi % 2 != 0 || d->wi % 2 != 0 || d->ho * 2 != d->hi || d->wo * 2 != d->wi) return false;
+  const long long pin = (long long)d->n * d->hi * d->wi, pout = (long long)d->n * d->ho * d->wo;
+  return pin * 16 < (1LL << 31) && pout * 256 < (1LL << 31) && device_lds_fits(StemWgradCfg::LDS);
+}
+
+bool stem_wgrad_ok(const udaseg_conv_desc* d) { return stem_wgrad_applicable(d); }
+
+int launch_stem_wgrad(const udaseg_conv_desc* d, const float* x, const float* dy, float* dw, int accumulate, hipStream_t st) {
+  using C = StemWgradCfg;
+  if (!stem_wgrad_applicable(d)) {
+    set_error("stem weight gradient: geometry not supported");
+    return UDASEG_E_UNSUPPORTED;
+  }
+  if (!accumulate) {
+    hipError_t e = hipMemsetAsync(dw, 0, (size_t)64 * 196 * sizeof(float), st);
+    if (e != hipSuccess) return hip_fail(e, "hipMemsetAsync(stem wgrad)");
+  }
+  StemWgradArgs a = {};
+  a.x = x; a.dy = dy; a.dw = dw;
+  a.n = d->n; a.h = d->hi; a.w = d->wi;
+  a.ntx = cdiv(d->wo, C::TW);
+  a.nty = cdiv(d->ho, C::TH);
+  a.signs = f3_signs_on() ? 1 : 0;
+  a.x_bytes = (unsigned)((long long)d->n * d->hi * d->wi * 16);
+  a.dy_bytes = (unsigned)((long long)d->n * d->ho * d->wo * 256);
+  const long long ntiles = (long long)d->n * a.nty * a.ntx;
+  if (ntiles <= 0) return UDASEG_OK;
+  a.ntiles = (int)ntiles;
+  const int opt = opt_get(UDASEG_OPT_STEM_WGRAD);
+  static std::atomic<int> per_cu{0};
+  if (per_cu == 0) {
+    hipError_t e = hipFuncSetAttribute(reinterpret_cast<const void*>(conv_stem_f32x3_kernel_wgrad),
+                                       hipFuncAttributeMaxDynamicSharedMemorySize, C::LDS);
+    if (e != hipSuccess) return hip_fail(e, "hipFuncSetAttribute(conv_stem_f32x3_kernel_wgrad)");
+    int occ = 0;
+    if (hipOccupancyMaxActiveBlocksPerMultiprocessor(&occ, conv_stem_f32x3_kernel_wgrad, C::NT, C::LDS) != hipSuccess || occ < 1) occ = 1;
+    per_cu = occ;
+  }
+  const long long want = opt >= 2 ? opt : (long long)device_cu_count() * per_cu;
+  const long long blocks = ntiles < want ? ntiles : want;
+  static std::atomic<int> kid{-1};
+  if (kid < 0) kid = kprof_id("conv_stem_f32x3_kernel_wgrad");
+  hipEvent_t ev = kprof_begin(st);
+  hipLaunchKernelGGL(conv_stem_f32x3_kernel_wgrad, dim3((unsigned)blocks), dim3(C::NT), C::LDS, st, a);
+  kprof_end(kid, ev, st, udaseg_conv_flops(d));
+  UDASEG_LAUNCH_CHECK("conv_stem_f32x3_kernel_wgrad launch");
+  return UDASEG_OK;
+}
+
 static bool stem_applicable(const udaseg_conv_desc* d) {
   if (!d || !f32_halo_enabled()) return false;
   if (d->kh != 7 || d->kw != 7 || d->stride != 2 || d->pad != 3 || d->ci != 4 || d->co != 64) return false;
   if (d->n <= 0 || d->hi < 2 || d->wi < 2 || d->hi % 2 != 0 || d->wi % 2 != 0 || d->ho * 2 != d->hi || d->wo * 2 != d->wi) return false;
   const long long pin = (long long)d->n * d->hi * d->wi, pout = (long long)d->n * d->ho * d->wo;
-  return pin * 16 < (1LL << 31) && pout * 256 < (1LL << 31);
+  return pin * 16 < (1LL << 31) && pout * 256 < (1LL << 31) && device_lds_fits(StemCfg::LDS);
 }
 
 }
@@ -232,13 +473,7 @@
   a.y_bytes = (unsigned)((long long)d->n * d->ho * d->wo * 256);
   const long long ntiles = (long long)d->n * a.nty * a.ntx;
   if (ntiles <= 0) return UDASEG_OK;
-  static int cus = 0;
-  if (cus == 0) {
-    int dev = 0;
-    hipDeviceProp_t pr;
-    cus = (hipGetDevice(&dev) == hipSuccess && hipGetDeviceProperties(&pr, dev) == hipSuccess && pr.multiProcessorCount > 0)
-              ? pr.multiProcessorCount : 256;
-  }
+  const int cus = device_cu_count();
   const long long blocks = ntiles < cus ? ntiles : cus;
   static std::atomic<bool> attr_done{false};
   if (!attr_done) {
diff --git a/uda_aerial_semantic_segmentation_research_amd/csrc/conv_wgrad.hip b/uda_aerial_semantic_segmentation_research_amd/csrc/conv_wgrad.hip
--- a/uda_aerial_semantic_segmentation_research_amd/csrc/conv_wgrad.hip
+++ b/uda_aerial_semantic_segmentation_research_amd/csrc/conv_wgrad.hip
@@ -898,6 +898,14 @@
 
 static bool wgrad_x3_on() {
   return udaseg::opt_get(UDASEG_OPT_WGRAD_X3) != 0 && udaseg::f32_split_enabled();
+}
+
+namespace udaseg {
+bool stem_wgrad_ok(const udaseg_conv_desc* d);
+int launch_stem_wgrad(const udaseg_conv_desc* d, const float* x, const float* dy, float* dw, int accumulate, hipStream_t st);
+bool n16_wgrad_ok(const udaseg_conv_desc* d, int up);
+int launch_n16_wgrad(const udaseg_conv_desc* d, const float* x, int up, const float* dy, float* dw, int accumulate, hipStream_t s,
+                     const float* in_scale, const float* in_shift, int in_act, float in_slope);
 }
 
 static int conv2d_wgrad_impl(const udaseg_conv_desc* d, const void* x, int src_c, int c_off, int up, const void* dy, float* dw,
@@ -940,6 +948,11 @@
     rc = d->co >= 128 ? launch_wgrad<128, 64, 2, 2>(a, accumulate, st, true)
        : d->co > 32   ? launch_wgrad<64, 64, 2, 2>(a, accumulate, st, true)
                       : launch_wgrad<32, 128, 1, 4>(a, accumulate, st, true);
+  else if (whole && !up && in_scale == nullptr && f32_split_enabled() && stem_wgrad_ok(d))
+    rc = launch_stem_wgrad(d, static_cast<const float*>(x), static_cast<const float*>(dy), dw, accumulate, st);
+  else if (whole && in_scale == nullptr && n16_wgrad_ok(d, up))
+    rc = launch_n16_wgrad(d, static_cast<const float*>(x), up, static_cast<const float*>(dy), dw, accumulate, st, nullptr, nullptr,
+                          UDASEG_ACT_NONE, 0.f);
   else if (whole && d->kh == d->kw &&
            small_wgrad_applicable(d->kh, d->stride, d->pad, d->ci, d->co, d->n * cdiv(d->hi, 16) * cdiv(d->wi, 16)))
     rc = launch_small_wgrad(static_cast<const float*>(x), static_cast<const float*>(dy), dw, d->n, d->hi, d->wi, d->ci, d->co,
@@ -984,6 +997,7 @@
   if (!d || d->kh != 3 || d->kw != 3 || d->stride != 1 || d->pad != 1 || d->n <= 0 || d->hi <= 0 || d->wi <= 0 || d->ci % 8 != 0 ||
       d->co % 4 != 0)
     return 0;
+  if (n16_wgrad_ok(d, up)) return 1;
   if (small_wgrad_applicable(d->kh, d->stride, d->pad, d->ci, d->co, d->n * cdiv(d->hi, 16) * cdiv(d->wi, 16))) return 1;
   return !up && !wgrad_halo_off(true) && wgrad_h2_applicable(d, 0, true) ? 1 : 0;
 }
@@ -999,14 +1013,17 @@
     return UDASEG_E_UNSUPPORTED;
   }
   hipStream_t st = as_stream(stream);
-  const bool small = small_wgrad_applicable(d->kh, d->stride, d->pad, d->ci, d->co, d->n * cdiv(d->hi, 16) * cdiv(d->wi, 16));
-  if (!small && !accumulate) {
+  const bool n16 = n16_wgrad_ok(d, up);
+  const bool small = !n16 && small_wgrad_applicable(d->kh, d->stride, d->pad, d->ci, d->co, d->n * cdiv(d->hi, 16) * cdiv(d->wi, 16));
+  if (!n16 && !small && !accumulate) {
     hipError_t e = hipMemsetAsync(dw, 0, (size_t)d->co * 9 * d->ci * sizeof(float), st);
     if (e != hipSuccess) return hip_fail(e, "hipMemsetAsync(dw)");
   }
   prof_begin(1, st);
   int rc;
-  if (small) {
+  if (n16) {
+    rc = launch_n16_wgrad(d, x, up, dy, dw, accumulate, st, in_scale, in_shift, in_act, in_slope);
+  } else if (small) {
     rc = launch_small_wgrad(x, dy, dw, d->n, d->hi, d->wi, d->ci, d->co, accumulate, st, up, in_scale, in_shift, in_act, in_slope);
   } else {
     rc = launch_wgrad_h2(d, x, nullptr, 0, dy, dw, true, st, in_scale, in_shift, in_act, in_slope);
diff --git a/uda_aerial_semantic_segmentation_research_amd/csrc/conv_wgrad_n16_f32x3.hip b/uda_aerial_semantic_segmentation_research_amd/csrc/conv_wgrad_n16_f32x3.hip
--- /dev/null
+++ b/uda_aerial_semantic_segmentation_research_amd/csrc/conv_wgrad_n16_f32x3.hip
@@ -0,0 +1,307 @@
+#include <stdlib.h>
+
+#include "common.h"
+#include "halo_common.h"
+
+namespace udaseg {
+
+struct N16WgradArgs {
+  const float* x;
+  const float* dy;
+  float* dw;
+  int n, h, w, ci, co, up;
+  int ntx, nty, ntiles;
+  int signs;
+  const float* in_scale;
+  const float* in_shift;
+  int in_act;
+  float in_slope;
+  unsigned x_bytes, dy_bytes;
+};
+
+template <int G, int T>
+struct N16WCfg {
+  static constexpr int NT = 256, NW = 4;
+  static constexpr int WR = G * T == 4 ? 2 : 1;
+  static constexpr int GW = G / WR;
+  static constexpr int TR = NW / WR, TW = 32, TP = TR * TW;
+  static constexpr int HR = TR + 2, HWD = TW + 2, HP = HR * HWD;
+  static constexpr int XCH = HP * 32, XPLANE = G * XCH;
+  static constexpr int DCH = TP * 32, DPLANE = T * DCH;
+  static constexpr int LDS = 3 * (XPLANE + DPLANE);
+  static constexpr int XO = 2 * G, DO = 2 * T;
+  static constexpr int XPC = HP * XO, DPC = TP * DO;
+  static constexpr int NX = (XPC + NT - 1) / NT, ND = (DPC + NT - 1) / NT;
+  static constexpr int RED = 9 * G * T * 64 * 4 * 4;
+  static_assert(NT % XO == 0, "one channel octet per staging thread");
+  static_assert(RED <= LDS && LDS <= 160 * 1024, "LDS");
+};
+
+typedef short n16w_s16x4 __attribute__((ext_vector_type(4)));
+__device__ __forceinline__ bf16x8 n16w_fragment(const char* p) {
+  const n16w_s16x4 lo = __builtin_amdgcn_ds_read_tr16_b64_v4i16((n16w_s16x4 __attribute__((address_space(3)))*)(p));
+  const n16w_s16x4 hi = __builtin_amdgcn_ds_read_tr16_b64_v4i16((n16w_s16x4 __attribute__((address_space(3)))*)(p + 128));
+  return __builtin_bit_cast(bf16x8, __builtin_shufflevector(lo, hi, 0, 1, 2, 3, 4, 5, 6, 7));
+}
+
+template <int G, int T, bool XF>
+__global__ __launch_bounds__(256) void conv3x3_n16_f32x3_kernel(const N16WgradArgs a) {
+  using C = N16WCfg<G, T>;
+  extern __shared__ __attribute__((aligned(16))) char smem[];
+  char* const Xs = smem;
+  char* const Ds = smem + 3 * C::XPLANE;
+  const int tid = threadIdx.x, lane = tid & 63;
+  const int wave = __builtin_amdgcn_readfirstlane(tid >> 6);
+  const int row = wave / C::WR, g0 = (wave % C::WR) * C::GW;
+  const int H = a.h, W = a.w;
+  const int P = gridDim.x;
+
+  __amdgpu_buffer_rsrc_t rs_x = __builtin_amdgcn_make_buffer_rsrc(const_cast<float*>(a.x), 0, (int)a.x_bytes, 0x00020000);
+  __amdgpu_buffer_rsrc_t rs_d = __builtin_amdgcn_make_buffer_rsrc(const_cast<float*>(a.dy), 0, (int)a.dy_bytes, 0x00020000);
+  f32x4 xsc[2] = {{0.f, 0.f, 0.f, 0.f}, {0.f, 0.f, 0.f, 0.f}}, xsh[2] = {{0.f, 0.f, 0.f, 0.f}, {0.f, 0.f, 0.f, 0.f}};
+  if constexpr (XF) {
+    const int ch = (tid % C::XO) * 8;
+#pragma unroll
+    for (int l = 0; l < 2; ++l)
+#pragma unroll
+      for (int e = 0; e < 4; ++e) {
+        const bool ok = ch + 4 * l + e < a.ci;
+        xsc[l][e] = ok ? a.in_scale[ch + 4 * l + e] : 0.f;
+        xsh[l][e] = ok ? a.in_shift[ch + 4 * l + e] : 0.f;
+      }
+  }
+  u32x4 sx[C::NX][2], sd[C::ND][2];
+  unsigned x_in = 0;
+  auto load_tile = [&](int tl) {
+    const int tx = tl % a.ntx;
+    const int t2 = tl / a.ntx;
+    const int ty = t2 % a.nty, img = t2 / a.nty;
+    const int y0 = ty * C::TR, x0 = tx * C::TW;
+    x_in = 0;
+#pragma unroll
+    for (int i = 0; i < C::NX; ++i) {
+      const int pc = tid + i * C::NT;
+      const int pix = pc / C::XO, oct = pc % C::XO;
+      const int hy = pix / C::HWD, hx = pix - hy * C::HWD;
+      const int iy = y0 + hy - 1, ix = x0 + hx - 1;
+      const bool ok = pc < C::XPC && (unsigned)iy < (unsigned)H && (unsigned)ix < (unsigned)W && oct * 8 < a.ci;
+      const int p = a.up ? (img * (H >> 1) + (iy >> 1)) * (W >> 1) + (ix >> 1) : (img * H + iy) * W + ix;
+      const unsigned off = ok ? (unsigned)((p * a.ci + oct * 8) * 4) : 0x80000000u;
+      x_in |= (ok ? 1u : 0u) << i;
+      sx[i][0] = __builtin_amdgcn_raw_buffer_load_b128(rs_x, (int)off, 0, 0);
+      sx[i][1] = __builtin_amdgcn_raw_buffer_load_b128(rs_x, (int)off, 16, 0);
+    }
+#pragma unroll
+    for (int i = 0; i < C::ND; ++i) {
+      const int pc = tid + i * C::NT;
+      const int pix = pc / C::DO, oct = pc % C::DO;
+      const int oy = y0 + pix / C::TW, ox = x0 + pix % C::TW;
+      const bool ok = pc < C::DPC && oy < H && ox < W && oct * 8 < a.co;
+      const unsigned off = ok ? (unsigned)((((img * H + oy) * W + ox) * a.co + oct * 8) * 4) : 0x80000000u;
+      sd[i][0] = __builtin_amdgcn_raw_buffer_load_b128(rs_d, (int)off, 0, 0);
+      sd[i][1] = __builtin_amdgcn_raw_buffer_load_b128(rs_d, (int)off, 16, 0);
+    }
+  };
+  auto store_tile = [&](unsigned dsgn) {
+#pragma unroll
+    for (int i = 0; i < C::NX; ++i) {
+      const int pc = tid + i * C::NT;
+      const int pix = pc / C::XO, oct = pc % C::XO;
+      if constexpr (XF) {
+        const bool in = (x_in >> i) & 1u;
+#pragma unroll
+        for (int l = 0; l < 2; ++l) {
+          f32x4 v = __builtin_bit_cast(f32x4, sx[i][l]);
+#pragma unroll
+          for (int e = 0; e < 4; ++e) {
+            const float t = act_apply(__builtin_fmaf(v[e], xsc[l][e], xsh[l][e]), a.in_act, a.in_slope);
+            v[e] = in ? t : 0.f;
+          }
+          sx[i][l] = __builtin_bit_cast(u32x4, v);
+        }
+      }
+      if (i < C::NX - 1 || pc < C::XPC) {
+        char* const dst = Xs + (oct >> 1) * C::XCH + pix * 32 + (oct & 1) * 16;
+        u32x4 p0, p1, p2;
+        split3(sx[i][0], sx[i][1], p0, p1, p2);
+        *reinterpret_cast<u32x4*>(dst) = p0;
+        *reinterpret_cast<u32x4*>(dst + C::XPLANE) = p1;
+        *reinterpret_cast<u32x4*>(dst + 2 * C::XPLANE) = p2;
+      }
+    }
+#pragma unroll
+    for (int i = 0; i < C::ND; ++i) {
+      const int pc = tid + i * C::NT;
+      const int pix = pc / C::DO, oct = pc % C::DO;
+      if (i < C::ND - 1 || pc < C::DPC) {
+        char* const dst = Ds + (oct >> 1) * C::DCH + pix * 32 + (oct & 1) * 16;
+        u32x4 p0, p1, p2;
+        split3(sd[i][0] ^ dsgn, sd[i][1] ^ dsgn, p0, p1, p2);
+        *reinterpret_cast<u32x4*>(dst) = p0;
+        *reinterpret_cast<u32x4*>(dst + C::DPLANE) = p1;
+        *reinterpret_cast<u32x4*>(dst + 2 * C::DPLANE) = p2;
+      }
+    }
+  };
+
+  f32x4 acc[9][C::GW][T];
+#pragma unroll
+  for (int t = 0; t < 9; ++t)
+#pragma unroll
+    for (int g = 0; g < C::GW; ++g)
+#pragma unroll
+      for (int c = 0; c < T; ++c) acc[t][g][c] = f32x4{0.f, 0.f, 0.f, 0.f};
+
+  const int lane_off = (8 * (lane >> 4) + ((lane & 15) >> 2)) * 32 + 8 * (lane & 3);
+  const char* const dbase = Ds + row * C::TW * 32 + lane_off;
+  const char* const xbase = Xs + g0 * C::XCH + row * C::HWD * 32 + lane_off;
+
+  const int nseq = (a.ntiles - (int)blockIdx.x + P - 1) / P;
+  const int sq1 = a.signs ? (nseq + 2) / 4 : 0, sq3 = a.signs ? nseq - sq1 : 0;
+  bool negated = false;
+  int tile = blockIdx.x, seq = 0;
+  if (tile < a.ntiles) load_tile(tile);
+  for (; tile < a.ntiles; tile += P, ++seq) {
+    const bool neg = seq >= sq1 && seq < sq3;
+    if (neg != negated) {
+      negated = neg;
+#pragma unroll
+      for (int t = 0; t < 9; ++t)
+#pragma unroll
+        for (int g = 0; g < C::GW; ++g)
+#pragma unroll
+          for (int c = 0; c < T; ++c) acc[t][g][c] = -acc[t][g][c];
+    }
+    store_tile(neg ? 0x80000000u : 0u);
+    __syncthreads();
+    if (tile + P < a.ntiles) load_tile(tile + P);
+    bf16x8 A[T][3];
+#pragma unroll
+    for (int c = 0; c < T; ++c)
+#pragma unroll
+      for (int pl = 0; pl < 3; ++pl) A[c][pl] = n16w_fragment(dbase + pl * C::DPLANE + c * C::DCH);
+#pragma unroll
+    for (int t = 0; t < 9; ++t) {
+#pragma unroll
+      for (int g = 0; g < C::GW; ++g) {
+        bf16x8 B[3];
+#pragma unroll
+        for (int pl = 0; pl < 3; ++pl) B[pl] = n16w_fragment(xbase + pl * C::XPLANE + g * C::XCH + ((t / 3) * C::HWD + t % 3) * 32);
+#pragma unroll
+        for (int c = 0; c < T; ++c)
+#pragma unroll
+          for (int ij = 2; ij >= 0; --ij)
+#pragma unroll
+            for (int i = 0; i <= ij; ++i)
+              acc[t][g][c] = __builtin_amdgcn_mfma_f32_16x16x32_bf16(A[c][i], B[ij - i], acc[t][g][c], 0, 0, 0);
+      }
+    }
+    __syncthreads();
+  }
+  if (negated) {
+#pragma unroll
+    for (int t = 0; t < 9; ++t)
+#pragma unroll
+      for (int g = 0; g < C::GW; ++g)
+#pragma unroll
+        for (int c = 0; c < T; ++c) acc[t][g][c] = -acc[t][g][c];
+  }
+
+  float* const red = reinterpret_cast<float*>(smem);
+  constexpr int NRED = 9 * G * T * 4 * 64;
+  for (int idx = tid; idx < NRED; idx += C::NT) red[idx] = 0.f;
+  __syncthreads();
+#pragma unroll
+  for (int t = 0; t < 9; ++t)
+#pragma unroll
+    for (int g = 0; g < C::GW; ++g)
+#pragma unroll
+      for (int c = 0; c < T; ++c)
+#pragma unroll
+        for (int v = 0; v < 4; ++v) atomicAdd(red + (((t * G + g0 + g) * T + c) * 4 + v) * 64 + lane, acc[t][g][c][v]);
+  __syncthreads();
+  for (int idx = tid; idx < NRED; idx += C::NT) {
+    const int l = idx & 63, v = (idx >> 6) & 3, r = idx >> 8;
+    const int c = r % T, g = (r / T) % G, t = r / (T * G);
+    const int co = 16 * c + 4 * (l >> 4) + v, ci = 16 * g + (l & 15);
+    if (co < a.co && ci < a.ci) atomicAdd(a.dw + ((size_t)co * 9 + t) * a.ci + ci, red[idx]);
+  }
+}
+
+bool n16_wgrad_ok(const udaseg_conv_desc* d, int up) {
+  if (!d || !f32_halo_enabled() || !f32_split_enabled() || opt_get(UDASEG_OPT_N16_WGRAD) == 0) return false;
+  if (d->kh != 3 || d->kw != 3 || d->stride != 1 || d->pad != 1 || d->ho != d->hi || d->wo != d->wi) return false;
+  if (d->n <= 0 || d->hi <= 0 || d->wi <= 0 || d->ci % 8 != 0 || d->co % 8 != 0 || d->ci > 32 || d->co > 32) return false;
+  if (up && (d->hi % 2 != 0 || d->wi % 2 != 0)) return false;
+  const long long px = (long long)d->n * d->hi * d->wi;
+  if (px * 32 * 4 >= (1LL << 31)) return false;
+  const int G = (d->ci + 15) / 16, T = (d->co + 15) / 16;
+  const int lds = G == 1 && T == 1 ? N16WCfg<1, 1>::LDS : G == 2 && T == 1 ? N16WCfg<2, 1>::LDS : G == 1 ? N16WCfg<1, 2>::LDS
+                                                                                                   : N16WCfg<2, 2>::LDS;
+  return device_lds_fits(lds);
+}
+
+template <int G, int T>
+static int launch_n16w_t(N16WgradArgs& a, long long blocks, hipStream_t s, double flops) {
+  using C = N16WCfg<G, T>;
+  a.ntx = cdiv(a.w, C::TW);
+  a.nty = cdiv(a.h, C::TR);
+  const long long ntiles = (long long)a.n * a.nty * a.ntx;
+  if (ntiles <= 0) return UDASEG_OK;
+  if (ntiles >= (1LL << 31)) return UDASEG_E_UNSUPPORTED;
+  a.ntiles = (int)ntiles;
+  
+  const bool xf = a.in_scale != nullptr;
+  auto kern = xf ? conv3x3_n16_f32x3_kernel<G, T, true> : conv3x3_n16_f32x3_kernel<G, T, false>;
+  static std::atomic<int> per_cu[2] = {{0}, {0}};
+  if (per_cu[xf] == 0) {
+    hipError_t e = hipFuncSetAttribute(reinterpret_cast<const void*>(kern), hipFuncAttributeMaxDynamicSharedMemorySize, C::LDS);
+    if (e != hipSuccess) return hip_fail(e, "hipFuncSetAttribute(conv3x3_n16_f32x3 wgrad)");
+    int occ = 0;
+    if (hipOccupancyMaxActiveBlocksPerMultiprocessor(&occ, kern, C::NT, C::LDS) != hipSuccess || occ < 1) occ = 1;
+    per_cu[xf] = occ;
+  }
+  if (blocks <= 0) blocks = (long long)device_cu_count() * per_cu[xf];
+  static std::atomic<int> kid[2] = {{-1}, {-1}};
+  if (kid[xf] < 0) {
+    char nm[64];
+    snprintf(nm, sizeof(nm), "conv3x3_n16_f32x3_kernel<%d, %d, %s>", G, T, xf ? "true" : "false");
+    kid[xf] = kprof_id(nm);
+  }
+  if (blocks > ntiles) blocks = ntiles;
+  hipEvent_t ev = kprof_begin(s);
+  hipLaunchKernelGGL(kern, dim3((unsigned)blocks), dim3(C::NT), C::LDS, s, a);
+  kprof_end(kid[xf], ev, s, flops);
+  UDASEG_LAUNCH_CHECK("conv3x3_n16_f32x3 wgrad launch");
+  return UDASEG_OK;
+}
+
+int launch_n16_wgrad(const udaseg_conv_desc* d, const float* x, int up, const float* dy, float* dw, int accumulate, hipStream_t s,
+                     const float* in_scale, const float* in_shift, int in_act, float in_slope) {
+  if (!n16_wgrad_ok(d, up)) {
+    set_error("sixteen-wide weight gradient: geometry not supported");
+    return UDASEG_E_UNSUPPORTED;
+  }
+  if (!accumulate) {
+    hipError_t e = hipMemsetAsync(dw, 0, (size_t)d->co * 9 * d->ci * sizeof(float), s);
+    if (e != hipSuccess) return hip_fail(e, "hipMemsetAsync(n16 wgrad)");
+  }
+  N16WgradArgs a = {};
+  a.x = x; a.dy = dy; a.dw = dw;
+  a.n = d->n; a.h = d->hi; a.w = d->wi; a.ci = d->ci; a.co = d->co; a.up = up ? 1 : 0;
+  a.signs = f3_signs_on() ? 1 : 0;
+  a.in_scale = in_scale; a.in_shift = in_shift; a.in_act = in_act; a.in_slope = in_slope;
+  const long long px = (long long)d->n * d->hi * d->wi;
+  a.x_bytes = (unsigned)((up ? px / 4 : px) * d->ci * 4);
+  a.dy_bytes = (unsigned)(px * d->co * 4);
+  const int opt = opt_get(UDASEG_OPT_N16_WGRAD);
+  const long long blocks = opt >= 2 ? opt : 0;
+  const double fl = udaseg_conv_flops(d);
+  const int G = (d->ci + 15) / 16, T = (d->co + 15) / 16;
+  if (G == 1 && T == 1) return launch_n16w_t<1, 1>(a, blocks, s, fl);
+  if (G == 2 && T == 1) return launch_n16w_t<2, 1>(a, blocks, s, fl);
+  if (G == 1 && T == 2) return launch_n16w_t<1, 2>(a, blocks, s, fl);
+  return launch_n16w_t<2, 2>(a, blocks, s, fl);
+}
+
+}
```

New measurement: 1122 (median of 6 runs). 1.01x the previous value.
